# uberalex974/Reinforcement-Learning

Hardware: AMD Instinct MI355X
Metric: env-steps/sec (whole node) at 32768 arenas; PPO wall-clock per 1M steps (higher is better)
Workload: dtype f32

## Files before the change

### include/rlgpu_env.h

```cpp
#ifndef RLGPU_ENV_H
#define RLGPU_ENV_H

#include <stdint.h>
#include "rlgpu_arith.h"
#include "rlgpu_core.h"

#ifdef __cplusplus
extern "C" {
#endif

#define RLGPU_CARS 4
#define RLGPU_PADS 34
#define RLGPU_MANIFOLDS 12
#define RLGPU_MAX_SOLVER_ROWS 14
#define RLGPU_MAX_MESH_OBJECTS 32
#define RLGPU_OBS 167
#define RLGPU_ACTIONS 90
#define RLGPU_REWARDS 13
#define RLGPU_MAX_REWARDS 32
#define RLGPU_MAX_TERMINALS 8
#define RLGPU_SS_KICKOFF 0
#define RLGPU_SS_FUZZED_KICKOFF 1

enum {
// ... 96 lines not shown
    uint8_t prev_is_flipping[RLGPU_CARS];
    uint8_t prev_on_ground[RLGPU_CARS];
    uint8_t has_prev;
    uint8_t terminal;
    uint8_t pad[2];
    float prev_action[RLGPU_CARS][8];
    float no_touch_time;
    int32_t score_blue, score_orange;
    int32_t penalty_blue, penalty_orange;
    uint8_t ev_bump[RLGPU_CARS], ev_bumped[RLGPU_CARS], ev_demo[RLGPU_CARS], ev_demoed[RLGPU_CARS];
    uint32_t rng_counter;
    uint32_t manifold_overflow;
    int32_t episode_steps;
    uint16_t bp_cell[RLGPU_CARS + 1];
    uint8_t bp_rank[RLGPU_CARS + 1];
    uint8_t pad1;
} rlgpu_env_extra;

typedef struct {
    rlgpu_body ball;
    float ball_vel_impulse_cache[3];
    int32_t ball_sleeping;
    rlgpu_car cars[RLGPU_CARS];
    rlgpu_pad pads[RLGPU_PADS];
    rlgpu_env_extra env;
} rlgpu_arena_state;

typedef struct {
    int32_t num_arenas;
    int32_t tick_skip;
    int32_t action_delay;
    uint64_t seed;
    int32_t save_rewards;
    int32_t max_episode_steps;
    const float* mesh_tris;
    int32_t mesh_ntris;
    int32_t mesh_objects;
    const int32_t* mesh_object_ntris;
    const rlgpu_reward_spec* rewards;
    int32_t n_rewards;
    const rlgpu_terminal_spec* terminals;
    int32_t n_terminals;
    int32_t arith;
    int32_t arena_offset;
    int32_t state_setter;
} rlgpu_envset_config;

typedef struct {
    float* obs;
    uint8_t* masks;
    float* rewards;
    int8_t* terminals;
    float* trunc_obs;
} rlgpu_step_outputs;

typedef struct rlgpu_envset rlgpu_envset;

typedef struct {
    float* obs;
    uint8_t* action_masks;
    float* rewards;
    uint8_t* terminals;
    float* last_rewards;
    float* trunc_obs;
    int32_t num_players;
    int32_t num_arenas;
    int32_t num_rewards;
    int32_t* arena_player_start;
} rlgpu_envset_buffers;

int rlgpu_envset_create(const rlgpu_envset_config* cfg, rlgpu_envset** out);
int rlgpu_envset_destroy(rlgpu_envset* env);
int rlgpu_envset_buffers_get(rlgpu_envset* env, rlgpu_envset_buffers* out);

int rlgpu_envset_reset(rlgpu_envset* env, void* stream);
int rlgpu_envset_reset_arenas(rlgpu_envset* env, const uint8_t* d_mask, void* stream);

int rlgpu_envset_step_first_half(rlgpu_envset* env, void* stream);
int rlgpu_envset_step_second_half(rlgpu_envset* env, const int32_t* d_actions, void* stream);
int rlgpu_envset_step(rlgpu_envset* env, const int32_t* d_actions, int32_t reset_terminated,
                      const rlgpu_step_outputs* out, void* stream);
int rlgpu_envset_step_range(rlgpu_envset* env, int32_t first, int32_t count, const int32_t* d_actions,
                            int32_t reset_terminated, const rlgpu_step_outputs* out, void* stream);
int rlgpu_envset_sync(rlgpu_envset* env, void* stream);
int rlgpu_envset_set_output_only(rlgpu_envset* env, int32_t enable);

int rlgpu_envset_get_arenas(rlgpu_envset* env, int32_t first, int32_t count, rlgpu_arena_state* h_out);
int rlgpu_envset_set_arenas(rlgpu_envset* env, int32_t first, int32_t count, const rlgpu_arena_state* h_in);
int rlgpu_envset_build_obs(rlgpu_envset* env, void* stream);

int rlgpu_envset_set_profile(rlgpu_envset* env, unsigned long long* d_counters, int64_t capacity);

enum {
    RLGPU_SM_IN_AIR = 0,
    RLGPU_SM_BALL_TOUCH = 1,
    RLGPU_SM_DEMOED = 2,
    RLGPU_SM_SPEED = 3,
    RLGPU_SM_SPEED_TO_BALL = 4,
    RLGPU_SM_BOOST = 5,
    RLGPU_SM_TOUCH_HEIGHT = 6,
    RLGPU_SM_GOAL_SPEED = 7,
    RLGPU_NUM_STEP_METRICS = 8,
    RLGPU_SM_SLOT_GOAL_SPEED = 28,
    RLGPU_SM_SLOT_GOALS = 29,
    RLGPU_SM_SLOT_PASSES = 30,
    RLGPU_STEP_METRIC_SLOTS = 32
};
const char* rlgpu_step_metric_name(int32_t i);
int rlgpu_envset_enable_step_metrics(rlgpu_envset* env, int32_t enable);
int rlgpu_envset_step_metrics(rlgpu_envset* env, double* h_total, uint64_t* h_count, int32_t reset, void* stream);
int rlgpu_envset_step_metric_slots(rlgpu_envset* env, double* h_out, void* stream);

int rlgpu_envset_default_plugins(rlgpu_reward_spec* rewards, int32_t* n_rewards, rlgpu_terminal_spec* terminals,
                                 int32_t* n_terminals);

int rlgpu_arena_state_size(void);

#ifdef __cplusplus
}
#endif
#endif
```

### include/rlgpu_ppo.h

```cpp
#ifndef RLGPU_PPO_H
#define RLGPU_PPO_H

#include <stdint.h>
#include "rlgpu_core.h"

#ifdef __cplusplus
extern "C" {
#endif

#define RLGPU_MAX_LAYERS 8

typedef struct {
    int32_t obs_size;
    int32_t num_actions;
    int32_t policy_layers[RLGPU_MAX_LAYERS];
    int32_t n_policy_layers;
    int32_t critic_layers[RLGPU_MAX_LAYERS];
    int32_t n_critic_layers;
    int32_t layer_norm;
    float leaky_slope;
    int32_t activation;
    float policy_lr, critic_lr;
    float beta1, beta2, eps, weight_decay;
    float clip_range;
    float entropy_scale;
    float max_grad_norm;
    int32_t max_rows;
    uint64_t seed;
    int32_t train_gemm;
    int32_t infer_fp16;
    int32_t shared_layers[RLGPU_MAX_LAYERS];
    int32_t n_shared_layers;
    int64_t sample_row_offset;
    float policy_temperature;
    int32_t mask_entropy;
} rlgpu_ppo_config;

enum { RLGPU_GEMM_F32X6 = 0, RLGPU_GEMM_F32 = 1, RLGPU_GEMM_F16X3 = 2 };
enum { RLGPU_ACT_LEAKY_RELU = 0, RLGPU_ACT_RELU = 1, RLGPU_ACT_SIGMOID = 2, RLGPU_ACT_TANH = 3 };
enum { RLGPU_INFER_BF16 = 0, RLGPU_INFER_F16 = 1, RLGPU_INFER_F32 = 2 };

typedef struct rlgpu_ppo rlgpu_ppo;

enum {
    RLGPU_M_ENTROPY = 0, RLGPU_M_KL, RLGPU_M_POLICY_LOSS, RLGPU_M_CRITIC_LOSS, RLGPU_M_RATIO,
    RLGPU_M_CLIP_FRACTION, RLGPU_M_COUNT, RLGPU_M_GRAD_NORM_POLICY, RLGPU_M_GRAD_NORM_CRITIC,
    RLGPU_M_GRAD_NORM_SHARED, RLGPU_NUM_METRICS = 16
};

int rlgpu_ppo_create(const rlgpu_ppo_config* cfg, rlgpu_ppo** out);
int rlgpu_ppo_destroy(rlgpu_ppo* h);
int32_t rlgpu_ppo_config_size(void);

int rlgpu_ppo_buffers(rlgpu_ppo* h, float** d_params, float** d_grads, int64_t* num_params);
int rlgpu_ppo_model_range(rlgpu_ppo* h, int32_t model, int64_t* offset, int64_t* count);
int rlgpu_ppo_init_params(rlgpu_ppo* h, uint64_t seed, void* stream);
int rlgpu_ppo_refresh_half(rlgpu_ppo* h, void* stream);

int rlgpu_debug_infer_trace(void* d_buf, int64_t capacity);
int rlgpu_kernel_timing(int32_t enable);
int rlgpu_kernel_timing_read(double* ms, double* work, int64_t* count, int32_t nslots);

int rlgpu_ppo_forward(rlgpu_ppo* h, int32_t model, int32_t precision, const float* d_in, int32_t n,
                      float* d_out, void* stream);

int rlgpu_ppo_infer_actions(rlgpu_ppo* h, const float* d_obs, const uint8_t* d_masks, int32_t n,
                            int32_t deterministic, uint64_t rng_step, int32_t* d_actions, float* d_logp,
                            void* stream);
int rlgpu_ppo_set_version(rlgpu_ppo* h, const float* d_policy_params, void* stream);
int rlgpu_ppo_infer_actions_mixed(rlgpu_ppo* h, const float* d_obs, const uint8_t* d_masks, int32_t n,
                                  int32_t deterministic, uint64_t rng_step, const uint8_t* d_old_rows,
                                  int32_t* d_actions, float* d_logp, void* stream);
int rlgpu_ppo_infer_actions_rows(rlgpu_ppo* h, const float* d_obs, const uint8_t* d_masks, int32_t n, int64_t row0,
                                 int32_t deterministic, uint64_t rng_step, const uint8_t* d_old_rows,
                                 int32_t* d_actions, float* d_logp, void* stream);
int rlgpu_ppo_fused_infer(rlgpu_ppo* h, int32_t model);
int rlgpu_ppo_infer_critic(rlgpu_ppo* h, const float* d_obs, int64_t n, float* d_values, void* stream);

int rlgpu_mean_std(const float* d_x, int64_t n, float* d_out, void* stream);

int rlgpu_ppo_minibatch(rlgpu_ppo* h, const float* d_obs, const uint8_t* d_masks, const int32_t* d_actions,
                        const float* d_old_logp, const float* d_adv, const float* d_target,
                        const int32_t* d_index, int64_t start, int32_t n, int64_t batch_size,
                        const float* d_adv_stats, float* d_metrics, void* stream);

int rlgpu_ppo_optimizer_step(rlgpu_ppo* h, float* d_metrics, void* stream);
int rlgpu_ppo_zero_grad(rlgpu_ppo* h, void* stream);
int rlgpu_ppo_optimizer_state(rlgpu_ppo* h, int64_t* step, float** d_exp_avg, float** d_exp_avg_sq);
int rlgpu_ppo_set_optimizer_step(rlgpu_ppo* h, int64_t step);

int rlgpu_gemm(int32_t mode, int32_t a_layout, int32_t b_layout, const float* d_A, int64_t lda, const float* d_B,
               int64_t ldb, float* d_C, int64_t ldc, const float* d_bias, int32_t I, int32_t J, int32_t K, int32_t splits,
               void* stream);
int rlgpu_gemm_f32(int32_t a_layout, int32_t b_layout, const float* d_A, int64_t lda, const float* d_B, int64_t ldb,
                   float* d_C, int64_t ldc, const float* d_bias, int32_t I, int32_t J, int32_t K, int32_t splits,
                   void* stream);

int rlgpu_permutation(int64_t n, uint64_t seed, uint64_t counter, int32_t* d_out, void* stream);

#ifdef __cplusplus
}
#endif
#endif
```

### reinforcement-learning_amd/csrc/common.hpp

```cpp
#pragma once
#include <hip/hip_runtime.h>
#include <cstdint>
#include <cstdio>
#include <stdexcept>
#include <string>

#include "../../include/rlgpu_core.h"

namespace rlgpu {

void set_last_error(const std::string& msg);

struct Error : std::runtime_error {
    int code;
    Error(int c, const std::string& m) : std::runtime_error(m), code(c) {}
};

#define RLGPU_CHECK_HIP(expr)                                                                \
    do {                                                                                     \
        hipError_t _e = (expr);                                                              \
        if (_e != hipSuccess)                                                                \
            throw ::rlgpu::Error(RLGPU_ERR_HIP, std::string(#expr " failed: ") +             \
                                                    hipGetErrorString(_e));                  \
    } while (0)

#define RLGPU_REQUIRE(cond, msg)                                                             \
    do {                                                                                     \
        if (!(cond)) throw ::rlgpu::Error(RLGPU_ERR_INVALID_ARG, std::string(msg));          \
    } while (0)

template <class F>
inline int guarded(F&& f) {
    try {
        f();
        return RLGPU_OK;
    } catch (const Error& e) {
        set_last_error(e.what());
        return e.code;
    } catch (const std::bad_alloc&) {
        set_last_error("host allocation failed");
        return RLGPU_ERR_OOM;
    } catch (const std::exception& e) {
        set_last_error(e.what());
        return RLGPU_ERR_STATE;
    }
}

inline hipStream_t as_stream(void* s) { return reinterpret_cast<hipStream_t>(s); }

inline unsigned ceil_div(int64_t a, int64_t b) { return (unsigned)((a + b - 1) / b); }

void launch_mlp_infer_act(int act, bool f16, unsigned blocks, hipStream_t s, const void* args, size_t bytes);

}
```

### reinforcement-learning_amd/csrc/env.hip

```cpp
#include <mutex>
#include <algorithm>
#include <cmath>
#include <cstring>
#include <string>
#include <vector>

#include "common.hpp"
#include "env_step.hpp"
#include "mesh.hpp"
#include "../../include/rlgpu_gamestate.h"

namespace rl {
void env_k0_upload(const EnvConst& k, const RsqrtLut* lut);
void env_k1_upload(const EnvConst& k, const RsqrtLut* lut);
void env_k2_upload(const EnvConst& k, const RsqrtLut* lut);
void env_k0_launch(const StepArgs& g, int blocks, hipStream_t s);
void env_k1_launch(const StepArgs& g, int blocks, hipStream_t s);
void env_k2_launch(const StepArgs& g, int blocks, hipStream_t s);

static m3 host_euler_ypr(float yaw, float pitch, float roll) {
    float ci = std::cos(roll), cj = std::cos(pitch), ch = std::cos(yaw);
    float si = std::sin(roll), sj = std::sin(pitch), sh = std::sin(yaw);
    float cc = ci * ch, cs = ci * sh, sc = si * ch, ss = si * sh;
    return m3{v3{cj * ch, sj * sc - cs, sj * cc + ss}, v3{cj * sh, sj * ss + cc, sj * cs - sc}, v3{-sj, cj * si, cj * ci}};
}

static EnvConst make_env_const() {
    EnvConst k;
    std::memset(&k, 0, sizeof k);
    const float UU = 1.f / 50.f;
    k.ball_radius = 91.25f * UU;
    float elem = 0.4f * kBallMass * k.ball_radius * k.ball_radius;
    k.ball_inv_inertia = v3{1.f / elem, 1.f / elem, 1.f / elem};
    k.ball_inv_mass = 1.f / kBallMass;
    v3 hs = v3{120.507f, 86.6994f, 38.6591f} * UU;
    v3 h = v3{hs.x / 2.f, hs.y / 2.f, hs.z / 2.f};
    const float m0 = 0.04f;
    v3 impl = v3{h.x - m0, h.y - m0, h.z - m0};
    const float mn_half = h.x < h.y ? (h.x < h.z ? h.x : h.z) : (h.y < h.z ? h.y : h.z);
    const float safe = 0.1f * mn_half;
    k.car_margin = m0;
    if (safe < k.car_margin) {
        const v3 with_m = impl + v3{m0, m0, m0};
        k.car_margin = safe;
        impl = with_m - v3{safe, safe, safe};
    }
    k.car_impl = impl;
    {
        const v3 mn = v3{-4500.f * UU, -6000.f * UU, 0.f * UU}, mx = v3{4500.f * UU, 6000.f * UU, 2500.f * UU};
        const float cell = 370.f * UU * 1.f;
        const v3 range = mx - mn;
        k.bp_min = mn;
        k.bp_inv_cell = 1.f / cell;
        k.bp_cells[0] = std::max(1, (int)std::ceil(range.x / cell));
        k.bp_cells[1] = std::max(1, (int)std::ceil(range.y / cell));
        k.bp_cells[2] = std::max(1, (int)std::ceil(range.z / cell));
    }
    k.car_half = impl + v3{k.car_margin, k.car_margin, k.car_margin};
    k.car_offset = v3{13.87566f, 0.f, 20.755f} * UU;
    float lx = 2.f * k.car_half.x, ly = 2.f * k.car_half.y, lz = 2.f * k.car_half.z;
    v3 inertia = v3{ly * ly + lz * lz, lx * lx + lz * lz, lx * lx + ly * ly} * (kCarMass / 12.f);
    k.car_inv_inertia = v3{1.f / inertia.x, 1.f / inertia.y, 1.f / inertia.z};
    k.car_inv_mass = 1.f / kCarMass;
    for (int i = 0; i < 4; i++) {
        bool front = i < 2, left = i % 2;
        float radius = front ? 12.50f : 15.00f;
        v3 off = front ? v3{51.25f, 25.90f, 20.755f} : v3{-33.75f, 29.50f, 20.755f};
        if (left) off.y *= -1;
        float rest = (front ? 38.755f : 37.055f) - 12.f;
        k.wheel_conn[i] = off * UU;
        k.wheel_rest[i] = rest * UU;
        k.wheel_radius[i] = radius * UU;
        k.wheel_force_scale[i] = front ? (36.f - (1.f / 4.f)) : (54.f + (1.f / 4.f) + (1.5f / 100.f));
    }
    k.susp_travel = ((12.f * UU) * 100.f) / 100.f;
    k.ball_cbt = (float)((double)k.ball_radius + 0.08) * 0.02f;
    {
        v3 mn = k.car_offset - k.car_half, mx = k.car_offset + k.car_half;
        v3 c = (mn + mx) * 0.5f;
        float r = len(mx - mn) * 0.5f;
        k.car_cbt = (r + len(c)) * 0.02f;
    }
    k.gravity = v3{0, 0, -650.f} * UU;
    k.ball_damp = (float)std::pow((double)(1.f - 0.03f), (double)(1.f / 120.f));
    k.plane_n[0] = v3{0, 0, 1};
    k.plane_p[0] = v3{0, 0, 0};
    k.plane_n[1] = v3{0, 0, -1};
    k.plane_p[1] = v3{0, 0, 2048} * UU;
    k.plane_n[2] = v3{1, 0, 0};
    k.plane_p[2] = v3{-4096, 0, 2048 / 2} * UU;
    k.plane_n[3] = v3{-1, 0, 0};
    k.plane_p[3] = v3{4096, 0, 2048 / 2} * UU;
    for (int p = 0; p < 4; p++) {
        const v3 n = k.plane_n[p];
        k.plane_axis[p] = -1;
        if (std::fabs(n.x) == 1.f && n.y == 0.f && n.z == 0.f) k.plane_axis[p] = 0;
        if (n.x == 0.f && std::fabs(n.y) == 1.f && n.z == 0.f) k.plane_axis[p] = 1;
        if (n.x == 0.f && n.y == 0.f && std::fabs(n.z) == 1.f) k.plane_axis[p] = 2;
    }
    const float sx[5] = {-2048, 2048, -256, 256, 0}, sy[5] = {-2560, -2560, -3840, -3840, -4608};
    const float syaw[5] = {(float)(M_PI_4 * 1), (float)(M_PI_4 * 3), (float)(M_PI_4 * 2), (float)(M_PI_4 * 2), (float)(M_PI_4 * 2)};
// ... 181 lines not shown
        for (int i = 0; i < p.nr; i++) {
            const rlgpu_reward_spec& r = cfg->rewards[i];
            if (r.type < 0 || r.type >= RLGPU_NUM_REWARD_TYPES)
                throw rlgpu::Error(RLGPU_ERR_UNSUPPORTED,
                                   "rlgpu_envset_create: reward " + std::to_string(i) + " has unknown type " +
                                       std::to_string(r.type) + " (the device registry holds types 0.." +
                                       std::to_string(RLGPU_NUM_REWARD_TYPES - 1) + ", include/rlgpu_env.h RLGPU_RW_*)");
            p.rw[i] = r;
        }
    } else {
        RLGPU_REQUIRE(cfg->n_rewards == 0, "rlgpu_envset_create: n_rewards without a rewards list");
    }
    if (cfg->terminals) {
        RLGPU_REQUIRE(cfg->n_terminals >= 0 && cfg->n_terminals <= RLGPU_MAX_TERMINALS,
                      "rlgpu_envset_create: n_terminals must be in [0, " + std::to_string(RLGPU_MAX_TERMINALS) + "]");
        p.nt = cfg->n_terminals;
        for (int i = 0; i < p.nt; i++) {
            const rlgpu_terminal_spec& t = cfg->terminals[i];
            if (t.type < 0 || t.type >= RLGPU_NUM_TERMINAL_TYPES)
                throw rlgpu::Error(RLGPU_ERR_UNSUPPORTED,
                                   "rlgpu_envset_create: terminal condition " + std::to_string(i) + " has unknown type " +
                                       std::to_string(t.type) + " (the device registry holds types 0.." +
                                       std::to_string(RLGPU_NUM_TERMINAL_TYPES - 1) + ", include/rlgpu_env.h RLGPU_TC_*)");
            p.tc[i] = t;
        }
    } else {
        RLGPU_REQUIRE(cfg->n_terminals == 0, "rlgpu_envset_create: n_terminals without a terminals list");
    }
    return p;
}
}

extern "C" int rlgpu_envset_default_plugins(rlgpu_reward_spec* rewards, int32_t* n_rewards, rlgpu_terminal_spec* terminals,
                                            int32_t* n_terminals) {
    return rlgpu::guarded([&] {
        rl::Plugins p;
        example_main_plugins(p);
        if (rewards) std::memcpy(rewards, p.rw, sizeof(rlgpu_reward_spec) * p.nr);
        if (n_rewards) *n_rewards = p.nr;
        if (terminals) std::memcpy(terminals, p.tc, sizeof(rlgpu_terminal_spec) * p.nt);
        if (n_terminals) *n_terminals = p.nt;
    });
}

namespace {
struct EnvKernel {
    void (*upload)(const rl::EnvConst& k, const rl::RsqrtLut* lut);
    void (*launch)(const rl::StepArgs& g, int blocks, hipStream_t s);
};
const EnvKernel kEnvKernel[RLGPU_NUM_ARITH] = {{rl::env_k0_upload, rl::env_k0_launch},
                                               {rl::env_k1_upload, rl::env_k1_launch},
                                               {rl::env_k2_upload, rl::env_k2_launch}};
static_assert(RLGPU_ARITH_MSVC_X64 == 0 && RLGPU_ARITH_GCC_X64 == 1 && RLGPU_ARITH_SCALAR == 2, "kEnvKernel's order");

std::mutex g_init_mu;
struct DeviceInit {
    bool consts = false, rsqrt = false;
};
std::vector<DeviceInit> g_device_init;

void device_init(int arith) {
    std::lock_guard<std::mutex> lk(g_init_mu);
    int dev = 0;
    RLGPU_CHECK_HIP(hipGetDevice(&dev));
    if ((int)g_device_init.size() <= dev) g_device_init.resize(dev + 1);
    DeviceInit& done = g_device_init[dev];
    const bool consts = !done.consts, rsqrt = rl::sse_api(arith) && !done.rsqrt;
    if (!consts && !rsqrt) return;
    rl::RsqrtLut L{};
    if (rsqrt) {
        int bits = 0;
        const std::vector<uint32_t>& t = rlgpu::x86_rsqrt_table_or_throw(&bits);
        uint32_t* d = nullptr;
        RLGPU_CHECK_HIP(hipMalloc(&d, t.size() * sizeof(uint32_t)));
        RLGPU_CHECK_HIP(hipMemcpy(d, t.data(), t.size() * sizeof(uint32_t), hipMemcpyHostToDevice));
        L = rl::RsqrtLut{d, bits};
        RLGPU_CHECK_HIP(hipMemcpyToSymbol(HIP_SYMBOL(rl::kRsqrtLut), &L, sizeof L));
    }
    const rl::EnvConst k = rl::make_env_const();
    if (consts) RLGPU_CHECK_HIP(hipMemcpyToSymbol(HIP_SYMBOL(rl::C), &k, sizeof k));
    for (int a = 0; a < RLGPU_NUM_ARITH; a++) {
        const bool lut = rsqrt && rl::sse_api(a);
        if (consts || lut) kEnvKernel[a].upload(k, lut ? &L : nullptr);
    }
    done.consts = true;
    done.rsqrt = done.rsqrt || rsqrt;
}

void output_only_rows(const rlgpu_envset* e, rl::StepArgs& g) {
    if (!e->output_only) return;
    if (g.out_obs) g.obs = nullptr;
    if (g.out_masks) g.masks = nullptr;
    if (g.out_trunc) g.trunc_obs = nullptr;
}

struct Range {
    int first, count;
};
Range whole(const rlgpu_envset* e) { return Range{0, e->cfg.num_arenas}; }

void launch(rlgpu_envset* e, rl::StepArgs g, Range r, hipStream_t s) {
    const size_t a0 = (size_t)r.first, p0 = a0 * 4, nr = (size_t)e->plug.nr;
    g.arenas = e->d_arenas + a0 * rl::kRec;
    g.n = r.count;
    g.obs = e->d_obs + p0 * RLGPU_OBS;
    g.masks = e->d_masks + p0 * RLGPU_ACTIONS;
    g.rewards = e->d_rewards + p0;
    g.terminals = e->d_terminals + a0;
    g.last_rewards = e->cfg.save_rewards ? e->d_last_rewards + a0 * nr : nullptr;
    g.trunc_obs = e->d_trunc_obs + p0 * RLGPU_OBS;
    g.seed = e->cfg.seed;
    g.max_episode_steps = e->cfg.max_episode_steps;
    g.prof = e->d_prof;
    g.mesh = e->mesh;
    g.mesh.gjk = e->mesh.gjk + a0 / rl::kArenas * rl::kWG;
    g.plug = e->d_plug;
    g.arith = e->cfg.arith;
    g.arena_offset = e->cfg.arena_offset + r.first;
    g.fuzz = e->cfg.state_setter == RLGPU_SS_FUZZED_KICKOFF;
    g.pen_slots = e->pen_slots;
    g.reward_values = g.build && e->d_reward_values ? e->d_reward_values + p0 * nr : nullptr;
    output_only_rows(e, g);
    if (g.build && e->d_metrics) {
        if (r.first == 0) e->metric_players = (++e->metric_calls % 4) == 0;
        g.metrics = e->d_metrics + a0 * RLGPU_STEP_METRIC_SLOTS;
        g.metrics_players = e->metric_players;
    }
    kEnvKernel[e->cfg.arith].launch(g, rlgpu::ceil_div(r.count, rl::kArenas), s);
    RLGPU_CHECK_HIP(hipGetLastError());
}

rl::StepArgs blank(rl::ResetMode reset = rl::kResetNone) {
    rl::StepArgs g;
    std::memset(&g, 0, sizeof g);
    g.reset_mode = reset;
    return g;
}

rl::StepArgs step_args(const rlgpu_envset* e, bool first_half, const int32_t* d_actions,
                       rl::ResetMode reset = rl::kResetNone, const rlgpu_step_outputs* out = nullptr) {
    rl::StepArgs g = blank(reset);
    if (first_half) g.ticks_first = e->cfg.action_delay;
    if (d_actions) {
        g.actions = d_actions;
        g.ticks_second = e->cfg.tick_skip - e->cfg.action_delay;
        g.build = 1;
    }
    if (out) {
        g.out_obs = out->obs;
        g.out_masks = out->masks;
        g.out_rew = out->rewards;
        g.out_term = out->terminals;
        g.out_trunc = out->trunc_obs;
    }
    return g;
}

rl::StepArgs fused_step_args(const rlgpu_envset* e, const int32_t* d_actions, int32_t reset_terminated,
                             const rlgpu_step_outputs* out) {
    RLGPU_REQUIRE(e->cfg.action_delay > 0, "fused step needs actionDelay > 0");
    return step_args(e, true, d_actions, reset_terminated ? rl::kResetTerminated : rl::kResetNone, out);
}

void copy_records(const rlgpu_envset* e, int first, int count, void* host, hipMemcpyKind dir) {
    char* dev = e->d_arenas + (size_t)first * rl::kRec;
    const size_t rec = sizeof(rlgpu_arena_state);
    if (dir == hipMemcpyDeviceToHost)
        RLGPU_CHECK_HIP(hipMemcpy2D(host, rec, dev, rl::kRec, rec, count, dir));
    else
        RLGPU_CHECK_HIP(hipMemcpy2D(dev, rl::kRec, host, rec, rec, count, dir));
}

void download_metric_slots(const rlgpu_envset* e, double* h_out, hipStream_t s) {
    RLGPU_REQUIRE(e->d_metrics, "step metrics are not enabled (rlgpu_envset_enable_step_metrics)");
    RLGPU_CHECK_HIP(hipMemcpyAsync(h_out, e->d_metrics,
                                   (size_t)e->cfg.num_arenas * RLGPU_STEP_METRIC_SLOTS * sizeof(double),
                                   hipMemcpyDeviceToHost, s));
    RLGPU_CHECK_HIP(hipStreamSynchronize(s));
}

void free_set(rlgpu_envset* e) {
    for (void* p : e->allocs) (void)hipFree(p);
    (void)hipFree(e->d_metrics);
    (void)hipFree(e->d_reward_values);
    delete e;
}

}

extern "C" int rlgpu_arena_state_size(void) { return (int)sizeof(rlgpu_arena_state); }

extern "C" int rlgpu_envset_create(const rlgpu_envset_config* cfg, rlgpu_envset** out) {
    return rlgpu::guarded([&] {
        RLGPU_REQUIRE(cfg && out, "rlgpu_envset_create: null argument");
        RLGPU_REQUIRE(cfg->num_arenas > 0, "rlgpu_envset_create: num_arenas must be > 0");
        RLGPU_REQUIRE(cfg->tick_skip > 0, "tickSkip must be > 0 (EnvSet.cpp:48)");
        RLGPU_REQUIRE(cfg->action_delay >= 0 && cfg->action_delay <= cfg->tick_skip,
                      "actionDelay must be in [0, tickSkip] (EnvSet.cpp:49)");
        RLGPU_REQUIRE(cfg->mesh_tris == nullptr || cfg->mesh_ntris > 0, "mesh_ntris must be > 0 with mesh_tris");
        RLGPU_REQUIRE(cfg->arith >= 0 && cfg->arith < RLGPU_NUM_ARITH,
                      "rlgpu_envset_create: unknown arithmetic mode " + std::to_string(cfg->arith) + " (RLGPU_ARITH_*)");
        RLGPU_REQUIRE(cfg->state_setter == RLGPU_SS_KICKOFF || cfg->state_setter == RLGPU_SS_FUZZED_KICKOFF,
                      "rlgpu_envset_create: unknown state setter " + std::to_string(cfg->state_setter) + " (RLGPU_SS_*)");
        const rl::Plugins plug = plugins_from(cfg);
        device_init(cfg->arith);
        std::vector<float> builtin;
        const float* tris = cfg->mesh_tris;
        int ntris = cfg->mesh_ntris;
        if (!tris) {
            builtin = rlgpu::builtin_mesh_bt();
            tris = builtin.data();
// ... 156 lines not shown
}

extern "C" float* rlgpu_envset_reward_values(rlgpu_envset* e) { return e ? e->d_reward_values : nullptr; }

extern "C" int rlgpu_envset_download_gamestates(rlgpu_envset* e, int32_t first, int32_t count, rlgpu_gamestate* h_out,
                                                void* stream) {
    return rlgpu::guarded([&] {
        RLGPU_REQUIRE(e && h_out, "rlgpu_envset_download_gamestates: null argument");
        RLGPU_REQUIRE(first >= 0 && count >= 0 && first + count <= e->cfg.num_arenas, "arena range out of bounds");
        if (count == 0) return;
        RLGPU_CHECK_HIP(hipStreamSynchronize(rlgpu::as_stream(stream)));
        std::vector<rlgpu_arena_state> rec((size_t)count);
        copy_records(e, first, count, rec.data(), hipMemcpyDeviceToHost);
        rlgpu::gamestates_from_arenas(rec.data(), count, e->cfg.tick_skip, h_out);
    });
}

extern "C" int rlgpu_envset_buffers_get(rlgpu_envset* e, rlgpu_envset_buffers* out) {
    return rlgpu::guarded([&] {
        RLGPU_REQUIRE(e && out, "rlgpu_envset_buffers_get: null argument");
        out->obs = e->d_obs;
        out->action_masks = e->d_masks;
        out->rewards = e->d_rewards;
        out->terminals = e->d_terminals;
        out->last_rewards = e->d_last_rewards;
        out->trunc_obs = e->d_trunc_obs;
        out->num_players = e->num_players;
        out->num_arenas = e->cfg.num_arenas;
        out->num_rewards = e->plug.nr;
        out->arena_player_start = e->d_player_start;
    });
}

extern "C" int rlgpu_envset_reset(rlgpu_envset* e, void* stream) {
    return rlgpu::guarded([&] {
        RLGPU_REQUIRE(e, "null envset");
        launch(e, blank(rl::kResetSet), whole(e), rlgpu::as_stream(stream));
    });
}

extern "C" int rlgpu_envset_reset_arenas(rlgpu_envset* e, const uint8_t* d_mask, void* stream) {
    return rlgpu::guarded([&] {
        RLGPU_REQUIRE(e, "null envset");
        rl::StepArgs g = blank(rl::kResetMask);
        g.reset_mask = d_mask;
        launch(e, g, whole(e), rlgpu::as_stream(stream));
    });
}

extern "C" int rlgpu_envset_step_first_half(rlgpu_envset* e, void* stream) {
    return rlgpu::guarded([&] {
        RLGPU_REQUIRE(e, "null envset");
        launch(e, step_args(e, true, nullptr), whole(e), rlgpu::as_stream(stream));
    });
}

extern "C" int rlgpu_envset_step_second_half(rlgpu_envset* e, const int32_t* d_actions, void* stream) {
    return rlgpu::guarded([&] {
        RLGPU_REQUIRE(e && d_actions, "rlgpu_envset_step_second_half: null argument");
        launch(e, step_args(e, false, d_actions), whole(e), rlgpu::as_stream(stream));
    });
}

extern "C" int rlgpu_envset_step(rlgpu_envset* e, const int32_t* d_actions, int32_t reset_terminated,
                                 const rlgpu_step_outputs* out, void* stream) {
    return rlgpu::guarded([&] {
        RLGPU_REQUIRE(e && d_actions, "rlgpu_envset_step: null argument");
        launch(e, fused_step_args(e, d_actions, reset_terminated, out), whole(e), rlgpu::as_stream(stream));
    });
}

extern "C" int rlgpu_envset_step_range(rlgpu_envset* e, int32_t first, int32_t count, const int32_t* d_actions,
                                       int32_t reset_terminated, const rlgpu_step_outputs* out, void* stream) {
    return rlgpu::guarded([&] {
        RLGPU_REQUIRE(e && d_actions, "rlgpu_envset_step_range: null argument");
        const rl::StepArgs g = fused_step_args(e, d_actions, reset_terminated, out);
        RLGPU_REQUIRE(first >= 0 && count > 0 && first + count <= e->cfg.num_arenas && first % rl::kArenas == 0,
                      "rlgpu_envset_step_range: the range must lie in the set and start at a multiple of 4");
        RLGPU_REQUIRE(!e->d_prof, "rlgpu_envset_step_range: not with the per-phase profile");
        launch(e, g, Range{first, count}, rlgpu::as_stream(stream));
    });
}

extern "C" int rlgpu_envset_set_output_only(rlgpu_envset* e, int32_t enable) {
    return rlgpu::guarded([&] {
        RLGPU_REQUIRE(e, "null envset");
        e->output_only = enable != 0;
    });
}

extern "C" int rlgpu_envset_sync(rlgpu_envset* e, void* stream) {
    return rlgpu::guarded([&] {
        RLGPU_REQUIRE(e, "null envset");
        RLGPU_CHECK_HIP(hipStreamSynchronize(rlgpu::as_stream(stream)));
    });
}

extern "C" int rlgpu_envset_build_obs(rlgpu_envset* e, void* stream) {
    return rlgpu::guarded([&] {
        RLGPU_REQUIRE(e, "null envset");
        launch(e, blank(rl::kRebuildObs), whole(e), rlgpu::as_stream(stream));
    });
}

extern "C" int rlgpu_envset_get_arenas(rlgpu_envset* e, int32_t first, int32_t count, rlgpu_arena_state* h_out) {
    return rlgpu::guarded([&] {
        RLGPU_REQUIRE(e && h_out, "null argument");
        RLGPU_REQUIRE(first >= 0 && count >= 0 && first + count <= e->cfg.num_arenas, "arena range out of bounds");
        if (count == 0) return;
        RLGPU_CHECK_HIP(hipDeviceSynchronize());
        copy_records(e, first, count, h_out, hipMemcpyDeviceToHost);
    });
}

extern "C" int rlgpu_envset_set_arenas(rlgpu_envset* e, int32_t first, int32_t count, const rlgpu_arena_state* h_in) {
    return rlgpu::guarded([&] {
        RLGPU_REQUIRE(e && h_in, "null argument");
        RLGPU_REQUIRE(first >= 0 && count >= 0 && first + count <= e->cfg.num_arenas, "arena range out of bounds");
        if (count == 0) return;
        RLGPU_CHECK_HIP(hipDeviceSynchronize());
        copy_records(e, first, count, const_cast<rlgpu_arena_state*>(h_in), hipMemcpyHostToDevice);
    });
}

namespace rl {
__global__ void __launch_bounds__(16) box_triangle_kernel(int n, const float* rot, const float* centre, const float* tri,
                                                          const float* cbt, float* out, gjk::GjkScratch* scratch,
                                                          int lds, int ar) {
    __shared__ char small[16][gjk::kSmallBytes];
    __shared__ int lock[16];
    const int i = blockIdx.x * 16 + threadIdx.x;
    lock[threadIdx.x] = 0;
    if (i >= n) return;
    const float* r = rot + 9 * (size_t)i;
    const m3 R = m3{v3{r[0], r[1], r[2]}, v3{r[3], r[4], r[5]}, v3{r[6], r[7], r[8]}};
    const v3 c = v3{centre[3 * (size_t)i], centre[3 * (size_t)i + 1], centre[3 * (size_t)i + 2]};
    const float* t = tri + 9 * (size_t)i;
    const gjk::Shape sh{C.car_impl, C.car_margin, v3{t[0], t[1], t[2]}, v3{t[3], t[4], t[5]}, v3{t[6], t[7], t[8]}, ar};
    v3 nrm, pt;
    float d = 0.f;
    gjk::Scr slow = gjk::hbm_view(scratch + i);
    gjk::Scr fast = gjk::lds_view(small[threadIdx.x]);
    const bool hit = gjk::box_triangle(R, c, sh, cbt[i], lds ? &fast : nullptr, &lock[threadIdx.x], slow, nrm, pt, d);
    float* o = out + 8 * (size_t)i;
    o[0] = hit ? 1.f : 0.f;
    o[1] = hit ? nrm.x : 0.f;
    o[2] = hit ? nrm.y : 0.f;
    o[3] = hit ? nrm.z : 0.f;
    o[4] = hit ? pt.x : 0.f;
    o[5] = hit ? pt.y : 0.f;
    o[6] = hit ? pt.z : 0.f;
    o[7] = hit ? d : 0.f;
}
__device__ __forceinline__ void bt_load(int i, const float* rot, const float* centre, const float* tri, int ar, m3& R, v3& c,
                                        gjk::Shape& sh) {
    const float* r = rot + 9 * (size_t)i;
    R = m3{v3{r[0], r[1], r[2]}, v3{r[3], r[4], r[5]}, v3{r[6], r[7], r[8]}};
    c = v3{centre[3 * (size_t)i], centre[3 * (size_t)i + 1], centre[3 * (size_t)i + 2]};
    const float* t = tri + 9 * (size_t)i;
    sh = gjk::Shape{C.car_impl, C.car_margin, v3{t[0], t[1], t[2]}, v3{t[3], t[4], t[5]}, v3{t[6], t[7], t[8]}, ar};
}
__device__ __forceinline__ void bt_store(float* out, int i, bool hit, v3 nrm, v3 pt, float d) {
    float* o = out + 8 * (size_t)i;
    o[0] = hit ? 1.f : 0.f;
    o[1] = hit ? nrm.x : 0.f;
    o[2] = hit ? nrm.y : 0.f;
// ... 162 lines not shown
```

### reinforcement-learning_amd/csrc/env_step.hpp

```cpp
#pragma once
#include "env_builders.hpp"

namespace rl {

enum ResetMode : int {
    kResetNone = 0,
    kResetTerminated = 1,
    kResetSet = 2,
    kResetMask = 3,
    kResetAll = 4,
    kRebuildObs = 5
};

struct StepArgs {
    char* arenas;
    int n;
    int ticks_first;
    const int32_t* actions;
    int ticks_second;
    int build;
    int reset_mode;
    const uint8_t* reset_mask;
    float* obs;
    uint8_t* masks;
    float* rewards;
    uint8_t* terminals;
    float* last_rewards;
    float* trunc_obs;
    float* out_obs;
    uint8_t* out_masks;
    float* out_rew;
    int8_t* out_term;
    float* out_trunc;
    int max_episode_steps;
    uint64_t seed;
    unsigned long long* prof;
    MeshView mesh;
    double* metrics;
    int metrics_players;
    const Plugins* plug;
    int arith;
    int arena_offset;
    float* reward_values;
    int fuzz;
    int pen_slots;
};

#ifdef RLGPU_ENV_KERNEL

DEV void step_metrics(ArenaLDS* A, int l, double* m, bool players) {
    if (players) {
        const rlgpu_car& c = A->s.cars[l];
        const v3 pos = ld3(c.body.pos) * kBT2UU, vel = ld3(c.body.vel) * kBT2UU;
        const v3 bp = ld3(A->s.ball.pos) * kBT2UU;
        const bool touched = A->a.touched[l] != 0;
        const v3 dir = rs_norm(bp - pos);
        const float toward = vel.x * dir.x + vel.y * dir.y + vel.z * dir.z;
        m[RLGPU_SM_IN_AIR * 4 + l] += c.is_on_ground ? 0.0 : 1.0;
        m[RLGPU_SM_BALL_TOUCH * 4 + l] += touched ? 1.0 : 0.0;
        m[RLGPU_SM_DEMOED * 4 + l] += c.is_demoed ? 1.0 : 0.0;
        m[RLGPU_SM_SPEED * 4 + l] += (double)rs_len(vel);
        m[RLGPU_SM_SPEED_TO_BALL * 4 + l] += (double)(0.f > toward ? 0.f : toward);
        m[RLGPU_SM_BOOST * 4 + l] += (double)c.boost;
        if (touched) m[RLGPU_SM_TOUCH_HEIGHT * 4 + l] += (double)bp.z;
    }
    if (l == 0) {
        if (players) m[RLGPU_SM_SLOT_PASSES] += 1.0;
        if (A->a.goal) {
            m[RLGPU_SM_SLOT_GOAL_SPEED] += (double)rs_len(ld3(A->s.ball.vel) * kBT2UU);
            m[RLGPU_SM_SLOT_GOALS] += 1.0;
        }
    }
}


constexpr int kPadsPerLane = (RLGPU_PADS + kTeam - 1) / kTeam;
struct PadRegs {
    int px[kPadsPerLane], py[kPadsPerLane];
    v3 pos[kPadsPerLane], bmin[kPadsPerLane], bmax[kPadsPerLane];
    float rad[kPadsPerLane];
};
DEV void load_pad_regs(PadRegs& R, int l) {
#pragma unroll
    for (int k = 0; k < kPadsPerLane; k++) {
        const int p = l + k * kTeam < RLGPU_PADS ? l + k * kTeam : 0;
        R.px[k] = C.pad_cell_x[p];
        R.py[k] = C.pad_cell_y[p];
        R.pos[k] = C.pad_pos_bt[p];
        R.bmin[k] = C.pad_box_min[p];
        R.bmax[k] = C.pad_box_max[p];
        R.rad[k] = (C.pad_big[p] ? 208.f : 144.f) * kUU2BT;
    }
}

DEV void tick(ArenaLDS* A, const MeshView& M, int l, bool valid, uint64_t seed, int arena, Prof& P, const PadRegs& R,
                          int nvalid) {
    if (valid) {
        rlgpu_arena_state& s = A->s;
        if (l == 0) {
            A->u.wc.njob = 0;
            bool sleep = len2(ld3(s.ball.vel)) == 0 && len2(ld3(s.ball.angvel)) == 0;
            s.ball_sleeping = sleep;
            A->a.ball_sleep = sleep;
            A->a.active[0] = 1;
        } else if (l < 5) {
            const int c = l - 1;
            A->a.active[c + 1] = !s.cars[c].is_demoed;
            float* ctl = s.cars[c].controls;
            for (int k = 0; k < 5; k++) ctl[k] = stdclamp(ctl[k], -1.f, 1.f);
        }
        if (l < 5) {
            A->a.snap_vel[l] = bvel(A, l);
            A->a.snap_ang[l] = bang(A, l);
        }
    }
    sync();
    if (valid && l == 0) {
        rlgpu_arena_state& s = A->s;
        for (int c = 0; c < 4; c++) {
            rlgpu_car& cs = s.cars[c];
            if (cs.is_demoed) {
                cs.demo_respawn_timer = stdmax(cs.demo_respawn_timer - kTick, 0.f);
                if (cs.demo_respawn_timer == 0.f) {
                    int idx = (int)(rng_next(A, seed, arena) % 4u);
                    bool orange = c & 1;
                    v3 pos = v3{C.respawn_x[idx], C.respawn_y[idx] * (orange ? -1.f : 1.f), 36.f};
                    set_car_state(A, c, pos, C.respawn_rot[orange][idx], 100.f / 3.f, false);
                }
            }
        }
    }
// ... 167 lines not shown
            const int px = R.px[k], py = R.py[k];
            const v3 ppos = R.pos[k];
            const float rad = R.rad[k];
            const uint32_t prev_locked = A->s.pads[p].prev_locked_car_id;
            int locked = -1;
#pragma unroll
            for (int ci = 0; ci < 4; ci++) {
                if (px < cx0[ci] || px > cx1[ci] || py < cy0[ci] || py > cy1[ci]) continue;
                v3 cpos = cp[ci];
                bool col = false;
                if (prev_locked == (uint32_t)(ci + 1)) {
                    v3 mn, mx;
                    body_aabb(ci + 1, cpos, ldm(A->s.cars[ci].body.rot), mn, mx);
                    const v3 bmin = R.bmin[k], bmax = R.bmax[k];
                    col = (bmax.x > mn.x && bmax.y > mn.y && bmax.z > mn.z) && (bmin.x < mx.x && bmin.y < mx.y && bmin.z < mx.z);
                } else {
                    float dx = cpos.x - ppos.x, dy = cpos.y - ppos.y;
                    if (dx * dx + dy * dy < rad * rad) col = fabsf(cpos.z - ppos.z) < (95.f * kUU2BT);
                }
                if (col) locked = ci;
            }
            A->a.locked[p] = locked;
        }
    }
    sync();
    P.mark(9);
    uint64_t picked[kPadsPerLane];
#pragma unroll
    for (int k = 0; k < kPadsPerLane; k++) {
        const int p = l + k * kTeam;
        bool pick = false;
        if (valid && p < RLGPU_PADS) {
            rlgpu_pad& pd = A->s.pads[p];
            const int lk = A->a.locked[p];
            if (lk >= 0 && pd.is_active) {
                pick = true;
                pd.is_active = 0;
                pd.cooldown = R.rad[k] > 144.f * kUU2BT ? 10.f : 4.f;
            }
            pd.prev_locked_car_id = lk >= 0 ? (uint32_t)(lk + 1) : 0u;
        }
        picked[k] = __ballot(pick);
    }
    if (valid && l == 0) {
        const int team = (int)(threadIdx.x >> 4);
#pragma unroll
        for (int k = 0; k < kPadsPerLane; k++)
            for (uint32_t bits = (uint32_t)(picked[k] >> (16 * team)) & 0xffffu; bits; bits &= bits - 1u) {
                const int p = __ffs(bits) - 1 + k * kTeam;
                rlgpu_car& cs = A->s.cars[A->a.locked[p]];
                cs.boost = stdmin(cs.boost + (C.pad_big[p] ? 100.f : 12.f), 100.f);
            }
        rlgpu_body* b = &A->s.ball;
        v3 v = ld3(b->vel), w = ld3(b->angvel);
        v3 cache = ld3(A->s.ball_vel_impulse_cache);
        if (!is_zero(cache)) {
            v += cache;
            st3(A->s.ball_vel_impulse_cache, zero3());
        }
        const float maxv = 6000.f * kUU2BT;
        if (len2(v) > maxv * maxv) v = bt_normalize(v, arith(A)) * maxv;
        if (len2(w) > 6.f * 6.f) w = bt_normalize(w, arith(A)) * 6.f;
        st3(b->vel, v);
        st3(b->angvel, w);
        A->s.env.tick_count++;
    }
    sync();
    P.mark(10);
}

DEV void copy_rows(ArenaLDS* A, int l, int arena, float* obs, uint8_t* masks) {
    if (obs) {
        const float* src = &A->u.out.obs[0][0];
        float* dst = obs + (size_t)arena * 4 * RLGPU_OBS;
        for (int k = l; k < 4 * RLGPU_OBS; k += kTeam) dst[k] = src[k];
    }
    if (masks) {
        const uint8_t* msrc = &A->u.out.masks[0][0];
        uint8_t* mdst = masks + (size_t)arena * 4 * RLGPU_ACTIONS;
        for (int k = l; k < 4 * RLGPU_ACTIONS; k += kTeam) mdst[k] = msrc[k];
    }
}

__global__ void __launch_bounds__(kWG) RLGPU_ENV_KERNEL(StepArgs g) {
    __shared__ ArenaLDS lds[kArenas];
    const int team = threadIdx.x >> 4, l = threadIdx.x & 15;
    const int arena = blockIdx.x * kArenas + team;
    const bool valid = arena < g.n;
    ArenaLDS* A = &lds[team];
    Prof P{g.prof, g.prof ? (long long)clock64() : 0};
    {
        int first = blockIdx.x * kArenas;
        int cnt = g.n - first < kArenas ? g.n - first : kArenas;
        const int chunks = kRec / 16;
        for (int k = threadIdx.x; k < cnt * chunks; k += kWG) {
            int a = k / chunks, c = k % chunks;
            const uint4* src = (const uint4*)(g.arenas + (size_t)(first + a) * kRec) + c;
            uint4* dst = (uint4*)&lds[a] + c;
            *dst = *src;
        }
    }
    sync(); P.mark(11);
    if (valid && l < 5) {
        A->a.force[l] = zero3();
        A->a.torque[l] = zero3();
        update_inertia(A, l);
    }
    if (l == 0) {
        A->a.epa_lock = A->a.npen = 0;
        A->a.arith = g.arith;
    }
    if (threadIdx.x == 0) g_pen_save.cap = g.pen_slots;
    sync(); P.mark(11);
    if (g.ticks_first > 0) {
        if (valid && l == 0) {
            rlgpu_env_extra& e = A->s.env;
            for (int i = 0; i < 3; i++) e.prev_ball_vel[i] = A->s.ball.vel[i] * kBT2UU;
            for (int i = 0; i < 4; i++) {
                e.prev_boost[i] = A->s.cars[i].boost;
                e.prev_is_flipping[i] = A->s.cars[i].is_flipping;
                e.prev_on_ground[i] = A->s.cars[i].is_on_ground;
                e.ev_bump[i] = e.ev_bumped[i] = e.ev_demo[i] = e.ev_demoed[i] = 0;
            }
            e.has_prev = 1;
        }
        sync(); P.mark(11);
    }
    {
        PadRegs pregs;
        load_pad_regs(pregs, l);
        const int t1 = g.ticks_first, t2 = g.actions ? g.ticks_second : 0;
        for (int t = 0;; t++) {
            if (g.actions && t == t1) {
                if (valid && l < 4) {
                    int a = g.actions[arena * 4 + l];
                    a = a < 0 ? 0 : (a > RLGPU_ACTIONS - 1 ? RLGPU_ACTIONS - 1 : a);
                    const float* x = C.action[a];
                    float* c = A->s.cars[l].controls;
                    for (int k = 0; k < 5; k++) c[k] = x[k];
                    c[5] = x[5] == 1 ? 1.f : 0.f;
                    c[6] = x[6] == 1 ? 1.f : 0.f;
                    c[7] = x[7] == 1 ? 1.f : 0.f;
                    for (int k = 0; k < 8; k++) A->s.env.prev_action[l][k] = x[k];
                }
                sync(); P.mark(11);
            }
            if (t >= t1 + t2) break;
            tick(A, g.mesh, l, valid, g.seed, arena + g.arena_offset, P, pregs, stdmin(kArenas, g.n - (int)blockIdx.x * kArenas));
        }
    }
    uint8_t term = 0;
    if (g.build) {
        if (valid && l == 0) {
            rlgpu_env_extra& e = A->s.env;
            int64_t cur = e.tick_count;
            int64_t tick_skip = cur - e.last_tick_count > 0 ? cur - e.last_tick_count : 0;
            float delta_time = (int)tick_skip * (1.0f / 120.0f);
            bool any = false;
            for (int i = 0; i < 4; i++) {
                const rlgpu_car& c = A->s.cars[i];
                bool t = c.ball_hit_valid && (uint64_t)c.ball_hit_tick >= (uint64_t)(cur - tick_skip);
                A->a.touched[i] = t;
                any |= t;
            }
            float by = A->s.ball.pos[1] * kBT2UU;
            bool goal = fabsf(by) > (5124.25f + 91.25f);
            A->a.goal = goal;
            if (any) e.no_touch_time = 0;
            else e.no_touch_time += delta_time;
            if (goal) {
                if (by > 0) e.score_blue++;
                else e.score_orange++;
            }
            uint8_t tt = 0;
            for (int k = 0; k < g.plug->nt; k++) {
                const rlgpu_terminal_spec& tc = g.plug->tc[k];
                bool hit = false, trunc = false;
                if (tc.type == RLGPU_TC_NO_TOUCH) {
                    hit = !any && e.no_touch_time >= tc.param;
                    trunc = true;
                } else if (tc.type == RLGPU_TC_SCORE_LIMIT) {
                    const int lim = (int)tc.param;
                    hit = (e.score_blue >= lim) || (e.score_orange >= lim);
                } else if (tc.type == RLGPU_TC_GOAL_SCORE) {
                    hit = goal;
                }
                if (hit) {
                    const uint8_t cur = trunc ? 2 : 1;
                    if (tt == 0 || cur == 1) tt = cur;
                }
            }
            e.terminal = tt;
            if (goal) {
                if (by > 0) e.penalty_blue++;
                else e.penalty_orange++;
            }
            e.episode_steps++;
            uint8_t tj = tt;
            if (!tj && g.max_episode_steps > 0 && e.episode_steps >= g.max_episode_steps) tj = 2;
            if (tj) e.episode_steps = 0;
            A->a.traj_term = tj;
        }
        sync(); P.mark(12);
        if (valid) {
            const int pi = l & 3, q = l >> 2;
            const PView me = view_player(A, pi);
            v3 bp = ld3(A->s.ball.pos) * kBT2UU, bv = ld3(A->s.ball.vel) * kBT2UU, pbv = ld3(A->s.env.prev_ball_vel);
            const int nr = g.plug->nr;
            constexpr int kPer = (RLGPU_MAX_REWARDS + 3) / 4;
            float ov[kPer];
#pragma unroll
            for (int k = 0; k < kPer; k++) ov[k] = 0.f;
#pragma unroll 1
            for (int k = 0; q + 4 * k < nr; k++) {
                const int r = q + 4 * k;
                const float o = reward_value(A, g.plug->rw[r], pi, me, bp, bv, pbv, A->a.goal != 0);
#pragma unroll
                for (int j = 0; j < kPer; j++) ov[j] = j == k ? o : ov[j];
                if (pi == 0 && g.last_rewards) g.last_rewards[(size_t)arena * nr + r] = o;
                if (g.reward_values) g.reward_values[((size_t)arena * 4 + pi) * nr + r] = o;
            }
            float all = 0.f;
            const int base = (int)(threadIdx.x & ~15u) + pi;
#pragma unroll
            for (int r = 0; r < RLGPU_MAX_REWARDS; r++) {
                if (r >= nr) break;
                const float o = __shfl(ov[r >> 2], base + 4 * (r & 3));
                all += o * g.plug->rw[r].weight;
            }
            if (l < 4) A->a.all_rewards[l] = all;
        }
        sync(); P.mark(12);
        if (valid && l < 4) {
            float r = A->a.all_rewards[l];
            g.rewards[arena * 4 + l] = r;
            if (g.out_rew) g.out_rew[arena * 4 + l] = r;
            if (g.out_term) g.out_term[arena * 4 + l] = (int8_t)A->a.traj_term;
        }
        if (g.metrics && valid && l < 4) step_metrics(A, l, g.metrics + (size_t)arena * RLGPU_STEP_METRIC_SLOTS,
                                                      g.metrics_players != 0);
        uint8_t tj = 0;
        if (valid) {
            term = A->s.env.terminal;
            tj = (uint8_t)A->a.traj_term;
        }
        sync(); P.mark(12);
        if (valid && l == 0) {
            g.terminals[arena] = term;
            A->s.env.last_tick_count = A->s.env.tick_count;
        }
        const bool fused_reset = g.reset_mode == kResetTerminated && valid && term != 0;
        if (valid) build_obs_rows(A, l);
        sync(); P.mark(13);
        if (valid) {
            copy_rows(A, l, arena, g.obs, g.masks);
            if (!fused_reset) copy_rows(A, l, arena, g.out_obs, g.out_masks);
            if (tj == 2) {
                copy_rows(A, l, arena, g.trunc_obs, nullptr);
                copy_rows(A, l, arena, g.out_trunc, nullptr);
            }
        }
        sync(); P.mark(13);
        if (g.reset_mode == kResetTerminated) {
            if (fused_reset && l == 0) kickoff_reset(A, g.seed, arena + g.arena_offset, g.fuzz != 0);
            sync(); P.mark(14);
            if (fused_reset) build_obs_rows(A, l);
            sync(); P.mark(14);
            if (fused_reset) {
                copy_rows(A, l, arena, g.obs, g.masks);
                copy_rows(A, l, arena, g.out_obs, g.out_masks);
            }
            sync(); P.mark(14);
        }
    }
    if (g.reset_mode >= kResetSet) {
        bool do_reset = false;
        if (valid) {
            if (g.reset_mode == kResetSet) do_reset = g.terminals[arena] != 0;
            else if (g.reset_mode == kResetMask) do_reset = g.reset_mask ? g.reset_mask[arena] != 0 : true;
            else if (g.reset_mode == kResetAll) do_reset = true;
        }
        sync(); P.mark(14);
        if (do_reset && l == 0) {
            kickoff_reset(A, g.seed, arena + g.arena_offset, g.fuzz != 0);
            if (g.reset_mode == kResetSet) g.terminals[arena] = 0;
        }
        sync(); P.mark(14);
        bool rebuild = do_reset || (valid && g.reset_mode == kRebuildObs);
        if (rebuild) build_obs_rows(A, l);
        sync(); P.mark(14);
        if (rebuild) copy_rows(A, l, arena, g.obs, g.masks);
        sync(); P.mark(14);
    }
    {
        int first = blockIdx.x * kArenas;
        int cnt = g.n - first < kArenas ? g.n - first : kArenas;
        const int chunks = kRec / 16;
        for (int k = threadIdx.x; k < cnt * chunks; k += kWG) {
            int a = k / chunks, c = k % chunks;
            uint4* dst = (uint4*)(g.arenas + (size_t)(first + a) * kRec) + c;
            const uint4* src = (const uint4*)&lds[a] + c;
            *dst = *src;
        }
    }
    P.mark(15);
    if (g.prof && valid && l == 0 && A->a.npen) {
        atomicAdd(&g.prof[28], (unsigned long long)A->a.npen);
        atomicAdd(&g.prof[kProfWG + (size_t)blockIdx.x * kProfPhases + 23], (unsigned long long)A->a.npen);
        atomicAdd(&g.prof[kProfWG + (size_t)gridDim.x * kProfPhases + arena], (unsigned long long)A->a.npen);
    }
}
#endif

}
```

### reinforcement-learning_amd/csrc/infer_kernels.hpp

```cpp
#pragma once
#include <hip/hip_runtime.h>
#include <stdint.h>

#include "mlp_kernels.hpp"
#include "ppo_kernels.hpp"

namespace infer {

using mlp::bf16x8;
using mlp::f32x16;
using mlp::h2f;
using mlp::f2h;
using mlp::u32x4;

constexpr int IR = 64;
constexpr int IW = 8;
constexpr int IT = 64 * IW;
constexpr int IRW = IR / IW;
constexpr int IMAX = 512;
constexpr int IPITCH = IMAX + 8;
constexpr int kSampleProbs = 128;
static_assert(ppo::kMaxA <= kSampleProbs && kSampleProbs * 2 + ppo::kMaxA * 4 <= IPITCH * 2, "probs fit a row of Xs");
constexpr int IOUT = 128;
constexpr int kMaxLinear = 9;
// ... 8 lines not shown
    const int64_t blk = e >> 9;
    const int ks = (int)(blk % KS), jt = (int)(blk / KS);
    const int j = jt * 32 + (l & 31), k = ks * 16 + 8 * (l >> 5) + el;
    f[e] = (j < out && k < in) ? mlp::f2h<F16>(w[(int64_t)j * in + k]) : (uint16_t)0;
}

struct InferArgs {
    const float* X;
    int n, in;
    const uint16_t* P;
    const uint16_t* F;
    int nl;
    int width[kMaxLinear + 1];
    int64_t fw[kMaxLinear];
    int64_t hb[kMaxLinear], hg[kMaxLinear], hbe[kMaxLinear];
    float slope;
    int use_ln;
    int mode;
    float* out_f;
    const uint8_t* masks;
    int det;
    float temp;
    uint64_t seed, step;
    int64_t row0;
    int32_t* act;
    float* logp;
    const uint8_t* row_sel;
    int sel;
    unsigned long long* trace;
};
#define INFER_MARK(p) \
    if (a.trace && threadIdx.x == 0) a.trace[blockIdx.x * 16 + (p)] = wall_clock64()

template <int NR, int NC, bool F16>
DEV void linear_tiles(const uint16_t (*Xs)[IPITCH], const uint16_t* F, int KS, const int (&jt)[NC], int ti0, int nc_act,
                      int lane, f32x16 (&acc)[NR][NC]) {
    const uint16_t* base[NC];
#pragma unroll
    for (int c = 0; c < NC; c++) base[c] = F + ((int64_t)jt[c] * KS * 64 + lane) * 8;
    const uint16_t* arow[NR];
#pragma unroll
    for (int i = 0; i < NR; i++) {
        arow[i] = Xs[(ti0 + i) * 32 + (lane & 31)] + 8 * (lane >> 5);
#pragma unroll
        for (int c = 0; c < NC; c++)
#pragma unroll
            for (int r = 0; r < 16; r++) acc[i][c][r] = 0.f;
    }
    const int nch = (KS + 3) / 4;
    auto load = [&](u32x4 (&b)[4][NC], int kc) {
#pragma unroll
        for (int s = 0; s < 4; s++) {
            const int ks = min(kc * 4 + s, KS - 1);
#pragma unroll
            for (int c = 0; c < NC; c++) b[s][c] = *reinterpret_cast<const u32x4*>(base[c] + ks * 512);
        }
    };
    auto step = [&](const u32x4 (&b)[4][NC], int kc) {
#pragma unroll
        for (int s = 0; s < 4; s++) {
            const int ks = kc * 4 + s;
            if (ks >= KS) break;
            bf16x8 av[NR];
#pragma unroll
            for (int i = 0; i < NR; i++) av[i] = *reinterpret_cast<const bf16x8*>(arow[i] + ks * 16);
#pragma unroll
            for (int c = 0; c < NC; c++) {
                if (c >= nc_act) break;
#pragma unroll
                for (int i = 0; i < NR; i++) acc[i][c] = mlp::mfma16<F16>(av[i], __builtin_bit_cast(bf16x8, b[s][c]), acc[i][c]);
            }
        }
    };
    u32x4 b0[4][NC], b1[4][NC];
    load(b0, 0);
    for (int kc = 0; kc < nch; kc += 2) {
        load(b1, kc + 1);
        step(b0, kc);
        load(b0, kc + 2);
        step(b1, kc + 1);
    }
}

template <int MAXH, bool FULL, bool F16, int ACT>
DEV void ln_act_rows(uint16_t (*Xs)[IPITCH], const uint16_t* gamma, const uint16_t* beta, int H, float slope, int use_ln,
                     int w, int lane) {
    const bool vec = (H % 8 == 0) && (MAXH % 8 == 0);
    const bool maxform = slope >= 0.f && slope <= 1.f;
    auto in = [&](int q) { return FULL || mlp::hcol<MAXH>(lane, q) < H; };
    float g[MAXH], b[MAXH];
#pragma unroll
    for (int q = 0; q < MAXH; q++) {
        const int c = mlp::hcol<MAXH>(lane, q);
        g[q] = (use_ln && in(q)) ? h2f<F16>(gamma[c]) : 1.f;
        b[q] = (use_ln && in(q)) ? h2f<F16>(beta[c]) : 0.f;
    }
    float v[IRW][MAXH];
#pragma unroll
    for (int rg = 0; rg < IRW; rg++) {
        const uint16_t* z = Xs[w + IW * rg];
        if (vec) {
#pragma unroll
            for (int q = 0; q < MAXH; q += 8) {
                const int c = mlp::hcol<MAXH>(lane, q);
                u32x4 t = {0u, 0u, 0u, 0u};
                if (in(q)) t = *reinterpret_cast<const u32x4*>(z + c);
#pragma unroll
                for (int k = 0; k < 4; k++) {
                    v[rg][q + 2 * k] = h2f<F16>((uint16_t)(t[k] & 0xffffu));
                    v[rg][q + 2 * k + 1] = h2f<F16>((uint16_t)(t[k] >> 16));
                }
            }
        } else {
#pragma unroll
            for (int q = 0; q < MAXH; q++) {
                const int c = mlp::hcol<MAXH>(lane, q);
                v[rg][q] = in(q) ? h2f<F16>(z[c]) : 0.f;
            }
        }
    }
    if (use_ln) {
        float s[IRW];
#pragma unroll
        for (int rg = 0; rg < IRW; rg++) {
            s[rg] = 0.f;
#pragma unroll
            for (int q = 0; q < MAXH; q++) s[rg] += v[rg][q];
        }
#pragma unroll
        for (int rg = 0; rg < IRW; rg++) s[rg] = mlp::wave_sum_x(s[rg]);
#pragma unroll
        for (int rg = 0; rg < IRW; rg++) {
            const float mean = s[rg] / (float)H;
            float s2 = 0.f;
#pragma unroll
            for (int q = 0; q < MAXH; q++) {
                v[rg][q] = in(q) ? v[rg][q] - mean : 0.f;
                s2 += v[rg][q] * v[rg][q];
            }
            s[rg] = s2;
        }
#pragma unroll
        for (int rg = 0; rg < IRW; rg++) {
            s[rg] = mlp::wave_sum_x(s[rg]);
            const float rs = 1.f / sqrtf(s[rg] / (float)H + 1e-5f);
#pragma unroll
            for (int q = 0; q < MAXH; q++) v[rg][q] = h2f<F16>(f2h<F16>(v[rg][q] * rs * g[q] + b[q]));
        }
    }
#pragma unroll
    for (int rg = 0; rg < IRW; rg++) {
        uint16_t* z = Xs[w + IW * rg];
        uint16_t o[MAXH];
#pragma unroll
        for (int q = 0; q < MAXH; q++) {
            const float hv = v[rg][q];
            o[q] = f2h<F16>(mlp::act_fwd<ACT>(hv, slope, maxform));
        }
        if (vec) {
#pragma unroll
            for (int q = 0; q < MAXH; q += 8) {
                const int c = mlp::hcol<MAXH>(lane, q);
                u32x4 t;
#pragma unroll
                for (int k = 0; k < 4; k++) t[k] = (uint32_t)o[q + 2 * k] | ((uint32_t)o[q + 2 * k + 1] << 16);
                if (in(q)) *reinterpret_cast<u32x4*>(z + c) = t;
            }
        } else {
#pragma unroll
// ... 99 lines not shown
        if (t + IT * u < ptot) putp(t + IT * u, pv[u]);
    for (int f = t + IT * UP; f < ptot; f += IT) putp(f, a.P[pslot(f).src]);
    if (a.mode == 1) {
#pragma unroll
        for (int u = 0; u < UM; u++)
            if (t + IT * u < nd) *reinterpret_cast<uint32_t*>(&Ms[4 * (t + IT * u)]) = mv[u];
        for (int i = t + IT * UM; i < nd; i += IT)
            *reinterpret_cast<uint32_t*>(&Ms[4 * i]) = *reinterpret_cast<const uint32_t*>(msrc + 4 * i);
        for (int f = 4 * nd + t; f < mtot; f += IT) Ms[f] = msrc[f];
        if (t < IR) Sel[t] = t < rows && selv;
    }
    for (int l = 0; l + 1 < a.nl; l++) {
        const int KS = (a.width[l] + 15) / 16, N = a.width[l + 1], JT = (N + 31) / 32;
        const int jt[2] = {min(w, JT - 1), min(w + IW, JT - 1)};
        const int nt = (w < JT) + (w + IW < JT);
        f32x16 acc[2][2];
        __syncthreads();
        if (l < 3) INFER_MARK(1 + 2 * l);
        linear_tiles<2, 2, F16>(Xs, a.F + a.fw[l], KS, jt, 0, nt, lane, acc);
        __syncthreads();
        if (l < 3) INFER_MARK(2 + 2 * l);
        const uint16_t* bias = Pv[l][0];
        const int n16 = (N + 15) / 16 * 16;
#pragma unroll
        for (int c = 0; c < 2; c++) {
            const int j = (w + IW * c) * 32 + (lane & 31);
            if (c >= nt || j >= n16) continue;
            const float bj = j < N ? h2f<F16>(bias[j]) : 0.f;
#pragma unroll
            for (int i = 0; i < 2; i++)
#pragma unroll
                for (int r = 0; r < 16; r++)
                    Xs[acc_row(i, r, lane)][j] = j < N ? f2h<F16>(acc[i][c][r] + bj) : (uint16_t)0;
        }
        const uint16_t* gg = Pv[l][1];
        const uint16_t* bb = Pv[l][2];
        __syncthreads();
        if (l < 3) INFER_MARK(8 + l);
        if (N == 512) ln_act_rows<8, true, F16, ACT>(Xs, gg, bb, N, a.slope, a.use_ln, w, lane);
        else if (N <= 64) ln_act_rows<1, false, F16, ACT>(Xs, gg, bb, N, a.slope, a.use_ln, w, lane);
        else if (N <= 128) ln_act_rows<2, false, F16, ACT>(Xs, gg, bb, N, a.slope, a.use_ln, w, lane);
        else if (N <= 256) ln_act_rows<4, false, F16, ACT>(Xs, gg, bb, N, a.slope, a.use_ln, w, lane);
        else ln_act_rows<8, false, F16, ACT>(Xs, gg, bb, N, a.slope, a.use_ln, w, lane);
    }
    const int l = a.nl - 1, KS = (a.width[l] + 15) / 16, N = a.width[l + 1], JT = (N + 31) / 32;
    const int jt[1] = {min(w & 3, JT - 1)}, ti = w >> 2;
    f32x16 acc[1][1];
    __syncthreads();
    INFER_MARK(12);
    linear_tiles<1, 1, F16>(Xs, a.F + a.fw[l], KS, jt, ti, (w & 3) < JT, lane, acc);
    INFER_MARK(13);
    const int j = (w & 3) * 32 + (lane & 31);
    const float bj = j < N ? h2f<F16>(Pv[l][0][j]) : 0.f;
    if (a.mode == 0) {
        if (j < N)
#pragma unroll
            for (int r = 0; r < 16; r++) {
                const int i = r0 + acc_row(ti, r, lane);
                if (i < a.n) a.out_f[(int64_t)i * N + j] = h2f<F16>(f2h<F16>(acc[0][0][r] + bj));
            }
        return;
    }
    __syncthreads();
    if (j < N)
#pragma unroll
        for (int r = 0; r < 16; r++) Xs[acc_row(ti, r, lane)][j] = f2h<F16>(acc[0][0][r] + bj);
    __syncthreads();
    INFER_MARK(14);
    {
        const auto rowfn = [&](int g, const uint16_t*& lg, const uint8_t*& mk, float*& pr, int& row, bool& ok) {
            const int r = w + IW * g;
            lg = Xs[r];
            mk = Ms + r * N;
            pr = reinterpret_cast<float*>(&Xs[r][kSampleProbs]);
            row = r0 + r;
            ok = Sel[r] != 0;
        };
        const auto mark = [&](int k) { INFER_MARK(k == 0 ? 7 : 11); };
        ppo::sample_rows_looped<IRW, F16>(rowfn, N, a.temp, a.det, a.seed, a.step, a.row0, lane, a.act, a.logp, mark);
    }
    INFER_MARK(15);
}

}
```

### reinforcement-learning_amd/csrc/ppo.hip

```cpp
#include <hipcub/hipcub.hpp>

#include <cmath>
#include <cstring>
#include <type_traits>
#include <vector>

#include "../../include/rlgpu_ppo.h"
#include "common.hpp"
#include "mlp_kernels.hpp"
#include "ppo_kernels.hpp"
#include "infer_kernels.hpp"

namespace {

using rlgpu::ceil_div;

#define RLGPU_H16_LAUNCH(F16, KERN, ...)                                                     \
    do {                                                                                     \
        if (F16) hipLaunchKernelGGL(KERN<true>, __VA_ARGS__);                                \
        else hipLaunchKernelGGL(KERN<false>, __VA_ARGS__);                                   \
    } while (0)

struct Side {
    int64_t planes = -1;
// ... 518 lines not shown
    const int64_t e = (int64_t)n * h->xh_ld;
    RLGPU_H16_LAUNCH(f16(h), mlp::rows_to_bf16, dim3(ceil_div(e, 256)), dim3(256), 0, s, X, h->cfg.obs_size, n, h->xh, h->xh_ld);
    RLGPU_CHECK_HIP(hipGetLastError());
    const uint16_t* in = h->xh;
    int64_t ld = h->xh_ld;
    int cur = 0;
    for (const Link& k : h->chain[mi]) {
        const Layer& L = *k.L;
        mlp::HGemmArgs g;
        g.A = in;
        g.B = P + L.hw;
        g.bias = P + L.hb;
        g.C = k.hidden ? h->zh : h->logits_h;
        g.lda = ld;
        g.ldb = L.in_pad;
        g.ldc = L.out;
        g.I = n;
        g.J = L.out;
        g.K = L.in_pad;
        g.gx = (int)ceil_div(L.out, mlp::BN);
        g.gy = (int)ceil_div(n, mlp::BM);
        RLGPU_H16_LAUNCH(f16(h), mlp::gemm_bf16, dim3(g.gx * g.gy), dim3(256), 0, s, g);
        RLGPU_CHECK_HIP(hipGetLastError());
        if (!k.hidden) return h->logits_h;
        const uint16_t* gg = L.hg >= 0 ? P + L.hg : nullptr;
        const uint16_t* bb = L.hbe >= 0 ? P + L.hbe : nullptr;
        hipLaunchKernelGGL(f16(h) ? mlp::ln_act_fwd_bf16_any<true>(L.out, h->cfg.activation) : mlp::ln_act_fwd_bf16_any<false>(L.out, h->cfg.activation),
                           dim3(ceil_div(n, mlp::LNF_ROWS)), dim3(256), 0, s, h->zh, gg, bb, n, L.out,
                           h->cfg.leaky_slope, h->cfg.layer_norm, h->ah[cur]);
        RLGPU_CHECK_HIP(hipGetLastError());
        in = h->ah[cur];
        ld = L.out;
        cur ^= 1;
    }
    return in;
}

void forward_f32(rlgpu_ppo* h, int model, const float* X, int n, float* out, hipStream_t s) {
    gather_obs(h, X, nullptr, 0, n, s);
    if (h->shared()) forward_train(h, 2, obs_input(h), n, nullptr, s);
    forward_train(h, model, model_input(h, model), n, out, s);
}

unsigned long long* g_infer_trace = nullptr;
int64_t g_infer_trace_cap = 0;

void build_chains(rlgpu_ppo* h) {
    for (int mi = 0; mi < 3; mi++) {
        auto& c = h->chain[mi];
        if (mi != 2 && h->shared())
            for (auto& L : h->M[2].L) c.push_back({&L, true});
        const Model& m = h->M[mi];
        for (size_t l = 0; l < m.L.size(); l++) c.push_back({&m.L[l], m.head_only || l + 1 < m.L.size()});
        bool fit = !c.empty() && (int)c.size() <= infer::kMaxLinear && !c.back().hidden;
        for (size_t l = 0; fit && l < c.size(); l++)
            fit = c[l].L->in <= infer::IMAX && c[l].L->out <= (l + 1 < c.size() ? infer::IMAX : infer::IOUT);
        h->fused_fit[mi] = fit;
    }
}
bool fused_ok(const rlgpu_ppo* h, int mi) {
    if (infer_f32(h) || !h->fused_fit[mi]) return false;
    const char* e = getenv("RLGPU_FUSED_INFER");
    return !(e && atoi(e) == 0);
}

struct Rows {
    const float* X;
    int64_t n, row0;
    const uint8_t* masks;
    Rows sub(const rlgpu_ppo_config& c, int64_t b, int64_t m) const {
        return {X + b * c.obs_size, m, row0 + b, masks ? masks + b * c.num_actions : nullptr};
    }
};
struct Draw {
    int det;
    uint64_t step;
    int32_t* act;
    float* logp;
    const uint8_t* row_sel = nullptr;
    int sel = 0;
    Draw sub(int64_t b) const { return {det, step, act + b, logp ? logp + b : nullptr, row_sel ? row_sel + b : nullptr, sel}; }
};

void infer_fused(rlgpu_ppo* h, int mi, bool ver, const Rows& r, float* out_f, const Draw* d, hipStream_t s) {
    const auto& c = h->chain[mi];
    const int n = (int)r.n;
    infer::InferArgs a{};
    a.X = r.X;
    a.n = n;
    a.in = h->cfg.obs_size;
    a.P = ver ? h->half_ver : h->half;
    a.F = ver ? h->frag_ver : h->frag;
    a.nl = (int)c.size();
    a.width[0] = a.in;
    for (int l = 0; l < a.nl; l++) {
        const Layer& L = *c[l].L;
        a.width[l + 1] = L.out;
        a.fw[l] = L.fw;
        a.hb[l] = L.hb;
        a.hg[l] = L.hg;
        a.hbe[l] = L.hbe;
    }
    a.slope = h->cfg.leaky_slope;
    a.use_ln = h->cfg.layer_norm;
    a.seed = h->cfg.seed;
    a.temp = h->cfg.policy_temperature;
    a.out_f = out_f;
    if (d) {
        a.mode = 1;
        a.masks = r.masks;
        a.row0 = r.row0;
        a.det = d->det;
        a.step = d->step;
        a.act = d->act;
        a.logp = d->logp;
        a.row_sel = d->row_sel;
        a.sel = d->sel;
    }
    a.trace = g_infer_trace;
    if (a.trace && ceil_div(n, infer::IR) * 16 > g_infer_trace_cap)
        throw rlgpu::Error(RLGPU_ERR_INVALID_ARG, "rlgpu_debug_infer_trace: buffer of " + std::to_string(g_infer_trace_cap) +
                                                      " entries, this launch needs " + std::to_string(ceil_div(n, infer::IR) * 16));
    if (h->cfg.activation != mlp::ACT_LEAKY)
        rlgpu::launch_mlp_infer_act(h->cfg.activation, f16(h), ceil_div(n, infer::IR), s, &a, sizeof(a));
    else
        RLGPU_H16_LAUNCH(f16(h), infer::mlp_infer, dim3(ceil_div(n, infer::IR)), dim3(infer::IT), 0, s, a);
    RLGPU_CHECK_HIP(hipGetLastError());
}

void infer_values(rlgpu_ppo* h, int mi, const Rows& r, float* out, hipStream_t s, bool half = false) {
    if (infer_f32(h) && !half) return forward_f32(h, mi, r.X, (int)r.n, out, s);
    if (fused_ok(h, mi)) return infer_fused(h, mi, false, r, out, nullptr, s);
    const uint16_t* y = forward_half(h, mi, r.X, (int)r.n, s);
    const int64_t e = r.n * h->M[mi].out;
    RLGPU_H16_LAUNCH(f16(h), ppo::bf16_to_f32, dim3(ceil_div(e, 256)), dim3(256), 0, s, y, out, e);
    RLGPU_CHECK_HIP(hipGetLastError());
}

void sample_pass(rlgpu_ppo* h, bool ver, const Rows& r, const Draw& d, hipStream_t s) {
    if (fused_ok(h, 0)) return infer_fused(h, 0, ver, r, nullptr, &d, s);
    const int n = (int)r.n;
    const auto sample = [&](auto kern, const auto* logits) {
        hipLaunchKernelGGL(kern, dim3(ceil_div(n, 4)), dim3(256), 0, s, logits, r.masks, n, h->cfg.num_actions,
                           h->cfg.policy_temperature, d.det, h->cfg.seed, d.step, r.row0, d.act, d.logp, d.row_sel, d.sel);
        RLGPU_CHECK_HIP(hipGetLastError());
    };
    if (infer_f32(h)) {
        forward_f32(h, 0, r.X, n, h->logits_f, s);
        return sample(ppo::sample_actions<false, float>, h->logits_f);
    }
    const uint16_t* y = forward_half(h, 0, r.X, n, s, ver ? h->half_ver : h->half);
    sample(f16(h) ? ppo::sample_actions<true> : ppo::sample_actions<false>, y);
}

void infer_policy(rlgpu_ppo* h, const Rows& rows, const Draw& draw, const uint8_t* old_rows, int64_t chunk, hipStream_t s) {
    for (int64_t b = 0; b < rows.n; b += chunk) {
        const Rows r = rows.sub(h->cfg, b, std::min(chunk, rows.n - b));
        Draw d = draw.sub(b);
        d.row_sel = old_rows ? old_rows + b : nullptr;
        for (d.sel = 0; d.sel < (old_rows ? 2 : 1); d.sel++) {
            if (d.sel) d.logp = nullptr;
            sample_pass(h, d.sel != 0, r, d, s);
        }
    }
}

Side add_side(Model& m, int rows, int k, bool frag) {
    const bool h3 = m.mode == RLGPU_GEMM_F16X3;
    const int rpad = h3 ? mlp::BNW : mlp::BN;
    Side S;
    S.rows = (int)ceil_div(rows, rpad) * rpad;
    S.ld = (int)ceil_div(k, mlp::XKMAX) * mlp::XKMAX;
    S.planes = m.nsplit;
    m.nsplit += (h3 ? 2 : 3) * S.plane();
    S.scale = m.nscale;
    m.nscale += S.rows;
    if (frag) {
        S.frag = m.nsplit;
        m.nsplit += 2 * (int64_t)mlp::RLN_J * S.ld;
    }
    return S;
}

void build_model(rlgpu_ppo* h, Model& m, int in, const int32_t* layers, int nl, int out, float lr, bool input_grad = false) {
    m.head_only = out == 0;
    if (m.head_only) nl--;
    m.in = in;
    m.out = m.head_only ? layers[nl] : out;
    m.lr = lr;
    m.mode = h->cfg.train_gemm;
    m.akind = h->cfg.activation;
    m.off = h->nparams;
    int prev = in;
    for (int l = 0; l <= nl; l++) {
        Layer L;
        L.in = prev;
        const bool hidden = l < nl || m.head_only;
        L.out = l < nl ? layers[l] : m.out;
        L.w = h->nparams;
        h->nparams += (int64_t)L.in * L.out;
// ... 255 lines not shown
extern "C" int rlgpu_ppo_refresh_half(rlgpu_ppo* h, void* stream) {
    return rlgpu::guarded([&] {
        RLGPU_REQUIRE(h, "null handle");
        refresh_half(h, rlgpu::as_stream(stream));
    });
}

extern "C" int rlgpu_ppo_forward(rlgpu_ppo* h, int32_t model, int32_t precision, const float* d_in, int32_t n, float* d_out,
                                 void* stream) {
    return rlgpu::guarded([&] {
        RLGPU_REQUIRE(h && d_in && d_out, "null argument");
        RLGPU_REQUIRE(model >= 0 && model < h->nm, "model must be 0, 1 or (with a shared head) 2");
        RLGPU_REQUIRE(n >= 0 && n <= h->cfg.max_rows, "n must be in [0, max_rows]");
        if (n == 0) return;
        hipStream_t s = rlgpu::as_stream(stream);
        if (precision != 0) return infer_values(h, model, Rows{d_in, n, 0, nullptr}, d_out, s, true);
        if (model != 2) return forward_f32(h, model, d_in, n, d_out, s);
        gather_obs(h, d_in, nullptr, 0, n, s);
        forward_train(h, 2, obs_input(h), n, nullptr, s);
        RLGPU_CHECK_HIP(hipMemcpyAsync(d_out, model_input(h, 0).X, (int64_t)n * h->M[2].out * sizeof(float),
                                       hipMemcpyDeviceToDevice, s));
    });
}

extern "C" int rlgpu_ppo_infer_actions(rlgpu_ppo* h, const float* d_obs, const uint8_t* d_masks, int32_t n,
                                       int32_t deterministic, uint64_t rng_step, int32_t* d_actions, float* d_logp,
                                       void* stream) {
    return rlgpu::guarded([&] {
        RLGPU_REQUIRE(h && d_obs && d_masks && d_actions, "null argument");
        RLGPU_REQUIRE(n >= 0, "n must be >= 0");
        infer_policy(h, Rows{d_obs, n, h->cfg.sample_row_offset, d_masks}, Draw{deterministic, rng_step, d_actions, d_logp},
                     nullptr, h->cfg.max_rows, rlgpu::as_stream(stream));
    });
}

extern "C" int rlgpu_debug_infer_trace(void* d_buf, int64_t capacity) {
    return rlgpu::guarded([&] {
        RLGPU_REQUIRE(!d_buf || capacity >= 16, "rlgpu_debug_infer_trace: capacity below one workgroup's 16 marks");
        g_infer_trace = (unsigned long long*)d_buf;
        g_infer_trace_cap = d_buf ? capacity : 0;
    });
}

extern "C" int rlgpu_ppo_set_version(rlgpu_ppo* h, const float* d_policy_params, void* stream) {
    return rlgpu::guarded([&] {
        RLGPU_REQUIRE(h && d_policy_params, "rlgpu_ppo_set_version: null argument");
        hipStream_t s = rlgpu::as_stream(stream);
        half_from(h, 0, d_policy_params, h->half_ver, h->frag_ver, s);
        if (h->shared()) half_from(h, 2, d_policy_params + h->M[0].count, h->half_ver, h->frag_ver, s);
        h->has_ver = true;
    });
}

extern "C" int rlgpu_ppo_infer_actions_mixed(rlgpu_ppo* h, const float* d_obs, const uint8_t* d_masks, int32_t n,
                                             int32_t deterministic, uint64_t rng_step, const uint8_t* d_old_rows,
                                             int32_t* d_actions, float* d_logp, void* stream) {
    return rlgpu::guarded([&] {
        RLGPU_REQUIRE(h && d_obs && d_masks && d_actions && d_old_rows, "null argument");
        RLGPU_REQUIRE(h->has_ver, "rlgpu_ppo_infer_actions_mixed: no version set (rlgpu_ppo_set_version)");
        if (infer_f32(h))
            throw rlgpu::Error(RLGPU_ERR_UNSUPPORTED, "rlgpu_ppo_infer_actions_mixed: fp32 inference (RLGPU_INFER_F32) "
                                                      "keeps no old-version copy (self-play needs 16-bit inference)");
        RLGPU_REQUIRE(n >= 0, "n must be >= 0");
        infer_policy(h, Rows{d_obs, n, h->cfg.sample_row_offset, d_masks}, Draw{deterministic, rng_step, d_actions, d_logp},
                     d_old_rows, h->cfg.max_rows, rlgpu::as_stream(stream));
    });
}

extern "C" int rlgpu_ppo_infer_actions_rows(rlgpu_ppo* h, const float* d_obs, const uint8_t* d_masks, int32_t n, int64_t row0,
                                            int32_t deterministic, uint64_t rng_step, const uint8_t* d_old_rows,
                                            int32_t* d_actions, float* d_logp, void* stream) {
    return rlgpu::guarded([&] {
        RLGPU_REQUIRE(h && d_obs && d_masks && d_actions, "null argument");
        RLGPU_REQUIRE(n >= 0 && row0 >= 0, "n and row0 must be >= 0");
        RLGPU_REQUIRE(!d_old_rows || h->has_ver, "rlgpu_ppo_infer_actions_rows: old rows without a version set");
        if (!fused_ok(h, 0))
            throw rlgpu::Error(RLGPU_ERR_UNSUPPORTED, "rlgpu_ppo_infer_actions_rows: the policy is not on the fused kernel "
                                                      "(widths, RLGPU_FUSED_INFER = 0 or fp32 inference)");
        const Rows rows{d_obs, n, row0 + h->cfg.sample_row_offset, d_masks};
        infer_policy(h, rows, Draw{deterministic, rng_step, d_actions, d_logp}, d_old_rows, INT64_MAX, rlgpu::as_stream(stream));
    });
}

extern "C" int rlgpu_ppo_fused_infer(rlgpu_ppo* h, int32_t model) { return h && model >= 0 && model < 3 && fused_ok(h, model); }

extern "C" int rlgpu_ppo_infer_critic(rlgpu_ppo* h, const float* d_obs, int64_t n, float* d_values, void* stream) {
    return rlgpu::guarded([&] {
        RLGPU_REQUIRE(h && d_obs && d_values, "null argument");
        hipStream_t s = rlgpu::as_stream(stream);
        const Rows rows{d_obs, n, 0, nullptr};
        const int64_t R = fused_ok(h, 1) ? (int64_t)1 << 30 : h->cfg.max_rows;
        for (int64_t b = 0; b < n; b += R) infer_values(h, 1, rows.sub(h->cfg, b, std::min(R, n - b)), d_values + b, s);
    });
}

extern "C" int rlgpu_mean_std(const float* d_x, int64_t n, float* d_out, void* stream) {
    return rlgpu::guarded([&] {
        RLGPU_REQUIRE(d_x && d_out && n > 0, "rlgpu_mean_std: bad argument");
        hipStream_t s = rlgpu::as_stream(stream);
        const int nb = 256;
        double* part = nullptr;
        RLGPU_CHECK_HIP(hipMallocAsync((void**)&part, nb * 2 * sizeof(double), s));
        hipLaunchKernelGGL(ppo::moments_partial, dim3(nb), dim3(256), 0, s, d_x, n, part);
        hipLaunchKernelGGL(ppo::moments_final, dim3(1), dim3(64), 0, s, part, nb, n, d_out);
        RLGPU_CHECK_HIP(hipGetLastError());
        RLGPU_CHECK_HIP(hipFreeAsync(part, s));
    });
}

extern "C" int rlgpu_ppo_minibatch(rlgpu_ppo* h, const float* d_obs, const uint8_t* d_masks, const int32_t* d_actions,
                                   const float* d_old_logp, const float* d_adv, const float* d_target, const int32_t* d_index,
                                   int64_t start, int32_t n, int64_t batch_size, const float* d_adv_stats, float* d_metrics,
                                   void* stream) {
    return rlgpu::guarded([&] {
        RLGPU_REQUIRE(h && d_obs && d_masks && d_actions && d_old_logp && d_adv && d_target && d_adv_stats,
                      "rlgpu_ppo_minibatch: null argument");
        RLGPU_REQUIRE(n > 0 && n <= h->cfg.max_rows, "minibatch rows must be in [1, max_rows]");
        RLGPU_REQUIRE(batch_size > 0, "batch_size must be > 0");
        hipStream_t s = rlgpu::as_stream(stream);
        float bsr = (float)n / (float)batch_size;
        int A = h->cfg.num_actions;
        gather_obs(h, d_obs, d_index, start, n, s);
        const Operand obs_in = obs_input(h), xin = model_input(h, 0);
        if (h->shared()) forward_train(h, 2, obs_in, n, nullptr, s);
        hipStream_t cs = h->aux;
        RLGPU_CHECK_HIP(hipEventRecord(h->ev_fork, s));
        RLGPU_CHECK_HIP(hipStreamWaitEvent(h->aux, h->ev_fork, 0));
        Model& pm = h->M[0];
        Model& cm = h->M[1];
        forward_train(h, 1, xin, n, cm.y, cs);
        hipLaunchKernelGGL(ppo::critic_loss, dim3(ceil_div(n, 256)), dim3(256), 0, cs, cm.y, d_target, d_index, start, n,
                           bsr, cm.dy, d_metrics);
        RLGPU_CHECK_HIP(hipGetLastError());
        backward(h, 1, xin, n, cm.dy, cs);
        RLGPU_CHECK_HIP(hipEventRecord(h->ev_join, h->aux));
        forward_train(h, 0, xin, n, pm.y, s);
        const int pl_blocks = (int)ceil_div(n, ppo::PL_ROWS);
        const bool pl_opt = h->cfg.policy_temperature != 1.f || h->cfg.mask_entropy != 0;
        hipLaunchKernelGGL(ppo::policy_loss_any(A, pl_opt), dim3(pl_blocks), dim3(256), 0, s, pm.y, d_masks, d_actions, d_old_logp, d_adv,
                           d_index, start, n, A, d_adv_stats, bsr, h->cfg.clip_range, h->cfg.entropy_scale,
                           1.f / std::log((float)A), h->cfg.policy_temperature, h->cfg.mask_entropy, pm.dy, dout_ld(A), d_metrics,
                           pm.lpart, amax_slot(pm, kAmaxOut));
        RLGPU_CHECK_HIP(hipGetLastError());
        backward(h, 0, xin, n, pm.dy, s, pm.lpart, pl_blocks);
        RLGPU_CHECK_HIP(hipStreamWaitEvent(s, h->ev_join, 0));
        if (h->shared()) {
            const int64_t e = (int64_t)n * h->M[2].out;
            hipLaunchKernelGGL(ppo::add2, dim3(ceil_div(ceil_div(e, 4), 256)), dim3(256), 0, s, pm.dX, cm.dX, h->dshared, e);
            RLGPU_CHECK_HIP(hipGetLastError());
            backward(h, 2, obs_in, n, h->dshared, s);
        }
    });
}

extern "C" int rlgpu_ppo_optimizer_step(rlgpu_ppo* h, float* d_metrics, void* stream) {
    return rlgpu::guarded([&] {
        RLGPU_REQUIRE(h, "null handle");
        hipStream_t s = rlgpu::as_stream(stream);
        h->step++;
        const auto& c = h->cfg;
        double bc1 = 1.0 - std::pow((double)c.beta1, (double)h->step);
        double bc2 = 1.0 - std::pow((double)c.beta2, (double)h->step);
        const int slot[3] = {RLGPU_M_GRAD_NORM_POLICY, RLGPU_M_GRAD_NORM_CRITIC, RLGPU_M_GRAD_NORM_SHARED};
        for (int mi = 0; mi < h->nm; mi++) {
            Model& m = h->M[mi];
            float* coef = h->scratch + 600 + mi;
// ... 164 lines not shown
```

### reinforcement-learning_amd/host/learner.cpp

```cpp
#include "learner.hpp"

#include <algorithm>
#include <chrono>
#include <cmath>
#include <cstdio>
#include <cstring>

#include "../csrc/common.hpp"
#include "../csrc/learner_kernels.hpp"
#include "cu_partition.hpp"

namespace {
constexpr int OBS = RLGPU_OBS, ACT = RLGPU_ACTIONS;
using clk = std::chrono::steady_clock;
double secs(clk::time_point a, clk::time_point b) { return std::chrono::duration<double>(b - a).count(); }

inline void hipCheck(hipError_t e, const char* what) {
    if (e != hipSuccess) throw rlgpu::Error(RLGPU_ERR_HIP, std::string(what) + ": " + hipGetErrorString(e));
}

inline uint64_t splitmix64(uint64_t x) {
    x += 0x9E3779B97F4A7C15ull;
    x = (x ^ (x >> 30)) * 0xBF58476D1CE4E5B9ull;
    x = (x ^ (x >> 27)) * 0x94D049BB133111EBull;
// ... 334 lines not shown
    traj.roff.Free();
    for (auto* a : {&traj.truncObs, &traj.truncVals, &traj.cObs, &traj.cLogp, &traj.cRews, &traj.cVals, &traj.cAdv,
                    &traj.cTarget, &traj.cRet})
        a->Free();
    traj.cMasks.Free();
    traj.cTerms.Free();
    exp_.Free();
    delete ppo_;
    delete env_;
}

constexpr int kAutoCollectGroups = 2;
constexpr int kAutoCollectArenas = 4096;

int Learner::CollectGroups() const {
    const int want = cfg_.collect_groups > 0                   ? cfg_.collect_groups
                     : cfg_.num_arenas >= kAutoCollectArenas ? kAutoCollectGroups
                                                             : 1;
    if (want <= 1 || hook_ || K_ > 1 || trajMode() || !rlgpu_ppo_fused_infer(ppo_->handle(), 0)) return 1;
    if (cfg_.num_arenas % (4 * want) != 0) return 1;
    return want;
}

bool Learner::EnsureGroupStreams(int G) {
    if ((int)gs_.size() == G) return true;
    if (gsRefused_ == G) return false;
    for (auto s : gs_) {
        (void)hipStreamSynchronize(s);
        (void)hipStreamDestroy(s);
    }
    for (auto e : gsEnd_) (void)hipEventDestroy(e);
    gs_.clear();
    gsEnd_.clear();
    std::vector<hipStream_t> ss;
    for (int g = 0; g < G; g++) {
        hipStream_t s = nullptr;
        if (rlgpu::cu_partition_stream(G, g, &s) != hipSuccess) {
            (void)hipGetLastError();
            for (auto x : ss) (void)hipStreamDestroy(x);
            gsRefused_ = G;
            return false;
        }
        ss.push_back(s);
    }
    gs_ = ss;
    gsEnd_.assign(G, nullptr);
    for (int g = 0; g < G; g++) hipCheck(hipEventCreateWithFlags(&gsEnd_[g], hipEventDisableTiming), "group event");
    if (!gsStart_) hipCheck(hipEventCreateWithFlags(&gsStart_, hipEventDisableTiming), "group event");
    return true;
}

void Learner::CollectGrouped(int G) {
    const int T = exp_.T, P = exp_.P, W = exp_.W;
    const rlgpu_rollout_view& v = exp_.v;
    const uint8_t* old = OldRows();
    const int Na = cfg_.num_arenas / G, Pg = 4 * Na;
    if (envTiming_) EnsureEvents((size_t)2 * T * G);
    hipCheck(hipEventRecord(gsStart_, s_), "group start");
    for (int g = 0; g < G; g++) hipCheck(hipStreamWaitEvent(gs_[g], gsStart_, 0), "group wait");
    rlgpu_ppo* ph = ppo_->handle();
    rlgpu_envset* eh = env_->handle();
    for (int t = 0; t < T; t++) {
        const size_t r = (size_t)t * P;
        for (int g = 0; g < G; g++) {
            const size_t p0 = (size_t)g * Pg, a = r + p0;
            RlgpuCheck(rlgpu_ppo_infer_actions_rows(ph, v.obs + a * W, v.masks + a * ACT, Pg, (int64_t)p0,
                                                    cfg_.deterministic != 0, (uint64_t)stats.rng_step,
                                                    old ? old + p0 : nullptr, v.actions + a, v.logp + a, gs_[g]),
                       "InferActions (group)");
            rlgpu_step_outputs o{v.obs + (a + P) * OBS, v.masks + (a + P) * ACT, v.rewards + a, v.terms + a,
                                 v.trunc_obs + a * OBS};
            if (envTiming_) hipCheck(hipEventRecord(ev_[2 * ((size_t)t * G + g)], gs_[g]), "event");
            RlgpuCheck(rlgpu_envset_step_range(eh, g * Na, Na, v.actions + a, 1, &o, gs_[g]), "EnvSet step (group)");
            if (envTiming_) hipCheck(hipEventRecord(ev_[2 * ((size_t)t * G + g) + 1], gs_[g]), "event");
        }
        stats.rng_step++;
    }
    for (int g = 0; g < G; g++) {
        hipCheck(hipEventRecord(gsEnd_[g], gs_[g]), "group end");
        hipCheck(hipStreamWaitEvent(s_, gsEnd_[g], 0), "group join");
    }
}

void Learner::Collect() {
    if (trajMode()) {
        CollectTrajectories();
        return;
    }
    if (const int G = CollectGroups(); G > 1 && EnsureGroupStreams(G)) {
        collectGroupsUsed_ = G;
        CollectGrouped(G);
        return;
    }
    collectGroupsUsed_ = 1;
    const int T = exp_.T, P = exp_.P, W = exp_.W;
    const rlgpu_rollout_view& v = exp_.v;
    if (envTiming_) EnsureEvents((size_t)2 * T);
    for (int t = 0; t < T; t++) {
        const size_t r = (size_t)t * P;
        ActAndStep(r, r + P, v.trunc_obs + r * OBS, v.trunc_obs + r * W, envTiming_ ? &ev_[2 * t] : nullptr);
    }
}

void Learner::ActAndStep(size_t row, size_t next, float* trunc, float* truncStacked, hipEvent_t* timing) {
    const int P = exp_.P, W = exp_.W;
    const rlgpu_rollout_view& v = exp_.v;
    const rlgpu_envset_buffers& st = env_->state();
    ppo_->InferActions(v.obs + row * W, v.masks + row * ACT, P, cfg_.deterministic != 0, (uint64_t)stats.rng_step,
                       v.actions + row, v.logp + row, OldRows());
    stats.rng_step++;
    rlgpu_step_outputs o{K_ > 1 ? nullptr : v.obs + next * OBS, v.masks + next * ACT, v.rewards + row, v.terms + row,
                         K_ > 1 ? nullptr : trunc};
    if (timing) hipCheck(hipEventRecord(timing[0], s_), "event");
    StepEnv(v.actions + row, o);
    if (timing) hipCheck(hipEventRecord(timing[1], s_), "event");
    if (K_ > 1) lk::stack_frames(st.obs, st.trunc_obs, v.terms + row, hist_, K_, P, OBS, v.obs + next * W, truncStacked, s_);
}

void Learner::EnsureEvents(size_t count) {
    if (ev_.size() >= count) return;
    for (auto e : ev_) (void)hipEventDestroy(e);
    ev_.assign(count, nullptr);
    for (auto& e : ev_) hipCheck(hipEventCreate(&e), "event");
}

void Learner::StepEnv(const int32_t* d_actions, const rlgpu_step_outputs& o) {
    if (!hook_) {
        env_->Step(d_actions, &o);
        return;
    }
    rlgpu_envset* e = env_->handle();
    const rlgpu_envset_buffers& st = env_->state();
    const int P = st.num_players;
    rlgpu_step_outputs pre{nullptr, nullptr, nullptr, o.terminals, nullptr};
    RlgpuCheck(rlgpu_envset_step(e, d_actions, 0, &pre, s_), "EnvSet step (hooked)");
    hipCheck(hipStreamSynchronize(s_), "sync");
    if (hook_(hookUser_, RLGPU_HOOK_AFTER_STEP) != 0)
        throw rlgpu::Error(RLGPU_ERR_STATE, std::string("Learner: step hook failed: ") + rlgpu_last_error());
    lk::host_step_finish(st.terminals, o.terminals, st.rewards, o.rewards, st.obs, st.trunc_obs, o.trunc_obs, P, OBS, s_);
    RlgpuCheck(rlgpu_envset_reset(e, s_), "EnvSet reset (hooked)");
    hipCheck(hipStreamSynchronize(s_), "sync");
    if (hook_(hookUser_, RLGPU_HOOK_AFTER_RESET) != 0)
        throw rlgpu::Error(RLGPU_ERR_STATE, std::string("Learner: step hook failed: ") + rlgpu_last_error());
    if (o.obs) hipCheck(hipMemcpyAsync(o.obs, st.obs, (size_t)P * OBS * 4, hipMemcpyDeviceToDevice, s_), "obs append");
    if (o.masks) hipCheck(hipMemcpyAsync(o.masks, st.action_masks, (size_t)P * ACT, hipMemcpyDeviceToDevice, s_), "mask append");
}

void Learner::Consume() {
    if (trajMode()) {
        ConsumeTrajectories();
        return;
    }
    const int T = exp_.T, P = exp_.P;
    const int64_t TP = (int64_t)T * P;
    const rlgpu_rollout_view& v = exp_.v;
    ppo_->InferCritic(v.obs, TP + P, v.values);
    lk::select_trunc(v.terms, TP, selScratch_, selBytes_, truncRows_, truncCount_, s_);
    int32_t ntr = 0;
    hipCheck(hipMemcpyAsync(&ntr, truncCount_, sizeof(int32_t), hipMemcpyDeviceToHost, s_), "trunc count");
    hipCheck(hipStreamSynchronize(s_), "sync");
    if (ntr > 0) {
        if (ntr > truncCap_) {
            if (truncObsC_) (void)hipFree(truncObsC_);
            if (truncValC_) (void)hipFree(truncValC_);
            truncCap_ = std::max<int64_t>(ntr, 2 * truncCap_);
            hipCheck(hipMalloc((void**)&truncObsC_, (size_t)truncCap_ * exp_.W * 4), "trunc obs");
            hipCheck(hipMalloc((void**)&truncValC_, (size_t)truncCap_ * 4), "trunc vals");
        }
        lk::gather_rows(v.trunc_obs, exp_.W, truncRows_, ntr, truncObsC_, s_);
// ... 221 lines not shown
        const int64_t need = std::max(J.nrec, J.ntrunc) + P;
        if (J.rp.cap < need) {
            for (auto* a : {&J.rp, &J.rstart, &J.rlen, &J.rcode, &J.rtidx}) a->Reserve(2 * need, s_, true);
            J.roff.Reserve(2 * need, s_, true);
        }
        J.truncObs.Reserve((J.ntrunc + P) * (int64_t)W, s_, true);
        const int r = (int)(J.step % Tm), rn = (int)((J.step + 1) % Tm);
        const size_t row = (size_t)r * P;
        ActAndStep(row, (size_t)rn * P, nullptr, J.truncStage, nullptr);
        lk::traj_step(v.terms + row, r, Tm, track, P, J.start, J.len, J.Records(), J.counters, J.trnew, s_);
        lk::traj_trunc_copy(K_ > 1 ? J.truncStage : st.trunc_obs, W, J.counters, J.trnew, J.truncObs.p, s_);
        J.step++;
        J.steps++;
        hipCheck(hipMemcpyAsync(J.hcounters, J.counters, lk::kTcCount * sizeof(int64_t), hipMemcpyDeviceToHost, s_),
                 "traj counters");
        hipCheck(hipStreamSynchronize(s_), "sync");
        J.nrec = J.hcounters[lk::kTcRecs];
        J.ntrunc = J.hcounters[lk::kTcTruncs];
        J.nrows = J.hcounters[lk::kTcSteps];
        if (J.nrows >= J.tsPerItr) break;
        if (J.steps + J.maxLen + 2 >= Tm) break;
    }
}

void Learner::ConsumeTrajectories() {
    TrajectoryStore& J = traj;
    const int P = exp_.P, W = exp_.W;
    const rlgpu_rollout_view& v = exp_.v;
    const int64_t M = J.nrows, K = J.nrec, ntr = J.ntrunc;
    J.cObs.Reserve(std::max<int64_t>(M, 1) * W, s_);
    J.cMasks.Reserve(std::max<int64_t>(M, 1) * ACT, s_);
    for (auto* a : {&J.cLogp, &J.cRews, &J.cVals, &J.cAdv, &J.cTarget, &J.cRet}) a->Reserve(std::max<int64_t>(M, 1), s_);
    J.cActs.Reserve(std::max<int64_t>(M, 1), s_);
    J.cTerms.Reserve(std::max<int64_t>(M, 1), s_);
    J.truncVals.Reserve(std::max<int64_t>(ntr, 1), s_);
    if (M == 0) {
        if (hasColl_ && cfg_.return_samples > 0) FeedReturnStat(J.cRet.p, {}, 0);
        return;
    }
    lk::traj_gather(J.Records(), K, J.Tmax, P, W, ACT, v.obs, v.masks, v.actions, v.logp, v.rewards, v.terms, J.cObs.p,
                    J.cMasks.p, J.cActs.p, J.cLogp.p, J.cRews.p, J.cTerms.p, s_);
    ppo_->InferCritic(J.cObs.p, M, J.cVals.p);
    if (ntr > 0) ppo_->InferCritic(J.truncObs.p, ntr, J.truncVals.p);
    const float std_ = (float)returnStat.GetSTD();
    hipCheck(hipMemsetAsync(clipSums_, 0, 2 * sizeof(float), s_), "clip sums");
    RlgpuCheck(rlgpu_gae_segments(J.cRews.p, J.cTerms.p, J.cVals.p, ntr > 0 ? J.truncVals.p : nullptr, J.roff.p, J.rlen.p,
                                  J.rtidx.p, K, cfg_.gamma, cfg_.gae_lambda, std_, cfg_.reward_clip_range, J.cAdv.p,
                                  J.cTarget.p, J.cRet.p, clipSums_, s_),
               "GAE");
    const int k = cfg_.return_samples;
    if (k <= 0) return;
    const int32_t m = (int32_t)std::min<int64_t>(k, M);
    std::vector<int64_t> idx((size_t)std::max(m, 1));
    if (m > 0) RlgpuCheck(rlgpu_sample_indices(cfg_.seed, cfg_.rank, stats.iteration, M, m, idx.data()), "return samples");
    FeedReturnStat(J.cRet.p, idx, m);
}

rlgpu_learner_report Learner::Iterate() {
    rlgpu_learner_report r{};
    auto t0 = clk::now();
    Collect();
    auto t0i = clk::now();
    hipCheck(hipStreamSynchronize(s_), "sync");
    auto t1 = clk::now();
    r.collect_issue_s = secs(t0, t0i);
    Consume();
    hipCheck(hipStreamSynchronize(s_), "sync");
    auto t2 = clk::now();
    Learn();
    FinishIteration();
    auto t2i = clk::now();
    hipCheck(hipStreamSynchronize(s_), "sync");
    auto t3 = clk::now();
    r.learn_issue_s = secs(t2, t2i);
    r.collect_s = secs(t0, t1);
    r.consume_s = secs(t1, t2);
    r.learn_s = secs(t2, t3);
    r.env_steps = (int64_t)(trajMode() ? traj.steps : exp_.T) * cfg_.num_arenas;
    r.env_launch_arenas = cfg_.num_arenas / std::max(1, collectGroupsUsed_);
    if (envTiming_ && !ev_.empty()) {
        double ms = 0;
        const int nt = trajMode() ? 0 : exp_.T * std::max(1, collectGroupsUsed_);
        std::vector<float> each(nt);
        for (int t = 0; t < nt; t++) {
            float x = 0;
            hipCheck(hipEventElapsedTime(&x, ev_[2 * t], ev_[2 * t + 1]), "elapsed");
            ms += x;
            each[t] = x;
        }
        r.env_kernel_ms = nt ? ms / nt : 0.0;
        if (nt) {
            std::sort(each.begin(), each.end());
            r.env_kernel_min_ms = each.front();
            r.env_kernel_max_ms = each.back();
            r.env_kernel_median_ms = (nt & 1) ? each[nt / 2] : 0.5 * ((double)each[nt / 2 - 1] + each[nt / 2]);
        }
    }
    return r;
}

void Learner::Start(int64_t iterations) {
    for (int64_t i = 0; i < iterations; i++) Iterate();
}

}

struct rlgpu_learner {
    GGL::Learner* L = nullptr;
};

extern "C" int rlgpu_learner_default_config(rlgpu_learner_config* c) {
    return rlgpu::guarded([&] {
        RLGPU_REQUIRE(c, "null config");
        std::memset(c, 0, sizeof(*c));
        c->num_arenas = 4096;
        c->tick_skip = 8;
        c->action_delay = 7;
        c->seed = 123;
        c->max_episode_duration = 300.f;
        c->rollout_len = 128;
        c->epochs = 2;
        c->mini_batch_size = 50000;
        c->batch_size = 0;
        c->overbatching = 1;
        c->gamma = 0.99f;
        c->gae_lambda = 0.95f;
        c->clip_range = 0.2f;
        c->entropy_scale = 0.035f;
        c->policy_lr = 2.5e-4f;
        c->critic_lr = 2.5e-4f;
        c->reward_clip_range = 200.f;
        c->return_samples = 150;
        c->policy_layers[0] = c->policy_layers[1] = 512;
        c->n_policy_layers = 2;
        c->critic_layers[0] = c->critic_layers[1] = 512;
        c->n_critic_layers = 2;
        c->train_gemm = RLGPU_GEMM_F16X3;
        c->rank = 0;
        c->world = 1;
        c->policy_temperature = 1.0f;
        c->mask_entropy = 0;
    });
}

extern "C" int32_t rlgpu_learner_config_size(void) { return (int32_t)sizeof(rlgpu_learner_config); }

extern "C" int rlgpu_learner_create(const rlgpu_learner_config* cfg, const rlgpu_collective* coll, void* stream,
                                    rlgpu_learner** out) {
    return rlgpu::guarded([&] {
        RLGPU_REQUIRE(cfg && out, "rlgpu_learner_create: null argument");
        auto* h = new rlgpu_learner();
        try {
            h->L = new GGL::Learner(*cfg, coll, rlgpu::as_stream(stream));
        } catch (...) {
            delete h;
            throw;
        }
        *out = h;
    });
}

extern "C" int rlgpu_learner_destroy(rlgpu_learner* h) {
    return rlgpu::guarded([&] {
        if (!h) return;
        delete h->L;
        delete h;
    });
}

// ... 232 lines not shown
```

### reinforcement-learning_amd/host/learner.hpp

```cpp
#pragma once
#include <hip/hip_runtime.h>

#include <cstdint>
#include <stdexcept>
#include <string>
#include <utility>
#include <vector>

#include "../../include/rlgpu_env.h"
#include "../../include/rlgpu_gae.h"
#include "../../include/rlgpu_learner.h"
#include "../../include/rlgpu_ppo.h"

namespace RLGC {

inline void RlgpuCheck(int st, const char* what) {
    if (st != RLGPU_OK) throw std::runtime_error(std::string(what) + ": " + rlgpu_last_error());
}

class EnvSetGPU {
public:
    EnvSetGPU(const rlgpu_envset_config& cfg, hipStream_t stream);
    ~EnvSetGPU();
    EnvSetGPU(const EnvSetGPU&) = delete;
// ... 93 lines not shown
    int64_t minibatches = 0;

    rlgpu_ppo* handle() const { return h_; }
    float* grads() const { return grads_; }
    int64_t num_params() const { return nparams_; }
    float* adv_stats() const { return adv_stats_; }
    float* metrics() const { return metrics_; }

private:
    rlgpu_ppo* h_ = nullptr;
    hipStream_t stream_;
    float* grads_ = nullptr;
    int64_t nparams_ = 0;
    float* adv_stats_ = nullptr;
    float* metrics_ = nullptr;
};

class Learner {
public:
    Learner(const rlgpu_learner_config& cfg, const rlgpu_collective* coll, hipStream_t stream);
    ~Learner();
    Learner(const Learner&) = delete;
    Learner& operator=(const Learner&) = delete;

    void Collect();
    void Consume();
    void Learn();
    void FinishIteration();
    rlgpu_learner_report Iterate();
    void Start(int64_t iterations);

    void SetOldTeam(int team) { oldTeam_ = team; }
    void SetGradHook(rlgpu_grad_hook_fn fn, void* user) {
        gradHook_ = fn;
        gradHookUser_ = user;
    }
    void SetStepHook(rlgpu_step_hook_fn fn, void* user) {
        hook_ = fn;
        hookUser_ = user;
    }
    void SetEnvTiming(bool on) { envTiming_ = on; }

    const rlgpu_learner_config& config() const { return cfg_; }
    RLGC::EnvSetGPU& env() { return *env_; }
    PPOLearnerGPU& ppo() { return *ppo_; }
    ExperienceBuffer& exp() { return exp_; }
    rlgpu_learner_stats stats;
    WelfordStat returnStat;

private:
    void StepEnv(const int32_t* d_actions, const rlgpu_step_outputs& o);
    void ActAndStep(size_t row, size_t next, float* trunc, float* truncStacked, hipEvent_t* timing);
    void EnsureEvents(size_t count);
    void AllReduceGrads(int epoch, int batch);
    void BatchAdvantageStats(const float* d_adv, const int32_t* d_idx, int64_t n);
    void CollectTrajectories();
    void ConsumeTrajectories();
    void FeedReturnStat(const float* d_ret, const std::vector<int64_t>& idx, int32_t m);
    bool trajMode() const { return cfg_.experience_mode == RLGPU_EXP_TRAJECTORIES; }
    hipStream_t s_;
    rlgpu_learner_config cfg_;
    rlgpu_collective coll_{};
    bool hasColl_ = false;
    RLGC::EnvSetGPU* env_ = nullptr;
    PPOLearnerGPU* ppo_ = nullptr;
    ExperienceBuffer exp_;
    int oldTeam_ = -1;
    bool envTiming_ = false;
    rlgpu_step_hook_fn hook_ = nullptr;
    void* hookUser_ = nullptr;
    rlgpu_grad_hook_fn gradHook_ = nullptr;
    void* gradHookUser_ = nullptr;
    int K_ = 1;
    float* hist_ = nullptr;
    std::vector<hipEvent_t> ev_;
    std::vector<hipStream_t> gs_;
    std::vector<hipEvent_t> gsEnd_;
    hipEvent_t gsStart_ = nullptr;
    int gsRefused_ = 0;
    int CollectGroups() const;
    bool EnsureGroupStreams(int G);
    int collectGroupsUsed_ = 1;
    void CollectGrouped(int G);
    uint8_t* oldRows_[2] = {nullptr, nullptr};
    const uint8_t* OldRows() const { return oldTeam_ >= 0 ? oldRows_[oldTeam_] : nullptr; }
    int32_t* trainRows_ = nullptr;
    int32_t* perm_ = nullptr;
    int32_t* permRows_ = nullptr;
    float* badv_ = nullptr;
    int64_t permCap_ = 0;
    void NeedLearnRows(int64_t n, const char* what) const;
    void ReserveLearnRows(int64_t M);
    int32_t* truncRows_ = nullptr;
    int32_t* truncCount_ = nullptr;
    void* selScratch_ = nullptr;
    size_t selBytes_ = 0;
    float* truncObsC_ = nullptr;
    float* truncValC_ = nullptr;
    int64_t truncCap_ = 0;
    int64_t* sampleIdx_ = nullptr;
    float* samples_ = nullptr;
    int32_t* ends_ = nullptr;
    std::vector<int32_t> hostEnds_;
    double* mom_ = nullptr;
    float* clipSums_ = nullptr;
  public:
    TrajectoryStore traj;
  private:
    std::vector<void*> allocs_;
    template <class T>
    T* Alloc(size_t count);
    void Release(void* p);
};

}
```

### reinforcement-learning_amd/rlgpu/learner.py

```python
import ctypes
import time

import numpy as np

from . import _lib
from .ppo import MAX_LAYERS, NUM_METRICS

OBS, ACTIONS = 167, 90


def _host_lib():
    L = _lib.lib()
    i64p, f64p = ctypes.POINTER(ctypes.c_int64), ctypes.POINTER(ctypes.c_double)
    L.rlgpu_batch_ranges.argtypes = [ctypes.c_int64, ctypes.c_int64, ctypes.c_int32, ctypes.c_void_p, ctypes.c_int64]
    L.rlgpu_batch_ranges.restype = ctypes.c_int64
    L.rlgpu_welford_add.argtypes = [i64p, f64p, f64p, ctypes.c_void_p, ctypes.c_int64]
    L.rlgpu_welford_std.argtypes = [ctypes.c_int64, ctypes.c_double]
    L.rlgpu_welford_std.restype = ctypes.c_double
    L.rlgpu_sample_indices.argtypes = [ctypes.c_uint64, ctypes.c_int32, ctypes.c_int64, ctypes.c_int64, ctypes.c_int32,
                                       ctypes.c_void_p]
    L.rlgpu_sample_finished_rows.argtypes = [ctypes.c_uint64, ctypes.c_int32, ctypes.c_int64, ctypes.c_void_p,
                                             ctypes.c_int32, ctypes.c_int32, ctypes.c_void_p,
                                             ctypes.POINTER(ctypes.c_int32)]
    return L
# ... 346 lines not shown
        self.old_version, self.old_team = None, 0
        self.skill = None
        if cfg.skill_tracker is not None and cfg.skill_tracker.enabled and rank == 0:
            from .skill import SkillTracker
            self.skill = SkillTracker(cfg.skill_tracker, self.ppo, self.device, cfg.tick_skip, cfg.action_delay,
                                      seed=cfg.seed, mesh=cfg.mesh, arith=cfg.arith)
        if cfg.train_against_old_versions or self.skill is not None:
            import os
            from .versions import PolicyVersionManager
            vf = os.path.join(cfg.checkpoint_folder, "policy_versions") if cfg.checkpoint_folder else None
            self.versions = PolicyVersionManager(self.ppo, vf, cfg.max_old_versions, cfg.ts_per_version, self.skill)
        self.last_checkpoint = None
        if cfg.checkpoint_folder:
            from . import checkpoint as _ckpt
            err = None
            if rank == 0:
                try:
                    self.last_checkpoint = _ckpt.load(self, cfg.checkpoint_folder)
                    if self.versions is not None:
                        self.versions.load_versions(self.total_steps)
                except Exception as e:
                    err = e
            if world > 1:
                sync_from_rank0(self, group, err)
            elif err is not None:
                raise err

    def close(self):
        if getattr(self, "_h", None):
            import torch
            torch.cuda.synchronize(self.device)
            if self.skill is not None:
                self.skill.close()
            self.env.close()
            self.ppo.close()
            _lib.check(_lib.lib().rlgpu_learner_destroy(self._h), "rlgpu_learner_destroy")
            self._h = None

    def __del__(self):
        try:
            self.close()
        except Exception:
            pass

    def _stats(self):
        st = _CStats()
        _lib.check(_lib.lib().rlgpu_learner_get_stats(self._h, ctypes.byref(st)), "rlgpu_learner_get_stats")
        return st

    def _set_stats(self, st):
        _lib.check(_lib.lib().rlgpu_learner_set_stats(self._h, ctypes.byref(st)), "rlgpu_learner_set_stats")

    def _set_stat(self, name, v):
        st = self._stats()
        setattr(st, name, int(v))
        self._set_stats(st)

    total_steps = property(lambda self: self._stats().total_steps, lambda self, v: self._set_stat("total_steps", v))
    iteration = property(lambda self: self._stats().iteration, lambda self, v: self._set_stat("iteration", v))

    def _metrics(self, reset):
        out = np.zeros(NUM_METRICS, np.float32)
        cnt = ctypes.c_int64()
        _lib.check(_lib.lib().rlgpu_learner_metrics(self._h, out.ctypes.data, ctypes.byref(cnt), int(reset)),
                   "rlgpu_learner_metrics")
        return out.tolist(), cnt.value

    def step_metrics(self, reset=True):
        import numpy as np
        from .env import EnvSet
        tot, cnt = np.zeros(8, np.float64), np.zeros(8, np.uint64)
        _lib.check(_lib.lib().rlgpu_learner_step_metrics(self._h, tot.ctypes.data, cnt.ctypes.data, int(reset)),
                   "rlgpu_learner_step_metrics")
        return {k: float(t) / int(c) for k, t, c in zip(EnvSet.step_metric_names(), tot, cnt) if c}

    _HOOK = ctypes.CFUNCTYPE(ctypes.c_int, ctypes.c_void_p, ctypes.c_int32)
    _GRAD_HOOK = ctypes.CFUNCTYPE(ctypes.c_int, ctypes.c_void_p, ctypes.c_void_p, ctypes.c_int64, ctypes.c_int32,
                                  ctypes.c_int32)

    def set_step_hook(self, fn):
        L = _lib.lib()
        if fn is None:
            self._hook = None
            _lib.check(L.rlgpu_learner_set_step_hook(self._h, None, None), "rlgpu_learner_set_step_hook")
            return

        def thunk(_user, phase):
            try:
                fn(int(phase))
                return 0
            except Exception:
                import traceback
                traceback.print_exc()
                return 1
        self._hook = self._HOOK(thunk)
        L.rlgpu_learner_set_step_hook.argtypes = [ctypes.c_void_p, self._HOOK, ctypes.c_void_p]
        _lib.check(L.rlgpu_learner_set_step_hook(self._h, self._hook, None), "rlgpu_learner_set_step_hook")

    def set_grad_hook(self, fn):
        import torch
        from ._lib import alias
        L = _lib.lib()
        if fn is None:
            self._ghook = None
            _lib.check(L.rlgpu_learner_set_grad_hook(self._h, None, None), "rlgpu_learner_set_grad_hook")
            return

        def thunk(_user, ptr, n, epoch, batch):
            try:
                fn(alias(ptr, (n,), torch.float32, self.device), int(epoch), int(batch))
                return 0
            except Exception:
                import traceback
                traceback.print_exc()
                return 1
        self._ghook = self._GRAD_HOOK(thunk)
        L.rlgpu_learner_set_grad_hook.argtypes = [ctypes.c_void_p, self._GRAD_HOOK, ctypes.c_void_p]
        _lib.check(L.rlgpu_learner_set_grad_hook(self._h, self._ghook, None), "rlgpu_learner_set_grad_hook")

    def set_env_timing(self, on=True):
        _lib.check(_lib.lib().rlgpu_learner_set_env_timing(self._h, int(on)), "rlgpu_learner_set_env_timing")

    def save(self):
        from . import checkpoint as _ckpt
        if not self.cfg.checkpoint_folder:
            raise ValueError("Learner.save: cfg.checkpoint_folder is not set")
        if self.rank == 0:
            self.last_checkpoint = _ckpt.save(self, self.cfg.checkpoint_folder, self.cfg.checkpoints_to_keep)
            if self.versions is not None:
                self.versions.save_versions()
        return self.last_checkpoint

    def collect(self):
        _lib.check(_lib.lib().rlgpu_learner_collect(self._h), "rlgpu_learner_collect")

    def consume(self):
        _lib.check(_lib.lib().rlgpu_learner_consume(self._h), "rlgpu_learner_consume")

    def learn(self):
        _lib.check(_lib.lib().rlgpu_learner_learn(self._h), "rlgpu_learner_learn")

    def batch(self):
        import torch
        b = _CBatch()
        _lib.check(_lib.lib().rlgpu_learner_batch(self._h, ctypes.byref(b)), "rlgpu_learner_batch")
        d, M, K, nt, W = self.device, max(b.num_rows, 1), max(b.num_segments, 1), max(b.num_truncs, 1), self.W

        def a(ptr, shape, dtype, dev):
            return _lib.alias(ptr, shape, dtype, dev) if ptr else torch.empty((0,) + tuple(shape[1:]), dtype=dtype, device=dev)
        f32, i32 = torch.float32, torch.int32
        out = {"obs": a(b.obs, (M, W), f32, d), "masks": a(b.masks, (M, ACTIONS), torch.uint8, d),
               "actions": a(b.actions, (M,), i32, d), "logp": a(b.logp, (M,), f32, d),
               "rewards": a(b.rewards, (M,), f32, d), "terms": a(b.terms, (M,), torch.int8, d),
               "values": a(b.values, (M,), f32, d), "adv": a(b.adv, (M,), f32, d), "target": a(b.target, (M,), f32, d),
               "ret": a(b.ret, (M,), f32, d), "trunc_obs": a(b.trunc_obs, (nt, W), f32, d),
               "trunc_vals": a(b.trunc_vals, (nt,), f32, d)}
        for k in ("seg_player", "seg_start", "seg_len", "seg_code", "seg_tidx"):
            out[k] = a(getattr(b, k), (K,), i32, d)[:b.num_segments]
        out["seg_off"] = a(b.seg_off, (K,), torch.int64, d)[:b.num_segments]
        for k in ("obs", "masks", "actions", "logp", "rewards", "terms", "values", "adv", "target", "ret"):
            out[k] = out[k][:b.num_rows]
        out["trunc_obs"], out["trunc_vals"] = out["trunc_obs"][:b.num_truncs], out["trunc_vals"][:b.num_truncs]
        out.update(num_rows=b.num_rows, num_truncs=b.num_truncs, num_segments=b.num_segments, store_rows=b.store_rows,
                   steps=b.steps, first_step=b.first_step)
        return out

    def finish_iteration(self):
# ... 32 lines not shown
```

### reinforcement-learning_amd/rlgpu/ppo.py

```python
import ctypes
import math

from . import _lib
from ._lib import alias

MAX_LAYERS = 8
NUM_METRICS = 16
METRICS = ("entropy", "kl", "policy_loss", "critic_loss", "ratio", "clip_fraction", "count",
           "grad_norm_policy", "grad_norm_critic", "grad_norm_shared")
MODEL_NAMES = ("policy", "critic", "shared_head")


class _Cfg(ctypes.Structure):
    _fields_ = [("obs_size", ctypes.c_int32), ("num_actions", ctypes.c_int32),
                ("policy_layers", ctypes.c_int32 * MAX_LAYERS), ("n_policy_layers", ctypes.c_int32),
                ("critic_layers", ctypes.c_int32 * MAX_LAYERS), ("n_critic_layers", ctypes.c_int32),
                ("layer_norm", ctypes.c_int32), ("leaky_slope", ctypes.c_float), ("activation", ctypes.c_int32),
                ("policy_lr", ctypes.c_float), ("critic_lr", ctypes.c_float),
                ("beta1", ctypes.c_float), ("beta2", ctypes.c_float), ("eps", ctypes.c_float),
                ("weight_decay", ctypes.c_float), ("clip_range", ctypes.c_float),
                ("entropy_scale", ctypes.c_float), ("max_grad_norm", ctypes.c_float),
                ("max_rows", ctypes.c_int32), ("seed", ctypes.c_uint64), ("train_gemm", ctypes.c_int32),
                ("infer_fp16", ctypes.c_int32), ("shared_layers", ctypes.c_int32 * MAX_LAYERS),
                ("n_shared_layers", ctypes.c_int32), ("sample_row_offset", ctypes.c_int64),
                ("policy_temperature", ctypes.c_float), ("mask_entropy", ctypes.c_int32)]

GEMM_F32X6, GEMM_F32, GEMM_F16X3 = 0, 1, 2
ACTIVATIONS = {"leaky_relu": 0, "relu": 1, "sigmoid": 2, "tanh": 3}


def activation_id(name):
    if name not in ACTIVATIONS:
        raise ValueError(f"activation must be one of {sorted(ACTIVATIONS)}, not {name!r}")
    return ACTIVATIONS[name]


_bound = False


def _bind():
    global _bound
    L = _lib.lib()
    if _bound:
        return L
    vp, i32, i64, u64, f32 = ctypes.c_void_p, ctypes.c_int32, ctypes.c_int64, ctypes.c_uint64, ctypes.c_float
    L.rlgpu_ppo_create.argtypes = [ctypes.POINTER(_Cfg), ctypes.POINTER(vp)]
    L.rlgpu_ppo_destroy.argtypes = [vp]
    L.rlgpu_ppo_config_size.restype = i32
    L.rlgpu_ppo_buffers.argtypes = [vp, ctypes.POINTER(vp), ctypes.POINTER(vp), ctypes.POINTER(i64)]
    L.rlgpu_ppo_model_range.argtypes = [vp, i32, ctypes.POINTER(i64), ctypes.POINTER(i64)]
    L.rlgpu_ppo_init_params.argtypes = [vp, u64, vp]
    L.rlgpu_ppo_refresh_half.argtypes = [vp, vp]
    L.rlgpu_ppo_forward.argtypes = [vp, i32, i32, vp, i32, vp, vp]
    L.rlgpu_ppo_infer_actions.argtypes = [vp, vp, vp, i32, i32, u64, vp, vp, vp]
    L.rlgpu_ppo_infer_critic.argtypes = [vp, vp, i64, vp, vp]
    L.rlgpu_mean_std.argtypes = [vp, i64, vp, vp]
    L.rlgpu_ppo_minibatch.argtypes = [vp, vp, vp, vp, vp, vp, vp, vp, i64, i32, i64, vp, vp, vp]
    L.rlgpu_ppo_optimizer_step.argtypes = [vp, vp, vp]
    L.rlgpu_ppo_zero_grad.argtypes = [vp, vp]
    L.rlgpu_ppo_optimizer_state.argtypes = [vp, ctypes.POINTER(i64), ctypes.POINTER(vp), ctypes.POINTER(vp)]
    L.rlgpu_ppo_set_optimizer_step.argtypes = [vp, i64]
    L.rlgpu_ppo_set_version.argtypes = [vp, vp, vp]
    L.rlgpu_ppo_infer_actions_mixed.argtypes = [vp, vp, vp, i32, i32, u64, vp, vp, vp, vp]
    L.rlgpu_permutation.argtypes = [i64, u64, u64, vp, vp]
    L.rlgpu_kernel_timing.argtypes = [i32]
    L.rlgpu_kernel_timing_read.argtypes = [vp, vp, vp, i32]
    _ = f32
    _bound = True
    return L


def param_count(obs_size, num_actions, layers, out=None, layer_norm=True):
    n, prev = 0, obs_size
    for h in layers:
        n += prev * h + h + (2 * h if layer_norm else 0)
        prev = h
    o = num_actions if out is None else out
    return n + prev * o + o


class PPO:

    def __init__(self, obs_size=167, num_actions=90, policy_layers=(512, 512), critic_layers=(512, 512),
                 layer_norm=True, policy_lr=2.5e-4, critic_lr=2.5e-4, clip_range=0.2, entropy_scale=0.035,
                 max_grad_norm=0.5, max_rows=50_000, seed=42, init=True, device="cuda:0",
                 betas=(0.9, 0.999), eps=1e-8, weight_decay=1e-2, leaky_slope=0.01, train_gemm=GEMM_F16X3,
                 infer_fp16=False, shared_layers=(), policy_temperature=1.0, mask_entropy=False, activation="leaky_relu"):
        import torch
        if not torch.cuda.is_available():
            raise _lib.RLGPUError("PPO needs an MI355X: the product path has no CPU fallback")
        L = _bind()
        self.device = torch.device(device)
        torch.cuda.set_device(self.device)
        c = _Cfg()
        c.obs_size, c.num_actions = obs_size, num_actions
        c.n_policy_layers, c.n_critic_layers = len(policy_layers), len(critic_layers)
        for i, v in enumerate(policy_layers):
            c.policy_layers[i] = v
        for i, v in enumerate(critic_layers):
            c.critic_layers[i] = v
        c.n_shared_layers = len(shared_layers)
        for i, v in enumerate(shared_layers):
            c.shared_layers[i] = v
        c.layer_norm, c.leaky_slope, c.activation = int(layer_norm), leaky_slope, activation_id(activation)
        self.leaky_slope, self.activation = leaky_slope, activation
        c.policy_lr, c.critic_lr = policy_lr, critic_lr
        c.beta1, c.beta2, c.eps, c.weight_decay = betas[0], betas[1], eps, weight_decay
        c.clip_range, c.entropy_scale, c.max_grad_norm = clip_range, entropy_scale, max_grad_norm
        c.max_rows, c.seed = max_rows, seed
        c.train_gemm = train_gemm
        c.infer_fp16 = int(infer_fp16)
        c.policy_temperature, c.mask_entropy = policy_temperature, int(mask_entropy)
        h = ctypes.c_void_p()
        _lib.check(L.rlgpu_ppo_create(ctypes.byref(c), ctypes.byref(h)), "rlgpu_ppo_create")
        self._h = h
        self.cfg = c
        self.optim_options = {"lr": (policy_lr, critic_lr, min(policy_lr, critic_lr)), "betas": tuple(betas), "eps": eps,
                              "weight_decay": weight_decay}
        self.obs_size, self.num_actions = obs_size, num_actions
        self.policy_layers, self.critic_layers, self.layer_norm = tuple(policy_layers), tuple(critic_layers), layer_norm
        self.shared_layers = tuple(shared_layers)
        self.max_rows = max_rows
        p, g, n = ctypes.c_void_p(), ctypes.c_void_p(), ctypes.c_int64()
        _lib.check(L.rlgpu_ppo_buffers(h, ctypes.byref(p), ctypes.byref(g), ctypes.byref(n)), "rlgpu_ppo_buffers")
        self.num_params = n.value
        self.params = alias(p.value, (n.value,), torch.float32, self.device)
        self.grads = alias(g.value, (n.value,), torch.float32, self.device)
        self.metrics = torch.zeros(NUM_METRICS, device=self.device)
        self.adv_stats = torch.zeros(2, device=self.device)
        if init:
            self.init_params(seed)

    @classmethod
    def wrap(cls, handle, device, policy_layers, critic_layers, max_rows, obs_size=167, num_actions=90,
             layer_norm=True, leaky_slope=0.01, metrics_source=None, owner=None, shared_layers=(), optim_options=None,
             activation="leaky_relu"):
        import torch
        L = _bind()
        self = cls.__new__(cls)
        self._h, self._owned, self._owner = ctypes.c_void_p(handle), False, owner
        self.device = torch.device(device)
        self.obs_size, self.num_actions = obs_size, num_actions
        self.policy_layers, self.critic_layers, self.layer_norm = tuple(policy_layers), tuple(critic_layers), layer_norm
        self.shared_layers = tuple(shared_layers)
        self.leaky_slope, self.max_rows = leaky_slope, max_rows
        activation_id(activation)
# ... 40 lines not shown

    def flat(self, grads=False):
        import torch
        return torch.cat([self.model_slice(m, grads) for m in self.models])

    def policy_version(self):
        import torch
        return torch.cat([self.model_slice(m) for m in self.models if m != 1])

    def model_in(self, model):
        return self.shared_layers[-1] if (self.shared_layers and model != 2) else self.obs_size

    def model_out(self, model):
        return (self.num_actions, 1, self.shared_layers[-1] if self.shared_layers else 0)[model]

    def init_params(self, seed):
        _lib.check(_lib.lib().rlgpu_ppo_init_params(self._h, seed, _lib.stream_ptr()), "init_params")

    def refresh_half(self):
        _lib.check(_lib.lib().rlgpu_ppo_refresh_half(self._h, _lib.stream_ptr()), "refresh_half")

    def torch_module(self, model):
        import torch
        layers = (self.policy_layers, self.critic_layers, self.shared_layers)[model]
        out = None if model == 2 else self.model_out(model)
        seq = make_sequential(self.model_in(model), out, layers, self.layer_norm, self.leaky_slope, self.activation)
        flat = self.model_slice(model).detach().cpu()
        o = 0
        with torch.no_grad():
            for prm in seq.parameters():
                prm.copy_(flat[o:o + prm.numel()].view_as(prm))
                o += prm.numel()
        return seq

    def torch_chain(self, model):
        import torch
        mods = list(self.torch_module(2)) if (self.shared_layers and model != 2) else []
        return torch.nn.Sequential(*(mods + list(self.torch_module(model))))

    def load_torch_module(self, model, seq):
        import torch
        flat = torch.cat([p.detach().reshape(-1).float() for p in seq.parameters()])
        dst = self.model_slice(model)
        assert flat.numel() == dst.numel(), "architecture mismatch"
        dst.copy_(flat.to(self.device))
        self.refresh_half()

    def forward(self, model, x, half=False, out=None):
        import torch
        n = x.shape[0]
        width = self.model_out(model)
        out = torch.empty((n, width), device=self.device) if out is None else out
        _lib.check(_lib.lib().rlgpu_ppo_forward(self._h, model, int(half), _lib.ptr(x.contiguous()), n, _lib.ptr(out),
                                                _lib.stream_ptr()), "rlgpu_ppo_forward")
        return out

    def infer_actions(self, obs, masks, step=0, deterministic=False, actions=None, logp=None):
        import torch
        n = obs.shape[0]
        actions = torch.empty(n, dtype=torch.int32, device=self.device) if actions is None else actions
        logp = torch.empty(n, device=self.device) if logp is None else logp
        _lib.check(_lib.lib().rlgpu_ppo_infer_actions(self._h, _lib.ptr(obs), _lib.ptr(masks), n, int(deterministic),
                                                      step, _lib.ptr(actions), _lib.ptr(logp), _lib.stream_ptr()),
                   "rlgpu_ppo_infer_actions")
        return actions, logp

    def set_version(self, policy_params):
        cnt = sum(self.model_range(m)[1] for m in self.models if m != 1)
        if policy_params.numel() != cnt:
            raise _lib.RLGPUError("policy version has the wrong parameter count")
        _lib.check(_lib.lib().rlgpu_ppo_set_version(self._h, _lib.ptr(policy_params.contiguous()), _lib.stream_ptr()),
                   "rlgpu_ppo_set_version")

    def infer_actions_mixed(self, obs, masks, old_rows, step=0, deterministic=False, actions=None, logp=None):
        import torch
        n = obs.shape[0]
        actions = torch.empty(n, dtype=torch.int32, device=self.device) if actions is None else actions
        logp = torch.empty(n, device=self.device) if logp is None else logp
        _lib.check(_lib.lib().rlgpu_ppo_infer_actions_mixed(self._h, _lib.ptr(obs), _lib.ptr(masks), n, int(deterministic),
                                                            step, _lib.ptr(old_rows), _lib.ptr(actions), _lib.ptr(logp),
                                                            _lib.stream_ptr()), "rlgpu_ppo_infer_actions_mixed")
        return actions, logp

    def infer_critic(self, obs, out=None):
        import torch
        n = obs.shape[0]
        out = torch.empty(n, device=self.device) if out is None else out
        _lib.check(_lib.lib().rlgpu_ppo_infer_critic(self._h, _lib.ptr(obs), n, _lib.ptr(out), _lib.stream_ptr()),
                   "rlgpu_ppo_infer_critic")
        return out

    def adv_normalizer(self, adv):
        _lib.check(_lib.lib().rlgpu_mean_std(_lib.ptr(adv), adv.numel(), _lib.ptr(self.adv_stats), _lib.stream_ptr()),
                   "rlgpu_mean_std")
        return self.adv_stats

    def minibatch(self, obs, masks, actions, old_logp, adv, target, index, start, n, batch_size):
        _lib.check(_lib.lib().rlgpu_ppo_minibatch(
            self._h, _lib.ptr(obs), _lib.ptr(masks), _lib.ptr(actions), _lib.ptr(old_logp), _lib.ptr(adv),
            _lib.ptr(target), _lib.ptr(index), start, n, batch_size, _lib.ptr(self.adv_stats), _lib.ptr(self.metrics),
            _lib.stream_ptr()), "rlgpu_ppo_minibatch")
        self._count += 1

    _count = 0

    def optimizer_step(self):
        _lib.check(_lib.lib().rlgpu_ppo_optimizer_step(self._h, _lib.ptr(self.metrics), _lib.stream_ptr()),
                   "rlgpu_ppo_optimizer_step")

    def zero_grad(self):
        _lib.check(_lib.lib().rlgpu_ppo_zero_grad(self._h, _lib.stream_ptr()), "zero_grad")

    def read_metrics(self, reset=True):
        if self._metrics_source is not None:
            m, cnt = self._metrics_source(reset)
            cnt = max(cnt, 1)
            return {"Policy Entropy": m[0] / cnt, "Mean KL Divergence": m[1] / cnt, "Policy Loss": m[2] / cnt,
                    "Critic Loss": m[3] / cnt, "Ratio": m[4] / cnt, "SB3 Clip Fraction": m[5] / cnt,
                    "Policy Grad Norm": m[7], "Critic Grad Norm": m[8], "Shared Head Grad Norm": m[9]}
        m = self.metrics.cpu().tolist()
        cnt = max(self._count, 1)
        rep = {"Policy Entropy": m[0] / cnt, "Mean KL Divergence": m[1] / cnt, "Policy Loss": m[2] / cnt,
               "Critic Loss": m[3] / cnt, "Ratio": m[4] / cnt, "SB3 Clip Fraction": m[5] / cnt,
               "Policy Grad Norm": m[7], "Critic Grad Norm": m[8], "Shared Head Grad Norm": m[9]}
        if reset:
            self.metrics.zero_()
            self._count = 0
        return rep

    def optimizer_state(self):
        import torch
        step, m, v = ctypes.c_int64(), ctypes.c_void_p(), ctypes.c_void_p()
        _lib.check(_lib.lib().rlgpu_ppo_optimizer_state(self._h, ctypes.byref(step), ctypes.byref(m), ctypes.byref(v)),
                   "optimizer_state")
        return (step.value, alias(m.value, (self.num_params,), torch.float32, self.device),
                alias(v.value, (self.num_params,), torch.float32, self.device))

    def set_optimizer_step(self, step):
        _lib.check(_lib.lib().rlgpu_ppo_set_optimizer_step(self._h, int(step)), "set_optimizer_step")

    def model_sizes(self, model):
        return [p.numel() for p in self.torch_module(model).parameters()]


def make_sequential(obs_size, out, layers, layer_norm=True, leaky_slope=0.01, activation="leaky_relu"):
    import torch
    act = (lambda: torch.nn.LeakyReLU(leaky_slope), torch.nn.ReLU, torch.nn.Sigmoid, torch.nn.Tanh)[activation_id(activation)]
    mods, prev = [], obs_size
    for hdim in layers:
        mods.append(torch.nn.Linear(prev, hdim))
        if layer_norm:
            mods.append(torch.nn.LayerNorm(hdim))
        mods.append(act())
        prev = hdim
    if out is not None:
        mods.append(torch.nn.Linear(prev, out))
    return torch.nn.Sequential(*mods)


KERNEL_TIMING_SLOTS = ("forward / input-gradient GEMMs", "weight-gradient GEMMs", "LayerNorm forward",
                       "LayerNorm backward")


def kernel_timing(enable):
    _bind()
    _lib.check(_lib.lib().rlgpu_kernel_timing(1 if enable else 0), "rlgpu_kernel_timing")
# ... 23 lines not shown
```

Baseline: 2.032 million.

## Fuse rollout collection into one persistent env-step plus policy-inference kernel

Adds a collection-loop kernel that, for the whole rollout of T steps, runs the env step and a one-wave MLP policy inference inside a single launch per arena group. It replaces per-step kernel launches and separate inference kernels with one long-running kernel. The intent is to remove launch overhead and the global-memory round trips between env stepping and action sampling. In exchange it only applies under narrow conditions (msvc_x64 arithmetic, action delay, no profiling, eligible policy). It also uses coarser timing, and correctness depends on the in-kernel sync between step and inference.

```diff
diff --git a/include/rlgpu_env.h b/include/rlgpu_env.h
--- a/include/rlgpu_env.h
+++ b/include/rlgpu_env.h
@@ -202,6 +202,19 @@
                       const rlgpu_step_outputs* out, void* stream);
 int rlgpu_envset_step_range(rlgpu_envset* env, int32_t first, int32_t count, const int32_t* d_actions,
                             int32_t reset_terminated, const rlgpu_step_outputs* out, void* stream);
+typedef struct {
+    float* obs;
+    uint8_t* masks;
+    int32_t* actions;
+    float* logp;
+    float* rewards;
+    int8_t* terminals;
+    float* trunc_obs;
+} rlgpu_collect_rollout;
+struct rlgpu_ppo;
+int rlgpu_envset_collect_loop_ok(rlgpu_envset* env, struct rlgpu_ppo* policy);
+int rlgpu_envset_collect_loop(rlgpu_envset* env, struct rlgpu_ppo* policy, int32_t steps, const rlgpu_collect_rollout* rollout,
+                              int32_t deterministic, uint64_t rng_step, void* stream);
 int rlgpu_envset_sync(rlgpu_envset* env, void* stream);
 int rlgpu_envset_set_output_only(rlgpu_envset* env, int32_t enable);
 
diff --git a/include/rlgpu_ppo.h b/include/rlgpu_ppo.h
--- a/include/rlgpu_ppo.h
+++ b/include/rlgpu_ppo.h
@@ -75,6 +75,11 @@
                                  int32_t deterministic, uint64_t rng_step, const uint8_t* d_old_rows,
                                  int32_t* d_actions, float* d_logp, void* stream);
 int rlgpu_ppo_fused_infer(rlgpu_ppo* h, int32_t model);
+int rlgpu_ppo_wave_infer(rlgpu_ppo* h, int32_t model);
+int rlgpu_ppo_infer_actions_wave(rlgpu_ppo* h, const float* d_obs, const uint8_t* d_masks, int32_t n, int64_t row0,
+                                 int32_t deterministic, uint64_t rng_step, const uint8_t* d_old_rows,
+                                 int32_t* d_actions, float* d_logp, void* stream);
+int rlgpu_ppo_infer_values_wave(rlgpu_ppo* h, int32_t model, const float* d_obs, int32_t n, float* d_out, void* stream);
 int rlgpu_ppo_infer_critic(rlgpu_ppo* h, const float* d_obs, int64_t n, float* d_values, void* stream);
 
 int rlgpu_mean_std(const float* d_x, int64_t n, float* d_out, void* stream);
diff --git a/reinforcement-learning_amd/csrc/common.hpp b/reinforcement-learning_amd/csrc/common.hpp
--- a/reinforcement-learning_amd/csrc/common.hpp
+++ b/reinforcement-learning_amd/csrc/common.hpp
@@ -51,5 +51,13 @@
 inline unsigned ceil_div(int64_t a, int64_t b) { return (unsigned)((a + b - 1) / b); }
 
 void launch_mlp_infer_act(int act, bool f16, unsigned blocks, hipStream_t s, const void* args, size_t bytes);
+void launch_mlp_infer_wave(bool f16, unsigned blocks, hipStream_t s, const void* args, size_t bytes);
 
 }
+
+struct rlgpu_ppo;
+namespace rlgpu {
+bool ppo_wave_policy(rlgpu_ppo* h, int obs_size, int num_actions);
+void ppo_wave_args(rlgpu_ppo* h, const float* d_obs, const uint8_t* d_masks, int64_t n, int deterministic, uint64_t rng_step,
+                   int32_t* d_actions, float* d_logp, void* blob, size_t cap, bool* f16);
+}
diff --git a/reinforcement-learning_amd/csrc/env.hip b/reinforcement-learning_amd/csrc/env.hip
--- a/reinforcement-learning_amd/csrc/env.hip
+++ b/reinforcement-learning_amd/csrc/env.hip
@@ -9,6 +9,7 @@
 #include "env_step.hpp"
 #include "mesh.hpp"
 #include "../../include/rlgpu_gamestate.h"
+#include "../../include/rlgpu_ppo.h"
 
 namespace rl {
 void env_k0_upload(const EnvConst& k, const RsqrtLut* lut);
@@ -17,6 +18,8 @@
 void env_k0_launch(const StepArgs& g, int blocks, hipStream_t s);
 void env_k1_launch(const StepArgs& g, int blocks, hipStream_t s);
 void env_k2_launch(const StepArgs& g, int blocks, hipStream_t s);
+void env_collect_k0_upload(const EnvConst& k, const RsqrtLut* lut);
+void env_collect_k0_launch(const CollectArgs& c, bool f16, int blocks, hipStream_t s);
 
 static m3 host_euler_ypr(float yaw, float pitch, float roll) {
     float ci = std::cos(roll), cj = std::cos(pitch), ch = std::cos(yaw);
@@ -364,6 +367,7 @@
     for (int a = 0; a < RLGPU_NUM_ARITH; a++) {
         const bool lut = rsqrt && rl::sse_api(a);
         if (consts || lut) kEnvKernel[a].upload(k, lut ? &L : nullptr);
+        if ((consts || lut) && a == RLGPU_ARITH_MSVC_X64) rl::env_collect_k0_upload(k, lut ? &L : nullptr);
     }
     done.consts = true;
     done.rsqrt = done.rsqrt || rsqrt;
@@ -381,7 +385,7 @@
 };
 Range whole(const rlgpu_envset* e) { return Range{0, e->cfg.num_arenas}; }
 
-void launch(rlgpu_envset* e, rl::StepArgs g, Range r, hipStream_t s) {
+rl::StepArgs placed(rlgpu_envset* e, rl::StepArgs g, Range r) {
     const size_t a0 = (size_t)r.first, p0 = a0 * 4, nr = (size_t)e->plug.nr;
     g.arenas = e->d_arenas + a0 * rl::kRec;
     g.n = r.count;
@@ -408,7 +412,10 @@
         g.metrics = e->d_metrics + a0 * RLGPU_STEP_METRIC_SLOTS;
         g.metrics_players = e->metric_players;
     }
-    kEnvKernel[e->cfg.arith].launch(g, rlgpu::ceil_div(r.count, rl::kArenas), s);
+    return g;
+}
+void launch(rlgpu_envset* e, const rl::StepArgs& g, Range r, hipStream_t s) {
+    kEnvKernel[e->cfg.arith].launch(placed(e, g, r), rlgpu::ceil_div(r.count, rl::kArenas), s);
     RLGPU_CHECK_HIP(hipGetLastError());
 }
 
@@ -731,6 +738,40 @@
     });
 }
 
+extern "C" int rlgpu_envset_collect_loop_ok(rlgpu_envset* e, rlgpu_ppo* policy) {
+    return e && policy && e->cfg.arith == RLGPU_ARITH_MSVC_X64 && e->cfg.action_delay > 0 && !e->d_prof &&
+           rlgpu::ppo_wave_policy(policy, RLGPU_OBS, RLGPU_ACTIONS);
+}
+
+extern "C" int rlgpu_envset_collect_loop(rlgpu_envset* e, rlgpu_ppo* policy, int32_t steps, const rlgpu_collect_rollout* ro,
+                                         int32_t deterministic, uint64_t rng_step, void* stream) {
+    return rlgpu::guarded([&] {
+        RLGPU_REQUIRE(e && policy && ro && steps > 0, "rlgpu_envset_collect_loop: bad argument");
+        RLGPU_REQUIRE(ro->obs && ro->masks && ro->actions && ro->logp && ro->rewards && ro->terminals,
+                      "rlgpu_envset_collect_loop: null rollout array");
+        if (!rlgpu_envset_collect_loop_ok(e, policy))
+            throw rlgpu::Error(RLGPU_ERR_UNSUPPORTED, "rlgpu_envset_collect_loop: not eligible (msvc_x64 arithmetic, no "
+                                                      "profile, a policy on the one-wave inference kernel)");
+        const int64_t P = e->num_players;
+        const rlgpu_step_outputs out{ro->obs + P * RLGPU_OBS, ro->masks + P * RLGPU_ACTIONS, ro->rewards, ro->terminals,
+                                     ro->trunc_obs};
+        rl::CollectArgs c;
+        std::memset(&c, 0, sizeof c);
+        c.metric_calls = (int)(e->metric_calls % 4);
+        c.g = placed(e, fused_step_args(e, ro->actions, 1, &out), whole(e));
+        if (c.g.metrics) {
+            e->metric_calls += (uint64_t)(steps - 1);
+            e->metric_players = e->metric_calls % 4 == 0;
+        }
+        c.T = steps;
+        c.P = P;
+        bool f16 = false;
+        rlgpu::ppo_wave_args(policy, ro->obs, ro->masks, P, deterministic, rng_step, ro->actions, ro->logp, c.inf.b,
+                             sizeof c.inf.b, &f16);
+        rl::env_collect_k0_launch(c, f16, rlgpu::ceil_div(e->cfg.num_arenas, rl::kArenas), rlgpu::as_stream(stream));
+    });
+}
+
 extern "C" int rlgpu_envset_set_output_only(rlgpu_envset* e, int32_t enable) {
     return rlgpu::guarded([&] {
         RLGPU_REQUIRE(e, "null envset");
diff --git a/reinforcement-learning_amd/csrc/env_collect_k0.hip b/reinforcement-learning_amd/csrc/env_collect_k0.hip
--- /dev/null
+++ b/reinforcement-learning_amd/csrc/env_collect_k0.hip
@@ -0,0 +1,30 @@
+#define RLGPU_ENV_ARITH 0
+#define RLGPU_ENV_COLLECT_KERNEL env_collect_a0
+#include <hip/hip_bf16.h>
+#include <hip/hip_fp16.h>
+#include <hip/hip_runtime.h>
+#include <math.h>
+#include <stdint.h>
+
+#include <cstdlib>
+
+#include "../../include/rlgpu_detmath.h"
+#include "common.hpp"
+#pragma clang fp contract(fast)
+namespace {
+#include "infer_kernels.hpp"
+}
+#pragma clang fp contract(off)
+#include "env_step.hpp"
+
+namespace rl {
+void env_collect_k0_upload(const EnvConst& k, const RsqrtLut* lut) {
+    RLGPU_CHECK_HIP(hipMemcpyToSymbol(HIP_SYMBOL(C), &k, sizeof k));
+    if (lut) RLGPU_CHECK_HIP(hipMemcpyToSymbol(HIP_SYMBOL(kRsqrtLut), lut, sizeof *lut));
+}
+void env_collect_k0_launch(const CollectArgs& c, bool f16, int blocks, hipStream_t s) {
+    if (f16) hipLaunchKernelGGL(env_collect_a0<true>, dim3(blocks), dim3(kWG), 0, s, c);
+    else hipLaunchKernelGGL(env_collect_a0<false>, dim3(blocks), dim3(kWG), 0, s, c);
+    RLGPU_CHECK_HIP(hipGetLastError());
+}
+}
diff --git a/reinforcement-learning_amd/csrc/env_step.hpp b/reinforcement-learning_amd/csrc/env_step.hpp
--- a/reinforcement-learning_amd/csrc/env_step.hpp
+++ b/reinforcement-learning_amd/csrc/env_step.hpp
@@ -46,7 +46,18 @@
     int pen_slots;
 };
 
-#ifdef RLGPU_ENV_KERNEL
+struct InferBlob {
+    alignas(8) unsigned char b[512];
+};
+struct CollectArgs {
+    StepArgs g;
+    int T;
+    int metric_calls;
+    int64_t P;
+    InferBlob inf;
+};
+
+#if defined(RLGPU_ENV_KERNEL) || defined(RLGPU_ENV_COLLECT_KERNEL)
 
 DEV void step_metrics(ArenaLDS* A, int l, double* m, bool players) {
     if (players) {
@@ -380,234 +391,47 @@
     }
 }
 
+#ifdef RLGPU_ENV_KERNEL
 __global__ void __launch_bounds__(kWG) RLGPU_ENV_KERNEL(StepArgs g) {
     __shared__ ArenaLDS lds[kArenas];
-    const int team = threadIdx.x >> 4, l = threadIdx.x & 15;
-    const int arena = blockIdx.x * kArenas + team;
-    const bool valid = arena < g.n;
-    ArenaLDS* A = &lds[team];
-    Prof P{g.prof, g.prof ? (long long)clock64() : 0};
-    {
-        int first = blockIdx.x * kArenas;
-        int cnt = g.n - first < kArenas ? g.n - first : kArenas;
-        const int chunks = kRec / 16;
-        for (int k = threadIdx.x; k < cnt * chunks; k += kWG) {
-            int a = k / chunks, c = k % chunks;
-            const uint4* src = (const uint4*)(g.arenas + (size_t)(first + a) * kRec) + c;
-            uint4* dst = (uint4*)&lds[a] + c;
-            *dst = *src;
-        }
-    }
-    sync(); P.mark(11);
-    if (valid && l < 5) {
-        A->a.force[l] = zero3();
-        A->a.torque[l] = zero3();
-        update_inertia(A, l);
-    }
-    if (l == 0) {
-        A->a.epa_lock = A->a.npen = 0;
-        A->a.arith = g.arith;
-    }
-    if (threadIdx.x == 0) g_pen_save.cap = g.pen_slots;
-    sync(); P.mark(11);
-    if (g.ticks_first > 0) {
-        if (valid && l == 0) {
-            rlgpu_env_extra& e = A->s.env;
-            for (int i = 0; i < 3; i++) e.prev_ball_vel[i] = A->s.ball.vel[i] * kBT2UU;
-            for (int i = 0; i < 4; i++) {
-                e.prev_boost[i] = A->s.cars[i].boost;
-                e.prev_is_flipping[i] = A->s.cars[i].is_flipping;
-                e.prev_on_ground[i] = A->s.cars[i].is_on_ground;
-                e.ev_bump[i] = e.ev_bumped[i] = e.ev_demo[i] = e.ev_demoed[i] = 0;
-            }
-            e.has_prev = 1;
-        }
-        sync(); P.mark(11);
-    }
-    {
-        PadRegs pregs;
-        load_pad_regs(pregs, l);
-        const int t1 = g.ticks_first, t2 = g.actions ? g.ticks_second : 0;
-        for (int t = 0;; t++) {
-            if (g.actions && t == t1) {
-                if (valid && l < 4) {
-                    int a = g.actions[arena * 4 + l];
-                    a = a < 0 ? 0 : (a > RLGPU_ACTIONS - 1 ? RLGPU_ACTIONS - 1 : a);
-                    const float* x = C.action[a];
-                    float* c = A->s.cars[l].controls;
-                    for (int k = 0; k < 5; k++) c[k] = x[k];
-                    c[5] = x[5] == 1 ? 1.f : 0.f;
-                    c[6] = x[6] == 1 ? 1.f : 0.f;
-                    c[7] = x[7] == 1 ? 1.f : 0.f;
-                    for (int k = 0; k < 8; k++) A->s.env.prev_action[l][k] = x[k];
-                }
-                sync(); P.mark(11);
-            }
-            if (t >= t1 + t2) break;
-            tick(A, g.mesh, l, valid, g.seed, arena + g.arena_offset, P, pregs, stdmin(kArenas, g.n - (int)blockIdx.x * kArenas));
-        }
-    }
-    uint8_t term = 0;
-    if (g.build) {
-        if (valid && l == 0) {
-            rlgpu_env_extra& e = A->s.env;
-            int64_t cur = e.tick_count;
-            int64_t tick_skip = cur - e.last_tick_count > 0 ? cur - e.last_tick_count : 0;
-            float delta_time = (int)tick_skip * (1.0f / 120.0f);
-            bool any = false;
-            for (int i = 0; i < 4; i++) {
-                const rlgpu_car& c = A->s.cars[i];
-                bool t = c.ball_hit_valid && (uint64_t)c.ball_hit_tick >= (uint64_t)(cur - tick_skip);
-                A->a.touched[i] = t;
-                any |= t;
-            }
-            float by = A->s.ball.pos[1] * kBT2UU;
-            bool goal = fabsf(by) > (5124.25f + 91.25f);
-            A->a.goal = goal;
-            if (any) e.no_touch_time = 0;
-            else e.no_touch_time += delta_time;
-            if (goal) {
-                if (by > 0) e.score_blue++;
-                else e.score_orange++;
-            }
-            uint8_t tt = 0;
-            for (int k = 0; k < g.plug->nt; k++) {
-                const rlgpu_terminal_spec& tc = g.plug->tc[k];
-                bool hit = false, trunc = false;
-                if (tc.type == RLGPU_TC_NO_TOUCH) {
-                    hit = !any && e.no_touch_time >= tc.param;
-                    trunc = true;
-                } else if (tc.type == RLGPU_TC_SCORE_LIMIT) {
-                    const int lim = (int)tc.param;
-                    hit = (e.score_blue >= lim) || (e.score_orange >= lim);
-                } else if (tc.type == RLGPU_TC_GOAL_SCORE) {
-                    hit = goal;
-                }
-                if (hit) {
-                    const uint8_t cur = trunc ? 2 : 1;
-                    if (tt == 0 || cur == 1) tt = cur;
-                }
-            }
-            e.terminal = tt;
-            if (goal) {
-                if (by > 0) e.penalty_blue++;
-                else e.penalty_orange++;
-            }
-            e.episode_steps++;
-            uint8_t tj = tt;
-            if (!tj && g.max_episode_steps > 0 && e.episode_steps >= g.max_episode_steps) tj = 2;
-            if (tj) e.episode_steps = 0;
-            A->a.traj_term = tj;
-        }
-        sync(); P.mark(12);
-        if (valid) {
-            const int pi = l & 3, q = l >> 2;
-            const PView me = view_player(A, pi);
-            v3 bp = ld3(A->s.ball.pos) * kBT2UU, bv = ld3(A->s.ball.vel) * kBT2UU, pbv = ld3(A->s.env.prev_ball_vel);
-            const int nr = g.plug->nr;
-            constexpr int kPer = (RLGPU_MAX_REWARDS + 3) / 4;
-            float ov[kPer];
-#pragma unroll
-            for (int k = 0; k < kPer; k++) ov[k] = 0.f;
-#pragma unroll 1
-            for (int k = 0; q + 4 * k < nr; k++) {
-                const int r = q + 4 * k;
-                const float o = reward_value(A, g.plug->rw[r], pi, me, bp, bv, pbv, A->a.goal != 0);
-#pragma unroll
-                for (int j = 0; j < kPer; j++) ov[j] = j == k ? o : ov[j];
-                if (pi == 0 && g.last_rewards) g.last_rewards[(size_t)arena * nr + r] = o;
-                if (g.reward_values) g.reward_values[((size_t)arena * 4 + pi) * nr + r] = o;
-            }
-            float all = 0.f;
-            const int base = (int)(threadIdx.x & ~15u) + pi;
-#pragma unroll
-            for (int r = 0; r < RLGPU_MAX_REWARDS; r++) {
-                if (r >= nr) break;
-                const float o = __shfl(ov[r >> 2], base + 4 * (r & 3));
-                all += o * g.plug->rw[r].weight;
-            }
-            if (l < 4) A->a.all_rewards[l] = all;
-        }
-        sync(); P.mark(12);
-        if (valid && l < 4) {
-            float r = A->a.all_rewards[l];
-            g.rewards[arena * 4 + l] = r;
-            if (g.out_rew) g.out_rew[arena * 4 + l] = r;
-            if (g.out_term) g.out_term[arena * 4 + l] = (int8_t)A->a.traj_term;
-        }
-        if (g.metrics && valid && l < 4) step_metrics(A, l, g.metrics + (size_t)arena * RLGPU_STEP_METRIC_SLOTS,
-                                                      g.metrics_players != 0);
-        uint8_t tj = 0;
-        if (valid) {
-            term = A->s.env.terminal;
-            tj = (uint8_t)A->a.traj_term;
-        }
-        sync(); P.mark(12);
-        if (valid && l == 0) {
-            g.terminals[arena] = term;
-            A->s.env.last_tick_count = A->s.env.tick_count;
-        }
-        const bool fused_reset = g.reset_mode == kResetTerminated && valid && term != 0;
-        if (valid) build_obs_rows(A, l);
-        sync(); P.mark(13);
-        if (valid) {
-            copy_rows(A, l, arena, g.obs, g.masks);
-            if (!fused_reset) copy_rows(A, l, arena, g.out_obs, g.out_masks);
-            if (tj == 2) {
-                copy_rows(A, l, arena, g.trunc_obs, nullptr);
-                copy_rows(A, l, arena, g.out_trunc, nullptr);
-            }
-        }
-        sync(); P.mark(13);
-        if (g.reset_mode == kResetTerminated) {
-            if (fused_reset && l == 0) kickoff_reset(A, g.seed, arena + g.arena_offset, g.fuzz != 0);
-            sync(); P.mark(14);
-            if (fused_reset) build_obs_rows(A, l);
-            sync(); P.mark(14);
-            if (fused_reset) {
-                copy_rows(A, l, arena, g.obs, g.masks);
-                copy_rows(A, l, arena, g.out_obs, g.out_masks);
-            }
-            sync(); P.mark(14);
-        }
-    }
-    if (g.reset_mode >= kResetSet) {
-        bool do_reset = false;
-        if (valid) {
-            if (g.reset_mode == kResetSet) do_reset = g.terminals[arena] != 0;
-            else if (g.reset_mode == kResetMask) do_reset = g.reset_mask ? g.reset_mask[arena] != 0 : true;
-            else if (g.reset_mode == kResetAll) do_reset = true;
-        }
-        sync(); P.mark(14);
-        if (do_reset && l == 0) {
-            kickoff_reset(A, g.seed, arena + g.arena_offset, g.fuzz != 0);
-            if (g.reset_mode == kResetSet) g.terminals[arena] = 0;
-        }
-        sync(); P.mark(14);
-        bool rebuild = do_reset || (valid && g.reset_mode == kRebuildObs);
-        if (rebuild) build_obs_rows(A, l);
-        sync(); P.mark(14);
-        if (rebuild) copy_rows(A, l, arena, g.obs, g.masks);
-        sync(); P.mark(14);
-    }
-    {
-        int first = blockIdx.x * kArenas;
-        int cnt = g.n - first < kArenas ? g.n - first : kArenas;
-        const int chunks = kRec / 16;
-        for (int k = threadIdx.x; k < cnt * chunks; k += kWG) {
-            int a = k / chunks, c = k % chunks;
-            uint4* dst = (uint4*)(g.arenas + (size_t)(first + a) * kRec) + c;
-            const uint4* src = (const uint4*)&lds[a] + c;
-            *dst = *src;
-        }
-    }
-    P.mark(15);
-    if (g.prof && valid && l == 0 && A->a.npen) {
-        atomicAdd(&g.prof[28], (unsigned long long)A->a.npen);
-        atomicAdd(&g.prof[kProfWG + (size_t)blockIdx.x * kProfPhases + 23], (unsigned long long)A->a.npen);
-        atomicAdd(&g.prof[kProfWG + (size_t)gridDim.x * kProfPhases + arena], (unsigned long long)A->a.npen);
-    }
+#include "env_step_body.inc"
 }
 #endif
 
-}
+#ifdef RLGPU_ENV_COLLECT_KERNEL
+template <bool F16>
+__global__ void __launch_bounds__(kWG) RLGPU_ENV_COLLECT_KERNEL(CollectArgs c) {
+    __shared__ ArenaLDS lds[kArenas];
+    static_assert(sizeof(infer::WaveLDS) <= sizeof(ArenaLDS) * kArenas, "the inference buffers fit the arena staging area");
+    static_assert(sizeof(infer::InferArgs) <= sizeof(c.inf) && alignof(infer::InferArgs) <= alignof(InferBlob), "InferBlob");
+    static_assert(infer::WR == 4 * kArenas, "a workgroup's players are one wave's rows");
+    const infer::InferArgs& a = *reinterpret_cast<const infer::InferArgs*>(c.inf.b);
+    infer::WaveLDS& S = *reinterpret_cast<infer::WaveLDS*>(lds);
+    const int64_t P = c.P, r0 = (int64_t)blockIdx.x * infer::WR;
+    const int rows = (int)(P - r0 < infer::WR ? P - r0 : infer::WR), A = a.width[a.nl];
+    for (int t = 0; t < c.T; t++) {
+        const int64_t row = (int64_t)t * P + r0;
+        infer::wave_infer<F16, mlp::ACT_LEAKY>(a, S, a.X + row * a.in, a.masks + row * A, rows, a.row0 + r0, a.step + t,
+                                                a.row_sel ? a.row_sel + r0 : nullptr, a.act + row, a.logp ? a.logp + row : nullptr,
+                                                nullptr, (int)threadIdx.x);
+        sync();
+        StepArgs s = c.g;
+        const int64_t tp = (int64_t)t * P;
+        s.actions = c.g.actions + tp;
+        if (s.out_obs) s.out_obs = c.g.out_obs + tp * RLGPU_OBS;
+        if (s.out_masks) s.out_masks = c.g.out_masks + tp * RLGPU_ACTIONS;
+        if (s.out_rew) s.out_rew = c.g.out_rew + tp;
+        if (s.out_term) s.out_term = c.g.out_term + tp;
+        if (s.out_trunc) s.out_trunc = c.g.out_trunc + tp * RLGPU_OBS;
+        if (s.metrics) s.metrics_players = (c.metric_calls + t + 1) % 4 == 0;
+        {
+            const StepArgs& g = s;
+#include "env_step_body.inc"
+        }
+        sync();
+    }
+}
+#endif
+#endif
+
+}
diff --git a/reinforcement-learning_amd/csrc/env_step_body.inc b/reinforcement-learning_amd/csrc/env_step_body.inc
--- /dev/null
+++ b/reinforcement-learning_amd/csrc/env_step_body.inc
@@ -0,0 +1,225 @@
+    const int team = threadIdx.x >> 4, l = threadIdx.x & 15;
+    const int arena = blockIdx.x * kArenas + team;
+    const bool valid = arena < g.n;
+    ArenaLDS* A = &lds[team];
+    Prof P{g.prof, g.prof ? (long long)clock64() : 0};
+    {
+        int first = blockIdx.x * kArenas;
+        int cnt = g.n - first < kArenas ? g.n - first : kArenas;
+        const int chunks = kRec / 16;
+        for (int k = threadIdx.x; k < cnt * chunks; k += kWG) {
+            int a = k / chunks, c = k % chunks;
+            const uint4* src = (const uint4*)(g.arenas + (size_t)(first + a) * kRec) + c;
+            uint4* dst = (uint4*)&lds[a] + c;
+            *dst = *src;
+        }
+    }
+    sync(); P.mark(11);
+    if (valid && l < 5) {
+        A->a.force[l] = zero3();
+        A->a.torque[l] = zero3();
+        update_inertia(A, l);
+    }
+    if (l == 0) {
+        A->a.epa_lock = A->a.npen = 0;
+        A->a.arith = g.arith;
+    }
+    if (threadIdx.x == 0) g_pen_save.cap = g.pen_slots;
+    sync(); P.mark(11);
+    if (g.ticks_first > 0) {
+        if (valid && l == 0) {
+            rlgpu_env_extra& e = A->s.env;
+            for (int i = 0; i < 3; i++) e.prev_ball_vel[i] = A->s.ball.vel[i] * kBT2UU;
+            for (int i = 0; i < 4; i++) {
+                e.prev_boost[i] = A->s.cars[i].boost;
+                e.prev_is_flipping[i] = A->s.cars[i].is_flipping;
+                e.prev_on_ground[i] = A->s.cars[i].is_on_ground;
+                e.ev_bump[i] = e.ev_bumped[i] = e.ev_demo[i] = e.ev_demoed[i] = 0;
+            }
+            e.has_prev = 1;
+        }
+        sync(); P.mark(11);
+    }
+    {
+        PadRegs pregs;
+        load_pad_regs(pregs, l);
+        const int t1 = g.ticks_first, t2 = g.actions ? g.ticks_second : 0;
+        for (int t = 0;; t++) {
+            if (g.actions && t == t1) {
+                if (valid && l < 4) {
+                    int a = g.actions[arena * 4 + l];
+                    a = a < 0 ? 0 : (a > RLGPU_ACTIONS - 1 ? RLGPU_ACTIONS - 1 : a);
+                    const float* x = C.action[a];
+                    float* c = A->s.cars[l].controls;
+                    for (int k = 0; k < 5; k++) c[k] = x[k];
+                    c[5] = x[5] == 1 ? 1.f : 0.f;
+                    c[6] = x[6] == 1 ? 1.f : 0.f;
+                    c[7] = x[7] == 1 ? 1.f : 0.f;
+                    for (int k = 0; k < 8; k++) A->s.env.prev_action[l][k] = x[k];
+                }
+                sync(); P.mark(11);
+            }
+            if (t >= t1 + t2) break;
+            tick(A, g.mesh, l, valid, g.seed, arena + g.arena_offset, P, pregs, stdmin(kArenas, g.n - (int)blockIdx.x * kArenas));
+        }
+    }
+    uint8_t term = 0;
+    if (g.build) {
+        if (valid && l == 0) {
+            rlgpu_env_extra& e = A->s.env;
+            int64_t cur = e.tick_count;
+            int64_t tick_skip = cur - e.last_tick_count > 0 ? cur - e.last_tick_count : 0;
+            float delta_time = (int)tick_skip * (1.0f / 120.0f);
+            bool any = false;
+            for (int i = 0; i < 4; i++) {
+                const rlgpu_car& c = A->s.cars[i];
+                bool t = c.ball_hit_valid && (uint64_t)c.ball_hit_tick >= (uint64_t)(cur - tick_skip);
+                A->a.touched[i] = t;
+                any |= t;
+            }
+            float by = A->s.ball.pos[1] * kBT2UU;
+            bool goal = fabsf(by) > (5124.25f + 91.25f);
+            A->a.goal = goal;
+            if (any) e.no_touch_time = 0;
+            else e.no_touch_time += delta_time;
+            if (goal) {
+                if (by > 0) e.score_blue++;
+                else e.score_orange++;
+            }
+            uint8_t tt = 0;
+            for (int k = 0; k < g.plug->nt; k++) {
+                const rlgpu_terminal_spec& tc = g.plug->tc[k];
+                bool hit = false, trunc = false;
+                if (tc.type == RLGPU_TC_NO_TOUCH) {
+                    hit = !any && e.no_touch_time >= tc.param;
+                    trunc = true;
+                } else if (tc.type == RLGPU_TC_SCORE_LIMIT) {
+                    const int lim = (int)tc.param;
+                    hit = (e.score_blue >= lim) || (e.score_orange >= lim);
+                } else if (tc.type == RLGPU_TC_GOAL_SCORE) {
+                    hit = goal;
+                }
+                if (hit) {
+                    const uint8_t cur = trunc ? 2 : 1;
+                    if (tt == 0 || cur == 1) tt = cur;
+                }
+            }
+            e.terminal = tt;
+            if (goal) {
+                if (by > 0) e.penalty_blue++;
+                else e.penalty_orange++;
+            }
+            e.episode_steps++;
+            uint8_t tj = tt;
+            if (!tj && g.max_episode_steps > 0 && e.episode_steps >= g.max_episode_steps) tj = 2;
+            if (tj) e.episode_steps = 0;
+            A->a.traj_term = tj;
+        }
+        sync(); P.mark(12);
+        if (valid) {
+            const int pi = l & 3, q = l >> 2;
+            const PView me = view_player(A, pi);
+            v3 bp = ld3(A->s.ball.pos) * kBT2UU, bv = ld3(A->s.ball.vel) * kBT2UU, pbv = ld3(A->s.env.prev_ball_vel);
+            const int nr = g.plug->nr;
+            constexpr int kPer = (RLGPU_MAX_REWARDS + 3) / 4;
+            float ov[kPer];
+#pragma unroll
+            for (int k = 0; k < kPer; k++) ov[k] = 0.f;
+#pragma unroll 1
+            for (int k = 0; q + 4 * k < nr; k++) {
+                const int r = q + 4 * k;
+                const float o = reward_value(A, g.plug->rw[r], pi, me, bp, bv, pbv, A->a.goal != 0);
+#pragma unroll
+                for (int j = 0; j < kPer; j++) ov[j] = j == k ? o : ov[j];
+                if (pi == 0 && g.last_rewards) g.last_rewards[(size_t)arena * nr + r] = o;
+                if (g.reward_values) g.reward_values[((size_t)arena * 4 + pi) * nr + r] = o;
+            }
+            float all = 0.f;
+            const int base = (int)(threadIdx.x & ~15u) + pi;
+#pragma unroll
+            for (int r = 0; r < RLGPU_MAX_REWARDS; r++) {
+                if (r >= nr) break;
+                const float o = __shfl(ov[r >> 2], base + 4 * (r & 3));
+                all += o * g.plug->rw[r].weight;
+            }
+            if (l < 4) A->a.all_rewards[l] = all;
+        }
+        sync(); P.mark(12);
+        if (valid && l < 4) {
+            float r = A->a.all_rewards[l];
+            g.rewards[arena * 4 + l] = r;
+            if (g.out_rew) g.out_rew[arena * 4 + l] = r;
+            if (g.out_term) g.out_term[arena * 4 + l] = (int8_t)A->a.traj_term;
+        }
+        if (g.metrics && valid && l < 4) step_metrics(A, l, g.metrics + (size_t)arena * RLGPU_STEP_METRIC_SLOTS,
+                                                      g.metrics_players != 0);
+        uint8_t tj = 0;
+        if (valid) {
+            term = A->s.env.terminal;
+            tj = (uint8_t)A->a.traj_term;
+        }
+        sync(); P.mark(12);
+        if (valid && l == 0) {
+            g.terminals[arena] = term;
+            A->s.env.last_tick_count = A->s.env.tick_count;
+        }
+        const bool fused_reset = g.reset_mode == kResetTerminated && valid && term != 0;
+        if (valid) build_obs_rows(A, l);
+        sync(); P.mark(13);
+        if (valid) {
+            copy_rows(A, l, arena, g.obs, g.masks);
+            if (!fused_reset) copy_rows(A, l, arena, g.out_obs, g.out_masks);
+            if (tj == 2) {
+                copy_rows(A, l, arena, g.trunc_obs, nullptr);
+                copy_rows(A, l, arena, g.out_trunc, nullptr);
+            }
+        }
+        sync(); P.mark(13);
+        if (g.reset_mode == kResetTerminated) {
+            if (fused_reset && l == 0) kickoff_reset(A, g.seed, arena + g.arena_offset, g.fuzz != 0);
+            sync(); P.mark(14);
+            if (fused_reset) build_obs_rows(A, l);
+            sync(); P.mark(14);
+            if (fused_reset) {
+                copy_rows(A, l, arena, g.obs, g.masks);
+                copy_rows(A, l, arena, g.out_obs, g.out_masks);
+            }
+            sync(); P.mark(14);
+        }
+    }
+    if (g.reset_mode >= kResetSet) {
+        bool do_reset = false;
+        if (valid) {
+            if (g.reset_mode == kResetSet) do_reset = g.terminals[arena] != 0;
+            else if (g.reset_mode == kResetMask) do_reset = g.reset_mask ? g.reset_mask[arena] != 0 : true;
+            else if (g.reset_mode == kResetAll) do_reset = true;
+        }
+        sync(); P.mark(14);
+        if (do_reset && l == 0) {
+            kickoff_reset(A, g.seed, arena + g.arena_offset, g.fuzz != 0);
+            if (g.reset_mode == kResetSet) g.terminals[arena] = 0;
+        }
+        sync(); P.mark(14);
+        bool rebuild = do_reset || (valid && g.reset_mode == kRebuildObs);
+        if (rebuild) build_obs_rows(A, l);
+        sync(); P.mark(14);
+        if (rebuild) copy_rows(A, l, arena, g.obs, g.masks);
+        sync(); P.mark(14);
+    }
+    {
+        int first = blockIdx.x * kArenas;
+        int cnt = g.n - first < kArenas ? g.n - first : kArenas;
+        const int chunks = kRec / 16;
+        for (int k = threadIdx.x; k < cnt * chunks; k += kWG) {
+            int a = k / chunks, c = k % chunks;
+            uint4* dst = (uint4*)(g.arenas + (size_t)(first + a) * kRec) + c;
+            const uint4* src = (const uint4*)&lds[a] + c;
+            *dst = *src;
+        }
+    }
+    P.mark(15);
+    if (g.prof && valid && l == 0 && A->a.npen) {
+        atomicAdd(&g.prof[28], (unsigned long long)A->a.npen);
+        atomicAdd(&g.prof[kProfWG + (size_t)blockIdx.x * kProfPhases + 23], (unsigned long long)A->a.npen);
+        atomicAdd(&g.prof[kProfWG + (size_t)gridDim.x * kProfPhases + arena], (unsigned long long)A->a.npen);
+    }
diff --git a/reinforcement-learning_amd/csrc/infer_kernels.hpp b/reinforcement-learning_amd/csrc/infer_kernels.hpp
--- a/reinforcement-learning_amd/csrc/infer_kernels.hpp
+++ b/reinforcement-learning_amd/csrc/infer_kernels.hpp
@@ -114,9 +114,10 @@
     }
 }
 
-template <int MAXH, bool FULL, bool F16, int ACT>
+template <int MAXH, bool FULL, bool F16, int ACT, int NRW = IRW, int RS = IW>
 DEV void ln_act_rows(uint16_t (*Xs)[IPITCH], const uint16_t* gamma, const uint16_t* beta, int H, float slope, int use_ln,
                      int w, int lane) {
+    constexpr int IRW = NRW, IW = RS;
     const bool vec = (H % 8 == 0) && (MAXH % 8 == 0);
     const bool maxform = slope >= 0.f && slope <= 1.f;
     auto in = [&](int q) { return FULL || mlp::hcol<MAXH>(lane, q) < H; };
@@ -382,4 +383,156 @@
     INFER_MARK(15);
 }
 
-}
+constexpr int WR = 16;
+constexpr int WNC = 4;
+struct WaveLDS {
+    uint16_t X[2][WR][IPITCH];
+    uint8_t M[WR * ppo::kMaxA];
+    uint8_t Sel[WR];
+};
+
+template <int NC, bool F16>
+DEV void linear_tiles_wave(const uint16_t (*Xs)[IPITCH], const uint16_t* F, int KS, int jt0, int JT, int lane,
+                           f32x16 (&acc)[NC]) {
+    const uint16_t* base[NC];
+#pragma unroll
+    for (int c = 0; c < NC; c++) {
+        base[c] = F + ((int64_t)min(jt0 + c, JT - 1) * KS * 64 + lane) * 8;
+#pragma unroll
+        for (int r = 0; r < 16; r++) acc[c][r] = 0.f;
+    }
+    const int nc_act = min(NC, JT - jt0);
+    const bool live = (lane & 31) < WR;
+    const uint16_t* arow = Xs[lane & (WR - 1)] + 8 * (lane >> 5);
+    const int nch = (KS + 3) / 4;
+    auto load = [&](u32x4 (&b)[4][NC], int kc) {
+#pragma unroll
+        for (int s = 0; s < 4; s++) {
+            const int ks = min(kc * 4 + s, KS - 1);
+#pragma unroll
+            for (int c = 0; c < NC; c++) b[s][c] = *reinterpret_cast<const u32x4*>(base[c] + ks * 512);
+        }
+    };
+    auto step = [&](const u32x4 (&b)[4][NC], int kc) {
+#pragma unroll
+        for (int s = 0; s < 4; s++) {
+            const int ks = kc * 4 + s;
+            if (ks >= KS) break;
+            u32x4 t = *reinterpret_cast<const u32x4*>(arow + ks * 16);
+            const u32x4 z = {0u, 0u, 0u, 0u};
+            t = live ? t : z;
+            const bf16x8 av = __builtin_bit_cast(bf16x8, t);
+#pragma unroll
+            for (int c = 0; c < NC; c++) {
+                if (c >= nc_act) break;
+                acc[c] = mlp::mfma16<F16>(av, __builtin_bit_cast(bf16x8, b[s][c]), acc[c]);
+            }
+        }
+    };
+    u32x4 b0[4][NC], b1[4][NC];
+    load(b0, 0);
+    for (int kc = 0; kc < nch; kc += 2) {
+        load(b1, kc + 1);
+        step(b0, kc);
+        load(b0, kc + 2);
+        step(b1, kc + 1);
+    }
+}
+
+template <bool F16, int ACT>
+DEV void wave_infer(const InferArgs& a, WaveLDS& S, const float* X, const uint8_t* masks, int rows, int64_t row0,
+                    uint64_t step, const uint8_t* row_sel, int32_t* act, float* logp, float* out_f, int lane) {
+    uint16_t (*in)[IPITCH] = S.X[0];
+    uint16_t (*out)[IPITCH] = S.X[1];
+    const int A = a.width[a.nl];
+    {
+        const int k16 = (a.in + 15) / 16 * 16;
+#pragma unroll 4
+        for (int r = 0; r < WR; r++)
+            for (int c = lane; c < k16; c += 64) {
+                const float x = X[(int64_t)min(r, rows - 1) * a.in + min(c, a.in - 1)];
+                in[r][c] = (r < rows && c < a.in) ? f2h<F16>(x) : (uint16_t)0;
+            }
+    }
+    if (a.mode == 1) {
+        for (int f = lane; f < rows * A; f += 64) S.M[f] = masks[f];
+        if (lane < WR) {
+            uint8_t selv = 1;
+            if (row_sel) selv = (row_sel[min(lane, rows - 1)] != 0) == (a.sel != 0);
+            S.Sel[lane] = lane < rows && selv;
+        }
+    }
+    f32x16 acc[WNC];
+    for (int l = 0; l + 1 < a.nl; l++) {
+        const int KS = (a.width[l] + 15) / 16, N = a.width[l + 1], JT = (N + 31) / 32;
+        const int n16 = (N + 15) / 16 * 16;
+        const uint16_t* bias = a.P + a.hb[l];
+        __syncthreads();
+        for (int jt0 = 0; jt0 < JT; jt0 += WNC) {
+            linear_tiles_wave<WNC, F16>(in, a.F + a.fw[l], KS, jt0, JT, lane, acc);
+#pragma unroll
+            for (int c = 0; c < WNC; c++) {
+                const int j = (jt0 + c) * 32 + (lane & 31);
+                if (jt0 + c >= JT || j >= n16) continue;
+                const float bj = j < N ? h2f<F16>(bias[j]) : 0.f;
+#pragma unroll
+                for (int r = 0; r < 8; r++)
+                    out[acc_row(0, r, lane)][j] = j < N ? f2h<F16>(acc[c][r] + bj) : (uint16_t)0;
+            }
+        }
+        const uint16_t* gg = a.P + (a.hg[l] >= 0 ? a.hg[l] : 0);
+        const uint16_t* bb = a.P + (a.hbe[l] >= 0 ? a.hbe[l] : 0);
+        __syncthreads();
+#pragma unroll 1
+        for (int w = 0; w < WR; w += 8) {
+            if (N == 512) ln_act_rows<8, true, F16, ACT, 8, 1>(out, gg, bb, N, a.slope, a.use_ln, w, lane);
+            else if (N <= 64) ln_act_rows<1, false, F16, ACT, 8, 1>(out, gg, bb, N, a.slope, a.use_ln, w, lane);
+            else if (N <= 128) ln_act_rows<2, false, F16, ACT, 8, 1>(out, gg, bb, N, a.slope, a.use_ln, w, lane);
+            else if (N <= 256) ln_act_rows<4, false, F16, ACT, 8, 1>(out, gg, bb, N, a.slope, a.use_ln, w, lane);
+            else ln_act_rows<8, false, F16, ACT, 8, 1>(out, gg, bb, N, a.slope, a.use_ln, w, lane);
+        }
+        uint16_t (*t)[IPITCH] = in;
+        in = out;
+        out = t;
+    }
+    const int l = a.nl - 1, KS = (a.width[l] + 15) / 16, N = a.width[l + 1], JT = (N + 31) / 32;
+    __syncthreads();
+    linear_tiles_wave<WNC, F16>(in, a.F + a.fw[l], KS, 0, JT, lane, acc);
+#pragma unroll
+    for (int c = 0; c < WNC; c++) {
+        const int j = c * 32 + (lane & 31);
+        if (c >= JT || j >= N) continue;
+        const float bj = h2f<F16>(a.P[a.hb[l] + j]);
+#pragma unroll
+        for (int r = 0; r < 8; r++) {
+            const int i = acc_row(0, r, lane);
+            const uint16_t y = f2h<F16>(acc[c][r] + bj);
+            if (a.mode == 0) {
+                if (i < rows) out_f[(int64_t)i * N + j] = h2f<F16>(y);
+            } else {
+                out[i][j] = y;
+            }
+        }
+    }
+    if (a.mode == 0) return;
+    __syncthreads();
+    const auto rowfn = [&](int g, const uint16_t*& lg, const uint8_t*& mk, float*& pr, int& row, bool& ok) {
+        lg = out[g];
+        mk = S.M + g * N;
+        pr = reinterpret_cast<float*>(&out[g][kSampleProbs]);
+        row = g;
+        ok = S.Sel[g] != 0;
+    };
+    ppo::sample_rows_looped<WR, F16>(rowfn, N, a.temp, a.det, a.seed, step, row0, lane, act, logp);
+}
+
+template <bool F16, int ACT = mlp::ACT_LEAKY>
+__global__ void __launch_bounds__(64) mlp_infer_wave(InferArgs a) {
+    __shared__ WaveLDS S;
+    const int r0 = blockIdx.x * WR, A = a.width[a.nl];
+    wave_infer<F16, ACT>(a, S, a.X + (int64_t)r0 * a.in, a.masks ? a.masks + (int64_t)r0 * A : nullptr, min(WR, a.n - r0),
+                         a.row0 + r0, a.step, a.row_sel ? a.row_sel + r0 : nullptr, a.act ? a.act + r0 : nullptr,
+                         a.logp ? a.logp + r0 : nullptr, a.out_f ? a.out_f + (int64_t)r0 * A : nullptr, (int)threadIdx.x);
+}
+
+}
diff --git a/reinforcement-learning_amd/csrc/infer_wave.hip b/reinforcement-learning_amd/csrc/infer_wave.hip
--- /dev/null
+++ b/reinforcement-learning_amd/csrc/infer_wave.hip
@@ -0,0 +1,27 @@
+#include <hip/hip_bf16.h>
+#include <hip/hip_fp16.h>
+#include <hip/hip_runtime.h>
+#include <math.h>
+#include <stdint.h>
+
+#include <cstdlib>
+#include <cstring>
+
+#include "../../include/rlgpu_detmath.h"
+#include "common.hpp"
+
+namespace {
+#include "infer_kernels.hpp"
+}
+
+namespace rlgpu {
+
+void launch_mlp_infer_wave(bool f16, unsigned blocks, hipStream_t s, const void* args, size_t bytes) {
+    infer::InferArgs a;
+    if (bytes != sizeof(a)) throw Error(RLGPU_ERR_STATE, "launch_mlp_infer_wave: InferArgs size mismatch");
+    std::memcpy(&a, args, sizeof(a));
+    if (f16) hipLaunchKernelGGL((infer::mlp_infer_wave<true, mlp::ACT_LEAKY>), dim3(blocks), dim3(64), 0, s, a);
+    else hipLaunchKernelGGL((infer::mlp_infer_wave<false, mlp::ACT_LEAKY>), dim3(blocks), dim3(64), 0, s, a);
+}
+
+}
diff --git a/reinforcement-learning_amd/csrc/ppo.hip b/reinforcement-learning_amd/csrc/ppo.hip
--- a/reinforcement-learning_amd/csrc/ppo.hip
+++ b/reinforcement-learning_amd/csrc/ppo.hip
@@ -624,7 +624,7 @@
     Draw sub(int64_t b) const { return {det, step, act + b, logp ? logp + b : nullptr, row_sel ? row_sel + b : nullptr, sel}; }
 };
 
-void infer_fused(rlgpu_ppo* h, int mi, bool ver, const Rows& r, float* out_f, const Draw* d, hipStream_t s) {
+infer::InferArgs fused_args(const rlgpu_ppo* h, int mi, bool ver, const Rows& r, float* out_f, const Draw* d) {
     const auto& c = h->chain[mi];
     const int n = (int)r.n;
     infer::InferArgs a{};
@@ -658,6 +658,19 @@
         a.logp = d->logp;
         a.row_sel = d->row_sel;
         a.sel = d->sel;
+    }
+    return a;
+}
+
+bool wave_ok(const rlgpu_ppo* h, int mi) { return fused_ok(h, mi) && h->cfg.activation == mlp::ACT_LEAKY; }
+
+void infer_fused(rlgpu_ppo* h, int mi, bool ver, const Rows& r, float* out_f, const Draw* d, hipStream_t s, bool wave = false) {
+    const int n = (int)r.n;
+    infer::InferArgs a = fused_args(h, mi, ver, r, out_f, d);
+    if (wave) {
+        rlgpu::launch_mlp_infer_wave(f16(h), ceil_div(n, infer::WR), s, &a, sizeof(a));
+        RLGPU_CHECK_HIP(hipGetLastError());
+        return;
     }
     a.trace = g_infer_trace;
     if (a.trace && ceil_div(n, infer::IR) * 16 > g_infer_trace_cap)
@@ -1079,6 +1092,53 @@
     });
 }
 
+bool rlgpu::ppo_wave_policy(rlgpu_ppo* h, int obs_size, int num_actions) {
+    return h && wave_ok(h, 0) && h->cfg.obs_size == obs_size && h->cfg.num_actions == num_actions;
+}
+void rlgpu::ppo_wave_args(rlgpu_ppo* h, const float* d_obs, const uint8_t* d_masks, int64_t n, int deterministic,
+                          uint64_t rng_step, int32_t* d_actions, float* d_logp, void* blob, size_t cap, bool* f16_out) {
+    RLGPU_REQUIRE(h && wave_ok(h, 0), "ppo_wave_args: the policy is not on the one-wave kernel");
+    const Draw d{deterministic, rng_step, d_actions, d_logp};
+    const infer::InferArgs a = fused_args(h, 0, false, Rows{d_obs, n, h->cfg.sample_row_offset, d_masks}, nullptr, &d);
+    RLGPU_REQUIRE(sizeof(a) <= cap, "ppo_wave_args: InferArgs do not fit the blob");
+    std::memcpy(blob, &a, sizeof(a));
+    *f16_out = f16(h);
+}
+
+extern "C" int rlgpu_ppo_wave_infer(rlgpu_ppo* h, int32_t model) { return h && model >= 0 && model < 3 && wave_ok(h, model); }
+
+extern "C" int rlgpu_ppo_infer_actions_wave(rlgpu_ppo* h, const float* d_obs, const uint8_t* d_masks, int32_t n, int64_t row0,
+                                            int32_t deterministic, uint64_t rng_step, const uint8_t* d_old_rows,
+                                            int32_t* d_actions, float* d_logp, void* stream) {
+    return rlgpu::guarded([&] {
+        RLGPU_REQUIRE(h && d_obs && d_masks && d_actions, "null argument");
+        RLGPU_REQUIRE(n >= 0 && row0 >= 0, "n and row0 must be >= 0");
+        RLGPU_REQUIRE(!d_old_rows || h->has_ver, "rlgpu_ppo_infer_actions_wave: old rows without a version set");
+        if (!wave_ok(h, 0))
+            throw rlgpu::Error(RLGPU_ERR_UNSUPPORTED, "rlgpu_ppo_infer_actions_wave: the policy is not eligible for the one-wave "
+                                                      "kernel (the fused kernel's conditions and LeakyReLU / ReLU)");
+        if (n == 0) return;
+        const Rows rows{d_obs, n, row0 + h->cfg.sample_row_offset, d_masks};
+        Draw d{deterministic, rng_step, d_actions, d_logp, d_old_rows, 0};
+        for (d.sel = 0; d.sel < (d_old_rows ? 2 : 1); d.sel++) {
+            if (d.sel) d.logp = nullptr;
+            infer_fused(h, 0, d.sel != 0, rows, nullptr, &d, rlgpu::as_stream(stream), true);
+        }
+    });
+}
+
+extern "C" int rlgpu_ppo_infer_values_wave(rlgpu_ppo* h, int32_t model, const float* d_obs, int32_t n, float* d_out,
+                                           void* stream) {
+    return rlgpu::guarded([&] {
+        RLGPU_REQUIRE(h && d_obs && d_out && n >= 0 && model >= 0 && model < 2, "rlgpu_ppo_infer_values_wave: bad argument");
+        if (!wave_ok(h, model))
+            throw rlgpu::Error(RLGPU_ERR_UNSUPPORTED, "rlgpu_ppo_infer_values_wave: the model is not eligible for the one-wave "
+                                                      "kernel (the fused kernel's conditions and LeakyReLU / ReLU)");
+        if (n == 0) return;
+        infer_fused(h, model, false, Rows{d_obs, n, 0, nullptr}, d_out, nullptr, rlgpu::as_stream(stream), true);
+    });
+}
+
 extern "C" int rlgpu_ppo_fused_infer(rlgpu_ppo* h, int32_t model) { return h && model >= 0 && model < 3 && fused_ok(h, model); }
 
 extern "C" int rlgpu_ppo_infer_critic(rlgpu_ppo* h, const float* d_obs, int64_t n, float* d_values, void* stream) {
diff --git a/reinforcement-learning_amd/host/learner.cpp b/reinforcement-learning_amd/host/learner.cpp
--- a/reinforcement-learning_amd/host/learner.cpp
+++ b/reinforcement-learning_amd/host/learner.cpp
@@ -440,9 +440,39 @@
     }
 }
 
+constexpr bool kAutoCollectLoop = true;
+
+bool Learner::CollectLoopOk() const {
+    if (hook_ || K_ > 1 || trajMode() || oldTeam_ >= 0) return false;
+    return rlgpu_envset_collect_loop_ok(env_->handle(), ppo_->handle()) != 0;
+}
+
+void Learner::CollectLoop() {
+    const rlgpu_rollout_view& v = exp_.v;
+    const rlgpu_collect_rollout ro{v.obs, v.masks, v.actions, v.logp, v.rewards, v.terms, v.trunc_obs};
+    if (envTiming_) {
+        EnsureEvents(2);
+        hipCheck(hipEventRecord(ev_[0], s_), "event");
+    }
+    RlgpuCheck(rlgpu_envset_collect_loop(env_->handle(), ppo_->handle(), exp_.T, &ro, cfg_.deterministic != 0,
+                                         (uint64_t)stats.rng_step, s_),
+               "collection loop");
+    if (envTiming_) hipCheck(hipEventRecord(ev_[1], s_), "event");
+    stats.rng_step += exp_.T;
+}
+
 void Learner::Collect() {
     if (trajMode()) {
         CollectTrajectories();
+        return;
+    }
+    collectLoopUsed_ = false;
+    const bool wantLoop = cfg_.collect_groups < 0 ||
+                          (kAutoCollectLoop && cfg_.collect_groups == 0 && cfg_.num_arenas >= kAutoCollectArenas);
+    if (wantLoop && CollectLoopOk()) {
+        collectGroupsUsed_ = 1;
+        collectLoopUsed_ = true;
+        CollectLoop();
         return;
     }
     if (const int G = CollectGroups(); G > 1 && EnsureGroupStreams(G)) {
@@ -830,9 +860,11 @@
         double ms = 0;
         const int nt = trajMode() ? 0 : exp_.T * std::max(1, collectGroupsUsed_);
         std::vector<float> each(nt);
+        float loop = 0;
+        if (collectLoopUsed_) hipCheck(hipEventElapsedTime(&loop, ev_[0], ev_[1]), "elapsed");
         for (int t = 0; t < nt; t++) {
-            float x = 0;
-            hipCheck(hipEventElapsedTime(&x, ev_[2 * t], ev_[2 * t + 1]), "elapsed");
+            float x = loop / (float)nt;
+            if (!collectLoopUsed_) hipCheck(hipEventElapsedTime(&x, ev_[2 * t], ev_[2 * t + 1]), "elapsed");
             ms += x;
             each[t] = x;
         }
diff --git a/reinforcement-learning_amd/host/learner.hpp b/reinforcement-learning_amd/host/learner.hpp
--- a/reinforcement-learning_amd/host/learner.hpp
+++ b/reinforcement-learning_amd/host/learner.hpp
@@ -199,6 +199,9 @@
     bool EnsureGroupStreams(int G);
     int collectGroupsUsed_ = 1;
     void CollectGrouped(int G);
+    bool collectLoopUsed_ = false;
+    bool CollectLoopOk() const;
+    void CollectLoop();
     uint8_t* oldRows_[2] = {nullptr, nullptr};
     const uint8_t* OldRows() const { return oldTeam_ >= 0 ? oldRows_[oldTeam_] : nullptr; }
     int32_t* trainRows_ = nullptr;
diff --git a/reinforcement-learning_amd/rlgpu/learner.py b/reinforcement-learning_amd/rlgpu/learner.py
--- a/reinforcement-learning_amd/rlgpu/learner.py
+++ b/reinforcement-learning_amd/rlgpu/learner.py
@@ -452,7 +452,7 @@
         L = _lib.lib()
         if fn is None:
             self._hook = None
-            _lib.check(L.rlgpu_learner_set_step_hook(self._h, None, None), "rlgpu_learner_set_step_hook")
+            _lib.check(L.rlgpu_learner_set_step_hook(self._h, ctypes.cast(None, self._HOOK), None), "rlgpu_learner_set_step_hook")
             return
 
         def thunk(_user, phase):
diff --git a/reinforcement-learning_amd/rlgpu/ppo.py b/reinforcement-learning_amd/rlgpu/ppo.py
--- a/reinforcement-learning_amd/rlgpu/ppo.py
+++ b/reinforcement-learning_amd/rlgpu/ppo.py
@@ -62,6 +62,10 @@
     L.rlgpu_ppo_set_optimizer_step.argtypes = [vp, i64]
     L.rlgpu_ppo_set_version.argtypes = [vp, vp, vp]
     L.rlgpu_ppo_infer_actions_mixed.argtypes = [vp, vp, vp, i32, i32, u64, vp, vp, vp, vp]
+    L.rlgpu_ppo_infer_actions_rows.argtypes = [vp, vp, vp, i32, i64, i32, u64, vp, vp, vp, vp]
+    L.rlgpu_ppo_infer_actions_wave.argtypes = [vp, vp, vp, i32, i64, i32, u64, vp, vp, vp, vp]
+    L.rlgpu_ppo_infer_values_wave.argtypes = [vp, i32, vp, i32, vp, vp]
+    L.rlgpu_ppo_wave_infer.argtypes = [vp, i32]
     L.rlgpu_permutation.argtypes = [i64, u64, u64, vp, vp]
     L.rlgpu_kernel_timing.argtypes = [i32]
     L.rlgpu_kernel_timing_read.argtypes = [vp, vp, vp, i32]
@@ -268,6 +272,33 @@
                                                             _lib.stream_ptr()), "rlgpu_ppo_infer_actions_mixed")
         return actions, logp
 
+    def _actions_rows(self, entry, obs, masks, row0, step, deterministic, old_rows, actions, logp):
+        import torch
+        n = obs.shape[0]
+        actions = torch.empty(n, dtype=torch.int32, device=self.device) if actions is None else actions
+        logp = torch.empty(n, device=self.device) if logp is None else logp
+        _lib.check(getattr(_lib.lib(), entry)(self._h, _lib.ptr(obs), _lib.ptr(masks), n, row0, int(deterministic), step,
+                                              _lib.ptr(old_rows) if old_rows is not None else None, _lib.ptr(actions),
+                                              _lib.ptr(logp), _lib.stream_ptr()), entry)
+        return actions, logp
+
+    def infer_actions_rows(self, obs, masks, row0=0, step=0, deterministic=False, old_rows=None, actions=None, logp=None):
+        return self._actions_rows("rlgpu_ppo_infer_actions_rows", obs, masks, row0, step, deterministic, old_rows, actions, logp)
+
+    def infer_actions_wave(self, obs, masks, row0=0, step=0, deterministic=False, old_rows=None, actions=None, logp=None):
+        return self._actions_rows("rlgpu_ppo_infer_actions_wave", obs, masks, row0, step, deterministic, old_rows, actions, logp)
+
+    def infer_values_wave(self, model, obs, out=None):
+        import torch
+        n = obs.shape[0]
+        out = torch.empty((n, self.model_out(model)), device=self.device) if out is None else out
+        _lib.check(_lib.lib().rlgpu_ppo_infer_values_wave(self._h, model, _lib.ptr(obs), n, _lib.ptr(out), _lib.stream_ptr()),
+                   "rlgpu_ppo_infer_values_wave")
+        return out
+
+    def wave_infer_ok(self, model=0):
+        return bool(_lib.lib().rlgpu_ppo_wave_infer(self._h, model))
+
     def infer_critic(self, obs, out=None):
         import torch
         n = obs.shape[0]
```

Result: faster. 2.345 million (median of 6 runs) (+15.4%).
